# DevilInChina/spmv

Measured on AMD Instinct MI355X. Metric: SpMV GFLOP/s (fp64 CSR, y = A x through spmv()), higher is better.
Workload: dtype f64

## Files before the change

include/spmv_hip.h:

```cpp
#include "spmv_Defines.h"
#if defined(__cplusplus)
extern "C" {
#endif
#ifndef SPMV_HIP_EXT_H
#define SPMV_HIP_EXT_H

enum {
    SPMV_HIP_OK = 0,
    SPMV_HIP_E_NODEVICE = 1,
    SPMV_HIP_E_ALLOC = 2,
    SPMV_HIP_E_ARG = 3,
    SPMV_HIP_E_RUNTIME = 4,
    SPMV_HIP_E_NOSTATE = 5,
    SPMV_HIP_E_RANGE = 6
};
int spmv_hip_last_error(void);
const char *spmv_hip_last_error_string(void);
void spmv_hip_clear_error(void);

int spmv_hip_device_count(void);
int spmv_hip_set_stream(spmv_Handle_t handle, void *hip_stream);
int spmv_hip_set_async(spmv_Handle_t handle, int async);
int spmv_hip_synchronize(spmv_Handle_t handle);
void spmv_hip_trim_pool(void);
// ... 88 lines not shown
int spmv_hip_attention_merge(spmv_Handle_t handle, int heads, int dv,
                             const void *O1, long long ldo1, const void *L1, long long ldl1,
                             const void *O2, long long ldo2, const void *L2, long long ldl2,
                             void *O, long long ldo,
                             void *L, long long ldl);

int spmv_hip_attention_gqa_backward_lse(spmv_Handle_t handle, BASIC_INT_TYPE m, const BASIC_INT_TYPE *RowPtr, const BASIC_INT_TYPE *ColIdx,
                                        const void *Matrix_Val, int heads, int kv_heads, int k, int dv, double scale,
                                        const void *Q, long long ldq, const void *K, long long ldk, const void *V, long long ldv,
                                        const void *B, long long ldb,
                                        const void *G, long long ldg,
                                        const void *O, long long ldo,
                                        const void *L, long long ldl,
                                        void *dQ, long long lddq,
                                        void *dK, long long lddk,
                                        void *dV, long long lddv,
                                        void *dB, long long lddb);

enum { SPMV_HIP_T_HANDLE = 0, SPMV_HIP_T_F16 = 1, SPMV_HIP_T_BF16 = 2 };

int spmv_hip_attention_gqa_lse_16(spmv_Handle_t handle, BASIC_INT_TYPE m, const BASIC_INT_TYPE *RowPtr, const BASIC_INT_TYPE *ColIdx,
                                  const void *Matrix_Val, int heads, int kv_heads, int k, int dv, double scale,
                                  int io_type,
                                  const void *Q, long long ldq, const void *K, long long ldk, const void *V, long long ldv,
                                  const void *B, long long ldb,
                                  void *O, long long ldo, int o_type,
                                  void *L, long long ldl);

int spmv_hip_attention_gqa_backward_16(spmv_Handle_t handle, BASIC_INT_TYPE m, const BASIC_INT_TYPE *RowPtr, const BASIC_INT_TYPE *ColIdx,
                                       const void *Matrix_Val, int heads, int kv_heads, int k, int dv, double scale,
                                       int io_type,
                                       const void *Q, long long ldq, const void *K, long long ldk, const void *V, long long ldv,
                                       const void *B, long long ldb,
                                       const void *G, long long ldg,
                                       const void *O, long long ldo,
                                       const void *L, long long ldl,
                                       int dq_type, void *dQ, long long lddq,
                                       int dkv_type, void *dK, long long lddk,
                                       void *dV, long long lddv,
                                       void *dB, long long lddb);

int spmv_hip_set_option(const char *key, long value);
long spmv_hip_get_option(const char *key);
int spmv_hip_set_thread_option(const char *key, long value);
void spmv_hip_clear_thread_options(void);
long spmv_hip_get_handle_option(spmv_Handle_t handle, const char *key);

typedef struct spmv_hip_info {
    int device;
    int schedule;
    int lanes_per_row;
    int sell_c, sell_sigma;
    int tile_nnz;
    int m, n;
    long long nnz;
    long long stored_nnz;
    int max_row_len, min_row_len, empty_rows;
    double mean_row_len;
    long long device_bytes;
    long long alg_bytes;
    double inspect_ms;
    const char *schedule_name;
    const char *kernel_name;
    int tuned_choice;
    float tune_ms[3];
    int x_groups;
    int x_groups_staged;
    int cache_blocked;
    long long stream_bytes;
    long long x_bytes;
    float route_ms[2];
    float split_ms[2];
    long long far_nnz;
    long long run_nnz;
    long long byte_nnz;
    long long tmpl_nnz;
    int blk_waves;
    char launch_kernels[160];
    int reproducible;
    int x_span_max;
    int lds_bytes;
    long long packed_nnz;
    float pack_ms[2];
} spmv_hip_info;
int spmv_hip_get_info(spmv_Handle_t handle, spmv_hip_info *out);
int spmv_hip_get_transpose_info(spmv_Handle_t handle, spmv_hip_info *out);

int spmv_hip_multi_gpus(spmv_Handle_t handle);
int spmv_hip_multi_uses_rccl(spmv_Handle_t handle);
int spmv_hip_multi_slices(spmv_Handle_t handle, int gpu, void **x_slice, long long *x_first, long long *x_count,
                          void **y_block, long long *y_first, long long *y_count, int *device);
int spmv_hip_multi_step(spmv_Handle_t handle);
int spmv_hip_multi_step_async(spmv_Handle_t handle);
int spmv_hip_multi_synchronize(spmv_Handle_t handle);
void spmv_hip_create_handle_from_blocks(spmv_Handle_t *Handle, int blocks, const BASIC_INT_TYPE *rows, BASIC_INT_TYPE n,
                                        BASIC_INT_TYPE *const *RowPtr, BASIC_INT_TYPE *const *ColIdx, void *const *Matrix_Val,
                                        SPMV_METHODS Function, BASIC_SIZE_TYPE size);

enum { SPMV_HIP_CG_CONVERGED = 0, SPMV_HIP_CG_MAX_ITERATIONS = 1, SPMV_HIP_CG_BREAKDOWN = 2, SPMV_HIP_CG_NONFINITE = 3 };
typedef struct spmv_hip_cg_options {
    double rtol, atol;
    int max_iterations;
    int check_every;
    int use_x0;
    const void *Dinv;
    double *history;
} spmv_hip_cg_options;
typedef struct spmv_hip_cg_result {
    int status;
    int iterations;
    double rr, bb;
} spmv_hip_cg_result;
int spmv_hip_cg(spmv_Handle_t handle, BASIC_INT_TYPE m, const BASIC_INT_TYPE *RowPtr, const BASIC_INT_TYPE *ColIdx,
                const void *Matrix_Val, const void *B, void *X,
                const spmv_hip_cg_options *opt, spmv_hip_cg_result *res);

int spmv_hip_bicgstab(spmv_Handle_t handle, BASIC_INT_TYPE m, const BASIC_INT_TYPE *RowPtr, const BASIC_INT_TYPE *ColIdx,
                      const void *Matrix_Val, const void *B, void *X,
                      const spmv_hip_cg_options *opt, spmv_hip_cg_result *res);

#define SPMV_HIP_CG_COLUMNS_MAX 16
int spmv_hip_cg_columns(spmv_Handle_t handle, BASIC_INT_TYPE m, const BASIC_INT_TYPE *RowPtr, const BASIC_INT_TYPE *ColIdx,
                        const void *Matrix_Val, int k, const void *B, long long ldb, void *X, long long ldx,
                        const spmv_hip_cg_options *opt, spmv_hip_cg_result *res );

#define SPMV_HIP_GMRES_RESTART_MAX 32
int spmv_hip_gmres(spmv_Handle_t handle, BASIC_INT_TYPE m, const BASIC_INT_TYPE *RowPtr, const BASIC_INT_TYPE *ColIdx,
                   const void *Matrix_Val, const void *B, void *X, int restart,
                   const spmv_hip_cg_options *opt, spmv_hip_cg_result *res);

#endif

#if defined(__cplusplus)
}
#endif
```

spmv_amd/api.py:

```python
from __future__ import annotations

import ctypes as C
import enum
import math
import os

import numpy as np

_PKG = os.path.dirname(os.path.abspath(__file__))
LIB_PATH = os.path.join(_PKG, "lib", "libspmv_hip.so")


class VECTORIZED_WAY(enum.IntEnum):
    VECTOR_NONE = 0
    VECTOR_AVX2 = 1
    VECTOR_AVX512 = 2
    VECTOR_HIP = 3
    VECTOR_TOTAL_SIZE = 4


class SPMV_METHODS(enum.IntEnum):
    Method_Serial = 0
    Method_Parallel = 1
    Method_Balanced = 2
    Method_Balanced2 = 3
    Method_Balanced_Yid = 4
    Method_SellCSigma = 5
    Method_CSR5SPMV = 6
    Method_Total_Size = 7
    Method_Numa = 8


_I = C.POINTER(C.c_int)
_V = C.c_void_p


class spmv_Handle(C.Structure):
    _fields_ = [("spmvMethod", C.c_int), ("data_size", C.c_ulong), ("nthreads", C.c_ulong),
                ("vectorizedWay", C.c_int), ("Level_3_opt_used", C.c_int), ("RowPtr", _I),
                ("ColIdx", _I), ("index", _I), ("Matrix_Val", _V), ("Y_temp", _V),
                ("extraHandle", _V)]


spmv_Handle_t = C.POINTER(spmv_Handle)


class spmv_hip_info(C.Structure):
    _fields_ = [("device", C.c_int), ("schedule", C.c_int), ("lanes_per_row", C.c_int),
                ("sell_c", C.c_int), ("sell_sigma", C.c_int), ("tile_nnz", C.c_int),
                ("m", C.c_int), ("n", C.c_int), ("nnz", C.c_longlong), ("stored_nnz", C.c_longlong),
                ("max_row_len", C.c_int), ("min_row_len", C.c_int), ("empty_rows", C.c_int),
                ("mean_row_len", C.c_double), ("device_bytes", C.c_longlong),
                ("alg_bytes", C.c_longlong), ("inspect_ms", C.c_double),
                ("schedule_name", C.c_char_p), ("kernel_name", C.c_char_p),
                ("tuned_choice", C.c_int), ("tune_ms", C.c_float * 3),
                ("x_groups", C.c_int), ("x_groups_staged", C.c_int), ("cache_blocked", C.c_int),
                ("stream_bytes", C.c_longlong), ("x_bytes", C.c_longlong), ("route_ms", C.c_float * 2), ("split_ms", C.c_float * 2), ("far_nnz", C.c_longlong), ("run_nnz", C.c_longlong), ("byte_nnz", C.c_longlong), ("tmpl_nnz", C.c_longlong),
                ("blk_waves", C.c_int), ("launch_kernels", C.c_char * 160), ("reproducible", C.c_int),
                ("x_span_max", C.c_int), ("lds_bytes", C.c_int),
                ("packed_nnz", C.c_longlong), ("pack_ms", C.c_float * 2)]


class spmv_hip_cg_options(C.Structure):
    _fields_ = [("rtol", C.c_double), ("atol", C.c_double), ("max_iterations", C.c_int), ("check_every", C.c_int), ("use_x0", C.c_int),
                ("Dinv", C.c_void_p), ("history", C.POINTER(C.c_double))]


class spmv_hip_cg_result(C.Structure):
    _fields_ = [("status", C.c_int), ("iterations", C.c_int), ("rr", C.c_double), ("bb", C.c_double)]


CG_STATUS = ("converged", "max_iterations", "breakdown", "nonfinite")

_GQA = "heads kv_heads k dv scale"
_ATTENTION = {stem: tuple((sizes + " " + operands).split()) for stem, sizes, operands in (
    ("attention", "k dv scale", "Q K V O"),
    ("attention_heads", "heads k dv scale", "Q K V O"),
    ("attention_backward", "k dv scale", "Q K V G dQ dK dV"),
    ("attention_heads_backward", "heads k dv scale", "Q K V G dQ dK dV"),
    ("attention_bias", "heads k dv scale", "Q K V B O"),
    ("attention_bias_backward", "heads k dv scale", "Q K V B G dQ dK dV dB"),
    ("attention_gqa", _GQA, "Q K V B O"),
    ("attention_gqa_backward", _GQA, "Q K V B G dQ dK dV dB"),
    ("attention_gqa_lse", _GQA, "Q K V B O L"),
    ("attention_gqa_lse_16", _GQA + " io_type", "Q K V B O o_type L"),
    ("attention_gqa_backward_lse", _GQA, "Q K V B G O L dQ dK dV dB"),
    ("attention_gqa_backward_16", _GQA + " io_type", "Q K V B G O L dq_type dQ dkv_type dK dV dB"),
)}
_CSR = [spmv_Handle_t, C.c_int, _V, _V, _V]
_TIMED = [spmv_Handle_t]
_TAIL = [C.c_int, C.c_int, C.POINTER(C.c_float)]


def _attention_prototypes():
    out = {}
    for stem, row in _ATTENTION.items():
        args = []
        for name in row:
            args += [C.c_double] if name == "scale" else [C.c_int] if name.islower() else [_V, C.c_longlong]
        out[f"spmv_hip_{stem}"] = (C.c_int, _CSR + args)
        out[f"spmv_hip_time_{stem}_launches"] = (C.c_double, _TIMED + args + _TAIL)
    return out


FUNCTIONS = {
    "spmv_create_handle_all_in_one": (None, [C.POINTER(spmv_Handle_t), C.c_int, C.c_int, _V, _V, _V,
                                             C.c_ulong, C.c_int, C.c_ulong, C.c_int, C.c_char_p]),
    "spmv": (None, [spmv_Handle_t, C.c_int, _V, _V, _V, _V, _V]),
    "spmv_destory_handle": (None, [spmv_Handle_t]),
    "spmv_clear_handle": (None, [spmv_Handle_t]),
    "spmv_hip_last_error": (C.c_int, []),
    "spmv_hip_last_error_string": (C.c_char_p, []),
    "spmv_hip_clear_error": (None, []),
    "spmv_hip_device_count": (C.c_int, []),
    "spmv_hip_trim_pool": (None, []),
    "spmv_hip_set_stream": (C.c_int, [spmv_Handle_t, _V]),
    "spmv_hip_set_async": (C.c_int, [spmv_Handle_t, C.c_int]),
    "spmv_hip_synchronize": (C.c_int, [spmv_Handle_t]),
    "spmv_hip_set_option": (C.c_int, [C.c_char_p, C.c_long]),
    "spmv_hip_get_option": (C.c_long, [C.c_char_p]),
    "spmv_hip_set_thread_option": (C.c_int, [C.c_char_p, C.c_long]),
    "spmv_hip_clear_thread_options": (None, []),
    "spmv_hip_get_handle_option": (C.c_long, [spmv_Handle_t, C.c_char_p]),
    "spmv_hip_update_values": (C.c_int, [spmv_Handle_t, _V]),
    "spmv_hip_multi_gpus": (C.c_int, [spmv_Handle_t]),
    "spmv_hip_multi_uses_rccl": (C.c_int, [spmv_Handle_t]),
    "spmv_hip_multi_slices": (C.c_int, [spmv_Handle_t, C.c_int, C.POINTER(_V), C.POINTER(C.c_longlong), C.POINTER(C.c_longlong),
                                        C.POINTER(_V), C.POINTER(C.c_longlong), C.POINTER(C.c_longlong), _I]),
    "spmv_hip_multi_step": (C.c_int, [spmv_Handle_t]),
    "spmv_hip_multi_step_async": (C.c_int, [spmv_Handle_t]),
    "spmv_hip_multi_synchronize": (C.c_int, [spmv_Handle_t]),
    "spmv_hip_create_handle_from_blocks": (None, [C.POINTER(spmv_Handle_t), C.c_int, _I, C.c_int, C.POINTER(_V), C.POINTER(_V), C.POINTER(_V),
                                                  C.c_int, C.c_ulong]),
    "spmv_hip_get_info": (C.c_int, [spmv_Handle_t, C.POINTER(spmv_hip_info)]),
    "spmv_hip_time_launches": (C.c_double, [spmv_Handle_t, _V, _V, C.c_int, C.c_int, C.POINTER(C.c_float)]),
    "spmv_hip_spmm": (C.c_int, [spmv_Handle_t, C.c_int, _V, _V, _V, C.c_int, _V, C.c_longlong, _V, C.c_longlong]),
    "spmv_hip_time_spmm_launches": (C.c_double, [spmv_Handle_t, C.c_int, _V, C.c_longlong, _V, C.c_longlong, C.c_int, C.c_int,
                                                 C.POINTER(C.c_float)]),
    "spmv_hip_spmv_transpose": (C.c_int, [spmv_Handle_t, C.c_int, _V, _V, _V, _V, _V]),
    "spmv_hip_prepare_transpose": (C.c_int, [spmv_Handle_t]),
    "spmv_hip_get_transpose_info": (C.c_int, [spmv_Handle_t, C.POINTER(spmv_hip_info)]),
    "spmv_hip_time_transpose_launches": (C.c_double, [spmv_Handle_t, _V, _V, C.c_int, C.c_int, C.POINTER(C.c_float)]),
    "spmv_hip_transpose_map": (C.c_int, [spmv_Handle_t, _I, _I]),
# ... 95 lines not shown


def _ptr(a):
    if a is None:
        return None
    if isinstance(a, int):
        return a
    if isinstance(a, np.ndarray):
        if not a.flags["C_CONTIGUOUS"]:
            raise ValueError("array must be contiguous")
        return a.ctypes.data
    if hasattr(a, "data_ptr"):
        if not a.is_contiguous():
            raise ValueError("tensor must be contiguous")
        return a.data_ptr()
    raise TypeError(type(a))


def _itemsize(a):
    return a.dtype.itemsize if isinstance(a, np.ndarray) else a.element_size()


def spmv_create_handle_all_in_one(m, n, RowPtr, ColIdx, Matrix_Val, nthreads, Function, size,
                                  vectorizedWay=VECTORIZED_WAY.VECTOR_HIP, MtxToken=None, check=True):
    lib = load()
    lib.spmv_hip_clear_error()
    h = spmv_Handle_t()
    tok = MtxToken.encode() if isinstance(MtxToken, str) else MtxToken
    lib.spmv_create_handle_all_in_one(C.byref(h), int(m), int(n), _ptr(RowPtr), _ptr(ColIdx), _ptr(Matrix_Val),
                                      int(nthreads), int(Function), int(size), int(vectorizedWay), tok)
    if check:
        _raise_if_error("spmv_create_handle_all_in_one")
    return h


def spmv(handle, m, RowPtr, ColIdx, Matrix_Val, Vector_Val_X, Vector_Val_Y, check=True):
    lib = load()
    lib.spmv(handle, int(m), _ptr(RowPtr), _ptr(ColIdx), _ptr(Matrix_Val), _ptr(Vector_Val_X), _ptr(Vector_Val_Y))
    if check:
        _raise_if_error("spmv")


def spmv_destory_handle(handle):
    load().spmv_destory_handle(handle)


def spmv_clear_handle(handle):
    load().spmv_clear_handle(handle)


def set_option(key, value):
    if load().spmv_hip_set_option(key.encode(), int(value)) != 0:
        load().spmv_hip_clear_error()
        raise ValueError(f"bad option {key}={value}")


def get_option(key):
    return load().spmv_hip_get_option(key.encode())


def set_thread_option(key, value):
    if load().spmv_hip_set_thread_option(key.encode(), int(value)) != 0:
        load().spmv_hip_clear_error()
        raise ValueError(f"bad option {key}={value}")


def clear_thread_options():
    load().spmv_hip_clear_thread_options()


def update_values(handle, Matrix_Val):
    _checked(load().spmv_hip_update_values(handle, _ptr(Matrix_Val)), "spmv_hip_update_values")


def _info_dict(info):
    out = {k: getattr(info, k) for k, _ in spmv_hip_info._fields_}
    out["schedule_name"] = (out["schedule_name"] or b"").decode()
    out["kernel_name"] = (out["kernel_name"] or b"").decode()
    out["launch_kernels"] = [k for k in (out["launch_kernels"] or b"").decode().split("+") if k]
    out["tune_ms"] = [float(v) for v in out["tune_ms"]]
    out["route_ms"] = [float(v) for v in out["route_ms"]]
    out["split_ms"] = [float(v) for v in out["split_ms"]]
    out["pack_ms"] = [float(v) for v in out["pack_ms"]]
    return out


def get_info(handle):
    info = spmv_hip_info()
    _checked(load().spmv_hip_get_info(handle, C.byref(info)), "spmv_hip_get_info")
    return _info_dict(info)


def get_transpose_info(handle):
    info = spmv_hip_info()
    _checked(load().spmv_hip_get_transpose_info(handle, C.byref(info)), "spmv_hip_get_transpose_info")
    return _info_dict(info)


def set_stream(handle, stream_ptr, async_=True):
    lib = load()
    lib.spmv_hip_set_stream(handle, stream_ptr)
    lib.spmv_hip_set_async(handle, 1 if async_ else 0)
    _raise_if_error("spmv_hip_set_stream")


def time_launches(handle, x, y, warmup=10, iters=100):
    return _timed("spmv_hip_time_launches", (handle, _ptr(x), _ptr(y)), warmup, iters)


def _block(a, name):
    if a is None:
        return None, 0, 0, 0
    if isinstance(a, np.ndarray):
        if a.ndim == 2 and a.size == 0:
            return a.ctypes.data, a.shape[0], a.shape[1], max(a.shape[1], 1)
        if a.ndim != 2 or (a.strides[1] != a.itemsize and a.shape[1] > 1) or a.strides[0] % a.itemsize:
            raise ValueError(f"{name} must be 2-D with column stride 1")
        return a.ctypes.data, a.shape[0], a.shape[1], a.strides[0] // a.itemsize
    if hasattr(a, "data_ptr"):
        if a.dim() != 2 or (a.stride(1) != 1 and a.shape[1] > 1):
            raise ValueError(f"{name} must be 2-D with column stride 1")
        return a.data_ptr(), a.shape[0], a.shape[1], a.stride(0)
    raise TypeError(type(a))


def _blocks(A, a_name, B, b_name):
    pa, _, k, lda = _block(A, a_name)
    pb, _, kb, ldb = _block(B, b_name)
    if A is not None and B is not None and kb != k:
        raise ValueError(f"{a_name} has {k} columns, {b_name} {kb}")
    if A is None:
        k = kb
    return int(k), pa, int(max(lda, 1) if A is not None else k), pb, int(max(ldb, 1) if B is not None else k)


def spmm(handle, m, RowPtr, ColIdx, Matrix_Val, X, Y, check=True):
    k, px, ldx, py, ldy = _blocks(X, "X", Y, "Y")
    return _checked(load().spmv_hip_spmm(handle, int(m), _ptr(RowPtr), _ptr(ColIdx), _ptr(Matrix_Val), k, px, ldx, py, ldy), "spmv_hip_spmm", check)


def time_spmm_launches(handle, X, Y, warmup=10, iters=100):
    px, _, k, ldx = _block(X, "X")
    py, _, _, ldy = _block(Y, "Y")
    return _timed("spmv_hip_time_spmm_launches", (handle, int(k), px, int(max(ldx, 1)), py, int(max(ldy, 1))), warmup, iters)


def spmv_transpose(handle, m, RowPtr, ColIdx, Matrix_Val, X, Y, check=True):
    return _checked(load().spmv_hip_spmv_transpose(handle, int(m), _ptr(RowPtr), _ptr(ColIdx), _ptr(Matrix_Val), _ptr(X), _ptr(Y)), "spmv_hip_spmv_transpose", check)


def prepare_transpose(handle, check=True):
    return _checked(load().spmv_hip_prepare_transpose(handle), "spmv_hip_prepare_transpose", check)


def time_transpose_launches(handle, x, y, warmup=10, iters=100):
    return _timed("spmv_hip_time_transpose_launches", (handle, _ptr(x), _ptr(y)), warmup, iters)


def transpose_map(handle, n, nnz):
    rp = np.empty(int(n) + 1, dtype=np.int32)
    perm = np.empty(max(int(nnz), 1), dtype=np.int32)
    _checked(load().spmv_hip_transpose_map(handle, rp.ctypes.data_as(_I), perm.ctypes.data_as(_I)), "spmv_hip_transpose_map")
    return rp, perm[:int(nnz)]


def spmm_transpose(handle, m, RowPtr, ColIdx, Matrix_Val, X, Y, check=True):
# ... 703 lines not shown
```

spmv_amd/csrc/kernels/csr_vector_tile.hpp:

```cpp
#pragma once
#include <climits>
#include <type_traits>
#include "common.hpp"
#include "csr_vector4.hpp"
#include "xwindows.hpp"

namespace spmv {

constexpr int kVecTileThreads = 256;
constexpr int kVecTileRows = kVecTileThreads;
constexpr int kTmplMax = 64;
constexpr int kTmplCount = 8;
constexpr int kTmplRows = 1024;
__device__ __forceinline__ void tile_rows(int b, int m, int rows_per_tile, const int *__restrict__ split, long long &r0, long long &r1)
{
    if (split) { r0 = split[b]; r1 = split[b + 1]; }
    else { r0 = (long long) b * rows_per_tile; r1 = r0 + rows_per_tile < m ? r0 + rows_per_tile : m; }
}

template <typename T, int L>
struct Lane4 {
    static constexpr int EPL = 16 / (int) sizeof(T);
    static __device__ __forceinline__ int pos(int l, int k) { return (k / EPL) * EPL * L + EPL * l + (k % EPL); }
    static __device__ __forceinline__ void load_val(const T *__restrict__ val, int base, int l, T (&v)[4])
// ... 219 lines not shown
        sum = group_sum_dpp<L>(sum);
        if (l == 0) y_lds[s * RW + sub] = sum;
        if (s + D < L) issue(s + D);
    }
    wave_lds_sync();
    const long long row = rw0 + lane;
    const int len = rp_lds[lane + 1] - rp_lds[lane];
    if (row < row_end && len <= long_thr) y[row] = y_lds[lane];
}

template <typename T, int L, int DEPTH = 4, bool PRE = true, bool PACK = false>
__global__ __launch_bounds__(kVecTileThreads) void csr_vector_tile_kernel(int m, int long_thr, const int *__restrict__ rowptr,
                                                                          const int *__restrict__ colidx,
                                                                          const unsigned short *__restrict__ col_local,
                                                                          const T *__restrict__ val,
                                                                          const TileWindows *__restrict__ wins,
                                                                          const unsigned short *__restrict__ row_slot,
                                                                          const unsigned char *__restrict__ col8,
                                                                          const unsigned short *__restrict__ tmpl, const unsigned char *__restrict__ row_tid,
                                                                          const T *__restrict__ x, T *__restrict__ y,
                                                                          const unsigned *__restrict__ pk_lo = nullptr, const unsigned char *__restrict__ pk_hi = nullptr,
                                                                          const int *__restrict__ tile_e = nullptr)
{
    extern __shared__ __attribute__((aligned(16))) unsigned char vec_x_lds[];
    __shared__ unsigned short tm_lds[kTmplCount * kTmplMax];
    T *xs = reinterpret_cast<T *>(vec_x_lds);
    __shared__ int rp_lds[kVecTileThreads / kWave][kWave + 2];
    __shared__ unsigned rs_lds[kVecTileThreads / kWave][kWave];
    __shared__ T y_lds[kVecTileThreads / kWave][kWave];
    const int lane = threadIdx.x & (kWave - 1), wave = threadIdx.x / kWave;
    const long long rw0 = (long long) blockIdx.x * kVecTileRows + wave * kWave;
    long long r = rw0 + lane, re = rw0 + kWave;
    if (r > m) r = m;
    if (re > m) re = m;
    const int rp = rowptr[r];
    const int rpe = rowptr[re];
    const TileWindows &tw = wins[blockIdx.x];
    const bool staged = tw.nwin > 0, runs = tw.runs == 1, bytes = tw.runs == 2, templ = tw.runs == 3;
    int c0[4] = {0, 0, 0, 0};
    T v0[4] = {T(0), T(0), T(0), T(0)};
    PackArgs pk;
    PackRaw r0;
    bool packed = false;
    if constexpr (PACK) {
        pk.lo = pk_lo; pk.hi = pk_hi; pk.e = tile_e[blockIdx.x];
        packed = pk.e != kPackNone;
    }
    if (PRE) {
        const int sub = lane / L, l = lane % L;
        const int q0 = __shfl(rp, sub, kWave);
        const int a = q0 & ~3;
        if (runs | templ) {}
        else if (bytes) Lane4<T, L>::load_col8(col8, a, l, c0);
        else if (staged) Lane4<T, L>::load_col16(col_local, a, l, c0);
        else Lane4<T, L>::load_col32(colidx, a, l, c0);
        if (PACK && packed) r0.load(pk, a, l);
        else Lane4<T, L>::load_val(val, a, l, v0);
    }
    rp_lds[wave][lane] = rp;
    if (lane == 0) rp_lds[wave][kWave] = rpe;
    if (runs | bytes) rs_lds[wave][lane] = row_slot[r];
    if (templ) {
        rs_lds[wave][lane] = (unsigned) row_slot[r] | ((unsigned) row_tid[r] * kTmplMax << 16);
        for (int i = threadIdx.x; i < kTmplCount * kTmplMax; i += kVecTileThreads) tm_lds[i] = tmpl[(size_t) blockIdx.x * (kTmplCount * kTmplMax) + i];
    }
    stage_windows<kVecTileThreads, T>(tw, x, xs);
    if (threadIdx.x == 0) xs[tw.total] = T(0);
    __syncthreads();
    if (rw0 >= m) return;
    const unsigned zoff = (unsigned) tw.total * (unsigned) sizeof(T);
#define SPMV_TILE_WAVE(MODE, ...)                                                                                                                                   \
    do {                                                                                                                                                            \
        if (PACK && packed) csr_vector_tile_wave<T, L, MODE, DEPTH, PRE, 0, PACK>((long long) m, long_thr, rw0, lane, rp_lds[wave], rs_lds[wave], y_lds[wave], colidx, col_local, val, x, xs, zoff, y, c0, v0, __VA_ARGS__, pk, r0); \
        else csr_vector_tile_wave<T, L, MODE, DEPTH, PRE>((long long) m, long_thr, rw0, lane, rp_lds[wave], rs_lds[wave], y_lds[wave], colidx, col_local, val, x, xs, zoff, y, c0, v0, __VA_ARGS__); \
    } while (0)
    if (runs) SPMV_TILE_WAVE(2, col8, nullptr);
    else if (bytes) SPMV_TILE_WAVE(3, col8, nullptr);
    else if (templ) SPMV_TILE_WAVE(4, col8, tm_lds);
    else if (staged) SPMV_TILE_WAVE(1, col8, nullptr);
    else SPMV_TILE_WAVE(0, col8, nullptr);
#undef SPMV_TILE_WAVE
}

template <typename T, int L, int DEPTH = 4, bool WIDE = false>
__global__ __launch_bounds__(kVecTileThreads) void csr_vector_rows_kernel(int long_thr, const int *__restrict__ split,
                                                                          int rows_per_block, int m,
                                                                          const int *__restrict__ rowptr,
                                                                          const int *__restrict__ colidx,
                                                                          const unsigned short *__restrict__ col_local,
                                                                          const T *__restrict__ val,
                                                                          const TileWindows *__restrict__ wins,
                                                                          const unsigned short *__restrict__ row_slot,
                                                                          const unsigned char *__restrict__ col8,
                                                                          const unsigned short *__restrict__ tmpl, const unsigned char *__restrict__ row_tid,
                                                                          const T *__restrict__ x, T *__restrict__ y)
{
    __shared__ unsigned short tm_lds[kTmplCount * kTmplMax];
    constexpr int SHIFT = WIDE ? (sizeof(T) == 8 ? 3 : 2) : 0;
    extern __shared__ __attribute__((aligned(16))) unsigned char vec_x_lds[];
    T *xs = reinterpret_cast<T *>(vec_x_lds);
    __shared__ int rp_lds[kVecTileThreads / kWave][kWave + 2];
    __shared__ unsigned rs_lds[kVecTileThreads / kWave][kWave];
    __shared__ T y_lds[kVecTileThreads / kWave][kWave];
    const int lane = threadIdx.x & (kWave - 1), wave = threadIdx.x / kWave;
    long long r_begin, r_end;
    tile_rows(blockIdx.x, m, rows_per_block, split, r_begin, r_end);
    const TileWindows &tw = wins[blockIdx.x];
    const bool staged = tw.nwin > 0, runs = tw.runs == 1, bytes = tw.runs == 2, templ = tw.runs == 3;
    if (templ) for (int i = threadIdx.x; i < kTmplCount * kTmplMax; i += kVecTileThreads) tm_lds[i] = tmpl[(size_t) blockIdx.x * (kTmplCount * kTmplMax) + i];
    stage_windows<kVecTileThreads, T>(tw, x, xs);
    if (threadIdx.x == 0) xs[tw.total] = T(0);
    __syncthreads();
    const unsigned zoff = WIDE ? (unsigned) tw.total : (unsigned) tw.total * (unsigned) sizeof(T);
    const int c0[4] = {0, 0, 0, 0};
    const T v0[4] = {T(0), T(0), T(0), T(0)};
    for (long long rw0 = r_begin + (long long) wave * kWave; rw0 < r_end; rw0 += kVecTileRows) {
        long long r = rw0 + lane, re = rw0 + kWave;
        if (r > r_end) r = r_end;
        if (re > r_end) re = r_end;
        rp_lds[wave][lane] = rowptr[r];
        if (lane == 0) rp_lds[wave][kWave] = rowptr[re];
        if (runs | bytes) rs_lds[wave][lane] = row_slot[r];
        if (templ) rs_lds[wave][lane] = (unsigned) row_slot[r] | ((unsigned) row_tid[r] * kTmplMax << 16);
        wave_lds_sync();
        if (runs) csr_vector_tile_wave<T, L, 2, DEPTH, false, SHIFT>(r_end, long_thr, rw0, lane, rp_lds[wave], rs_lds[wave], y_lds[wave], colidx, col_local, val, x, xs, zoff, y, c0, v0);
        else if (bytes) csr_vector_tile_wave<T, L, 3, DEPTH, false, SHIFT>(r_end, long_thr, rw0, lane, rp_lds[wave], rs_lds[wave], y_lds[wave], colidx, col_local, val, x, xs, zoff, y, c0, v0, col8);
        else if (templ) csr_vector_tile_wave<T, L, 4, DEPTH, false, SHIFT>(r_end, long_thr, rw0, lane, rp_lds[wave], rs_lds[wave], y_lds[wave], colidx, col_local, val, x, xs, zoff, y, c0, v0, col8, tm_lds);
        else if (staged) csr_vector_tile_wave<T, L, 1, DEPTH, false, SHIFT>(r_end, long_thr, rw0, lane, rp_lds[wave], rs_lds[wave], y_lds[wave], colidx, col_local, val, x, xs, zoff, y, c0, v0);
        else csr_vector_tile_wave<T, L, 0, DEPTH, false, SHIFT>(r_end, long_thr, rw0, lane, rp_lds[wave], rs_lds[wave], y_lds[wave], colidx, col_local, val, x, xs, zoff, y, c0, v0);
        wave_lds_sync();
    }
}

enum { kVecPipeKernel, kVecTileKernel, kVecRowsKernel };
struct VecArgs {
    int kernel = kVecPipeKernel;
    int lanes = 64, depth = 4;
    bool pre = true, wide = false;
    int m = 0, long_thr = INT_MAX, tiles = 0, maxspan = 0, rows = 256;
    const int *rowptr = nullptr, *colidx = nullptr, *split = nullptr;
    const void *val = nullptr;
    const unsigned short *col = nullptr, *rowslot = nullptr, *tmpl = nullptr;
    const unsigned char *col8 = nullptr, *rowtid = nullptr;
    const TileWindows *wins = nullptr;
    const unsigned *pk_lo = nullptr;
    const unsigned char *pk_hi = nullptr;
    const int *pk_e = nullptr;
    int device = 0;
    hipStream_t stream = nullptr;
};
hipError_t vector_launch(const VecArgs &a, const double *x, double *y);
hipError_t vector_launch(const VecArgs &a, const float *x, float *y);
hipError_t vector_launch_packed(const VecArgs &a, const double *x, double *y);
hipError_t rows_launch(const VecArgs &a, const double *x, double *y);
hipError_t rows_launch(const VecArgs &a, const float *x, float *y);

}
```

spmv_amd/csrc/kernels/xwindows_inspect.hpp:

```cpp
#pragma once
#include "csr_vector_tile.hpp"

namespace spmv {

static __global__ __launch_bounds__(kBlock) void csr_tile_windows_kernel(int m, int n, int rows_per_tile, int long_thr, int max_cols, int slot_bytes,
                                                                  const int *__restrict__ split,
                                                                  const int *__restrict__ rowptr,
                                                                  const int *__restrict__ colidx,
                                                                  TileWindows *__restrict__ wins,
                                                                  unsigned short *__restrict__ col_local,
                                                                  unsigned short *__restrict__ row_slot ,
                                                                  unsigned char *__restrict__ col8 ,
                                                                  unsigned short *__restrict__ tmpl ,
                                                                  unsigned char *__restrict__ row_tid ,
                                                                  int *__restrict__ staged )
{
    long long r0, r1;
    tile_rows(blockIdx.x, m, rows_per_tile, split, r0, r1);
    const int sub = threadIdx.x / 16, l = threadIdx.x % 16;
    auto loop = [&](auto body) {
        for (long long r = r0 + sub; r < r1; r += kBlock / 16) {
            const int p0 = rowptr[r], p1 = rowptr[r + 1];
            if (p1 - p0 > long_thr) continue;
            for (int p = p0 + l; p < p1; p += 16) body(colidx[p], (long long) p);
// ... 106 lines not shown
            int mn = INT_MAX, mx = 0;
            for (int p = p0 + l; p < p1; p += 16) { const int sl = col_local[p]; mn = sl < mn ? sl : mn; mx = sl > mx ? sl : mx; }
#pragma unroll
            for (int o = 8; o > 0; o >>= 1) { mn = min(mn, __shfl_xor(mn, o, 16)); mx = max(mx, __shfl_xor(mx, o, 16)); }
            okb &= mx - mn <= 255 * slot_bytes;
            if (l == 0) nb += p1 - p0;
        }
        okb = __syncthreads_and(okb);
        if (!okb) return;
        for (long long r = r0 + sub; r < r1; r += kBlock / 16) {
            const int p0 = rowptr[r], p1 = rowptr[r + 1];
            int mn = INT_MAX;
            const bool on = p1 - p0 <= long_thr && p1 > p0;
            if (on) for (int p = p0 + l; p < p1; p += 16) { const int sl = col_local[p]; mn = sl < mn ? sl : mn; }
#pragma unroll
            for (int o = 8; o > 0; o >>= 1) mn = min(mn, __shfl_xor(mn, o, 16));
            if (on) for (int p = p0 + l; p < p1; p += 16) col8[p] = (unsigned char) ((col_local[p] - mn) / slot_bytes);
            if (l == 0) row_slot[r] = (unsigned short) (on ? mn : 0);
        }
#pragma unroll
        for (int o = kWave / 2; o > 0; o >>= 1) nb += __shfl_xor(nb, o, kWave);
        if ((threadIdx.x & (kWave - 1)) == 0 && nb) atomicAdd(staged + 6, nb);
        if (threadIdx.x == 0) {
            wins[blockIdx.x].runs = 2;
            atomicAdd(staged + 5, 1);
            atomicAdd(staged + 7, (int) (r1 - r0));
        }
        return;
    }
    for (long long r = r0 + sub * 16 + l; r < r1; r += kBlock) {
        const int p0 = rowptr[r], p1 = rowptr[r + 1];
        int slot = 0;
        if (p1 > p0 && p1 - p0 <= long_thr) {
            const int c0 = colidx[p0];
            int w = 0;
            for (int k = 1; k < nwin; ++k) w = c0 >= tw.start[k] ? k : w;
            slot = (tw.base[w] + (c0 - tw.start[w])) * slot_bytes;
        }
        row_slot[r] = (unsigned short) slot;
    }
#pragma unroll
    for (int o = kWave / 2; o > 0; o >>= 1) entries += __shfl_xor(entries, o, kWave);
    if ((threadIdx.x & (kWave - 1)) == 0 && entries) atomicAdd(staged + 3, entries);
    if (threadIdx.x == 0) {
        wins[blockIdx.x].runs = 1;
        atomicAdd(staged + 2, 1);
        atomicAdd(staged + 4, (int) (r1 - r0));
    }
}

static __global__ __launch_bounds__(kBlock) void range_windows_kernel(long long total, long long group_len,
                                                               const long long *__restrict__ bounds, int bstride, int scale,
                                                               long long nbounds ,
                                                               int n, int max_cols, int *__restrict__ cols,
                                                               unsigned short *__restrict__ cols16, int pack16,
                                                               TileWindows *__restrict__ wins, int *__restrict__ staged, int rewrite)
{
    long long b, e;
    if (bounds) {
        long long i0 = (long long) blockIdx.x * bstride, i1 = i0 + bstride;
        if (i0 > nbounds) i0 = nbounds;
        if (i1 > nbounds) i1 = nbounds;
        b = bounds[i0] * scale;
        e = bounds[i1] * scale;
    }
    else { b = (long long) blockIdx.x * group_len; e = b + group_len; }
    if (e > total) e = total;
    auto loop = [&](auto body) {
        for (long long i = b + threadIdx.x; i < e; i += kBlock) body(cols[i], i);
    };
    auto store = [&](long long pos, int slot, int tile_total) {
        if (!cols16) { if (slot >= 0) cols[pos] = slot; return; }
        long long q = pos;
        if (pack16) {
            const long long tn = (long long) kWave * pack16, t = pos / tn;
            const int o = (int) (pos - t * tn), i = o / kWave, lane = o % kWave;
            q = t * tn + (i / 4) * (4 * kWave) + lane * 4 + (i % 4);
        }
        cols16[q] = (unsigned short) (slot >= 0 ? slot : tile_total);
    };
    build_windows(n, max_cols, loop, store, wins[blockIdx.x], staged, rewrite != 0);
}

static __global__ __launch_bounds__(kBlock) void wins_total_kernel(int count, const TileWindows *__restrict__ wins, unsigned long long *__restrict__ sum,
                                                            unsigned long long *__restrict__ staged_tiles)
{
    unsigned long long t = 0, c = 0;
    for (long long i = (long long) blockIdx.x * kBlock + threadIdx.x; i < count; i += (long long) gridDim.x * kBlock)
        if (wins[i].nwin > 0) { t += (unsigned long long) wins[i].total; c += 1; }
#pragma unroll
    for (int o = kWave / 2; o > 0; o >>= 1) { t += __shfl_xor(t, o, kWave); c += __shfl_xor(c, o, kWave); }
    if ((threadIdx.x & (kWave - 1)) == 0 && c) { atomicAdd(sum, t); atomicAdd(staged_tiles, c); }
}

}
```

spmv_amd/csrc/shim/inspect.hpp:

```cpp
#pragma once

static int build_range_windows(spmv_dev *d, int groups, long long total, long long group_len, const long long *bounds, int bstride,
                               int scale, int max_cols, int *cols, TileWindows *wins, int *staged_out, int *maxtotal_out,
                               unsigned short *cols16 = nullptr, int pack16 = 0, long long nbounds = 0)
{
    int *cnt = nullptr;
    int host2[2] = {0, 0};
    *staged_out = *maxtotal_out = 0;
    if (groups <= 0) return SPMV_HIP_OK;
    HIP_TRY(pool_malloc((void **) &cnt, 2 * sizeof(int)));
    hipError_t e = hipMemsetAsync(cnt, 0, 2 * sizeof(int), d->stream);
    range_windows_kernel<<<groups, kBlock, 0, d->stream>>>(total, group_len, bounds, bstride, scale, nbounds, d->n, max_cols, cols, cols16, pack16, wins, cnt, 0);
    if (e == hipSuccess) e = hipGetLastError();
    if (e == hipSuccess) e = hipMemcpyAsync(host2, cnt, sizeof host2, hipMemcpyDeviceToHost, d->stream);
    if (e == hipSuccess) e = hipStreamSynchronize(d->stream);
    if (e == hipSuccess && host2[0] * 2 >= groups) {
        range_windows_kernel<<<groups, kBlock, 0, d->stream>>>(total, group_len, bounds, bstride, scale, nbounds, d->n, max_cols, cols, cols16, pack16, wins, cnt, 1);
        e = hipGetLastError();
        if (e == hipSuccess) e = hipStreamSynchronize(d->stream);
        *staged_out = host2[0];
        *maxtotal_out = host2[1];
    }
    (void) pool_free(cnt);
    if (e != hipSuccess) return fail(SPMV_HIP_E_RUNTIME, "x-window inspector: %s", hipGetErrorString(e));
    return SPMV_HIP_OK;
}

constexpr size_t kVecXTileBytes = 48 * 1024;
template <typename T> static int build_long_rows(spmv_dev *d, int thr);
template <typename T>
static int build_csr5(spmv_dev *d, Csr5Plan &P, int m, long long nnz, const int *rowptr, const int *colidx, const T *val, int empty_rows,
                      double mean_row_len, const int *out_rows, bool natural = false, int sigma_override = 0);
template <typename T> static int autotune_vector(spmv_dev *d);
template <typename T> static int autotune_rows(spmv_dev *d);
static int build_packed_values(spmv_dev *d);
template <typename T> static int autotune_blocked(spmv_dev *d);
template <typename T> static double time_schedule(spmv_dev *d, int iters);
template <typename T> static int split_make(spmv_dev *d, spmv_dev **near_out, spmv_dev **far_out, bool values_only);
template <typename T> static int build_tile_windows(spmv_dev *d, int tiles, const int *split, int rows_per_tile = kVecTileRows, bool wide = false);
static int wins_sum(spmv_dev *d, const TileWindows *wins, int count, long long *elems, long long *tiles);
constexpr size_t kVecWideXTileBytes = 96 * 1024;

static int build_rowblock(spmv_dev *d)
{
    d->rb_stride = d->plan.rowblock_nnz;
    d->nblocks = (int) ((d->nnz + d->rb_stride - 1) / d->rb_stride);
    if (d->nblocks < 1) d->nblocks = 1;
    ALLOC_TRY(d, &d->rb_split, sizeof(int) * ((size_t) d->nblocks + 1), true);
    rowblock_split_kernel<<<grid_for((long long) d->nblocks + 1, kBlock, INT_MAX), kBlock, 0, d->stream>>>(
        d->m, (int) d->nnz, d->nblocks, d->rb_stride, d->rowptr, d->rb_split);
    HIP_TRY(hipGetLastError());
    HIP_TRY(hipStreamSynchronize(d->stream));
    return SPMV_HIP_OK;
}

template <typename T>
static int build_rowblock_tiles(spmv_dev *d)
{
    const int L = d->plan.lanes_per_row;
    int rc = build_long_rows<T>(d, L * 64 > 256 ? L * 64 : 256);
    if (rc) return rc;
    rc = build_tile_windows<T>(d, d->nblocks, d->rb_split);
    if (rc) return rc;
    if (d->vt_staged * 2 < d->vt_tiles && !d->plan.forced) {
        rc = build_tile_windows<T>(d, d->nblocks, d->rb_split, kVecTileRows, true);
        if (rc) return rc;
        if (d->vt_staged * 2 < d->vt_tiles) rc = build_tile_windows<T>(d, d->nblocks, d->rb_split);
    }
    return rc;
}

template <typename T>
static int build_tile_windows(spmv_dev *d, int tiles, const int *split, int rows_per_tile, bool wide)
{
    int *cnt = nullptr;
    int host2[11] = {0, 0, 0, 0, 0, 0, 0, 0, 0, 0, 0};
    d->vt_tiles = tiles;
    ALLOC_TRY(d, &cnt, sizeof host2, true);
    static_assert(kVecXTileBytes <= 65536, "LDS byte offsets must fit 16 bits");
    static_assert(kVecWideXTileBytes / sizeof(float) <= 65536, "LDS slot indices must fit 16 bits");
    if (!d->vt_col) {
        ALLOC_TRY(d, &d->vt_col, sizeof(unsigned short) * ((size_t) d->nnz + kStreamPad), true);
        HIP_TRY(hipMemsetAsync(d->vt_col, 0, sizeof(unsigned short) * ((size_t) d->nnz + kStreamPad), d->stream));
    }
    if (!d->vt_rowslot && d->plan.run_tiles) {
        ALLOC_TRY(d, &d->vt_rowslot, sizeof(unsigned short) * ((size_t) d->m + kStreamPad), true);
        HIP_TRY(hipMemsetAsync(d->vt_rowslot, 0, sizeof(unsigned short) * ((size_t) d->m + kStreamPad), d->stream));
    }
    if (!d->vt_col8 && d->vt_rowslot && !getenv("SPMV_HIP_NO_BYTE_TILES")) {
        ALLOC_TRY(d, &d->vt_col8, (size_t) d->nnz + kStreamPad, true);
        HIP_TRY(hipMemsetAsync(d->vt_col8, 0, (size_t) d->nnz + kStreamPad, d->stream));
    }
    if (d->vt_tmpl) { sched_free(d, d->vt_tmpl); d->vt_tmpl = nullptr; }
    if (d->vt_rowslot && !getenv("SPMV_HIP_NO_TEMPLATE_TILES")) {
        ALLOC_TRY(d, &d->vt_tmpl, sizeof(unsigned short) * kTmplCount * kTmplMax * (size_t) tiles, true);
        if (!d->vt_rowtid) {
            ALLOC_TRY(d, &d->vt_rowtid, (size_t) d->m + kStreamPad, true);
            HIP_TRY(hipMemsetAsync(d->vt_rowtid, 0, (size_t) d->m + kStreamPad, d->stream));
        }
    }
    if (d->vt_wins) sched_free(d, d->vt_wins);
    ALLOC_TRY(d, &d->vt_wins, sizeof(TileWindows) * (size_t) tiles, true);
    HIP_TRY(hipMemsetAsync(cnt, 0, sizeof host2, d->stream));
    csr_tile_windows_kernel<<<tiles, kBlock, 0, d->stream>>>(d->m, d->n, rows_per_tile, d->long_thr,
                                                             (int) ((wide ? kVecWideXTileBytes : kVecXTileBytes) / sizeof(T)) - 1, wide ? 1 : (int) sizeof(T),
                                                             split, d->rowptr, d->colidx,
                                                             d->vt_wins, d->vt_col, d->vt_rowslot, d->vt_col8, d->vt_tmpl, d->vt_rowtid, cnt);
    HIP_TRY(hipGetLastError());
    HIP_TRY(hipMemcpyAsync(host2, cnt, sizeof host2, hipMemcpyDeviceToHost, d->stream));
    HIP_TRY(hipStreamSynchronize(d->stream));
    d->vt_staged = host2[0];
    d->vt_maxspan = host2[1];
    d->vt_run_tiles = host2[2];
    d->vt_run_nnz = host2[3];
    d->vt_run_rows = host2[4];
    d->vt_byte_tiles = host2[5];
    d->vt_byte_nnz = host2[6];
    d->vt_byte_rows = host2[7];
    d->vt_tmpl_tiles = host2[8];
    d->vt_tmpl_nnz = host2[9];
    d->vt_tmpl_rows = host2[10];
    if (d->vt_tmpl && d->vt_tmpl_tiles == 0) { sched_free(d, d->vt_tmpl); d->vt_tmpl = nullptr; sched_free(d, d->vt_rowtid); d->vt_rowtid = nullptr; }
    if (d->vt_col8 && d->vt_byte_tiles == 0) { sched_free(d, d->vt_col8); d->vt_col8 = nullptr; }
    d->vt_wide = wide;
    d->vt_rows = rows_per_tile;
    return SPMV_HIP_OK;
}

constexpr size_t kSellXTileBytes = 96 * 1024;

template <typename T>
static int build_long_rows(spmv_dev *d, int thr)
{
    d->long_thr = thr;
    d->nlong = 0;
    d->c5_long = Csr5Plan();
    if (d->stats.max_row_len <= thr) return SPMV_HIP_OK;
    const int nb = (int) (((long long) d->m + kScanTile - 1) / kScanTile);
    int *flags = nullptr, *sums = nullptr, *total = nullptr, *scratch = nullptr;
    ALLOC_TRY(d, &sums, sizeof(int) * (size_t) nb, true);
    ALLOC_TRY(d, &total, sizeof(int), true);
    HIP_TRY(pool_malloc((void **) &flags, sizeof(int) * (size_t) d->m));
    long_rows_flag_kernel<<<grid_for(d->m, kBlock, d->cus * 8), kBlock, 0, d->stream>>>(d->m, thr, d->rowptr, flags);
    scan_block_sums_kernel<<<nb, kBlock, 0, d->stream>>>(d->m, flags, sums);
    scan_sums_inplace_kernel<<<1, kBlock, 0, d->stream>>>(nb, sums, total);
    if (hipMemcpyAsync(&d->nlong, total, sizeof(int), hipMemcpyDeviceToHost, d->stream) != hipSuccess || hipStreamSynchronize(d->stream) != hipSuccess) {
        (void) pool_free(flags);
        d->nlong = 0;
        return fail(SPMV_HIP_E_RUNTIME, "long-row scan failed");
    }
    if (d->nlong == 0) { (void) pool_free(flags); return SPMV_HIP_OK; }
    int rc = dev_alloc(d, (void **) &d->long_rows, sizeof(int) * (size_t) d->nlong, true);
    if (!rc) rc = dev_alloc(d, (void **) &scratch, sizeof(int) * (size_t) d->nlong, true);
    if (rc) { (void) pool_free(flags); d->nlong = 0; return rc; }
    csr5_compact_kernel<<<nb, kBlock, 0, d->stream>>>(d->m, flags, sums, d->rowptr, scratch, d->long_rows);
    hipError_t e = hipStreamSynchronize(d->stream);
    (void) pool_free(flags);
    if (e != hipSuccess) { d->nlong = 0; return fail(SPMV_HIP_E_RUNTIME, "long-row compaction: %s", hipGetErrorString(e)); }
    ALLOC_TRY(d, &d->lr_seg_start, sizeof(long long) * ((size_t) d->nlong + 1), true);

    {
        long long sub_nnz = 0;
        long_rows_len_kernel<<<grid_for(d->nlong, kBlock, INT_MAX), kBlock, 0, d->stream>>>(d->nlong, d->long_rows, d->rowptr, scratch);
        scan_i32_to_i64_kernel<<<1, kBlock, 0, d->stream>>>(d->nlong, scratch, d->lr_seg_start);
        HIP_TRY(hipGetLastError());
        HIP_TRY(hipMemcpyAsync(&sub_nnz, d->lr_seg_start + d->nlong, sizeof(long long), hipMemcpyDeviceToHost, d->stream));
        HIP_TRY(hipStreamSynchronize(d->stream));
        d->lsub_nnz = sub_nnz;
        ALLOC_TRY(d, &d->lsub_rowptr, sizeof(int) * ((size_t) d->nlong + 1), true);
        ALLOC_TRY(d, &d->lsub_colidx, sizeof(int) * (size_t) sub_nnz, true);
        ALLOC_TRY(d, &d->lsub_val, sizeof(T) * (size_t) sub_nnz, true);
        narrow_i64_kernel<<<grid_for((long long) d->nlong + 1, kBlock, INT_MAX), kBlock, 0, d->stream>>>(d->nlong + 1, d->lr_seg_start, d->lsub_rowptr);
        long_rows_gather_kernel<T><<<d->nlong, kBlock, 0, d->stream>>>(d->long_rows, d->rowptr, d->colidx, (const T *) d->val, d->lsub_rowptr,
                                                                      d->lsub_colidx, (T *) d->lsub_val);
        HIP_TRY(hipGetLastError());
        return build_csr5<T>(d, d->c5_long, d->nlong, sub_nnz, d->lsub_rowptr, d->lsub_colidx, (const T *) d->lsub_val, 0,
                             (double) sub_nnz / (double) d->nlong, d->long_rows);
    }
}


template <typename T>
static int build_vector_tiles(spmv_dev *d)
{
    d->vt_staged = d->vt_maxspan = 0;
    const int rows = kVecTileRows;
    d->vt_tiles = (int) (((long long) d->m + rows - 1) / rows);
    if (d->vt_tiles == 0 || d->nnz == 0) return SPMV_HIP_OK;
    int rc = build_tile_windows<T>(d, d->vt_tiles, nullptr, rows);
    if (rc || d->plan.forced) return rc;
    if (d->vt_staged * 2 >= d->vt_tiles) {
        long long welems = 0, wtiles = 0;
        const long long stream = (d->nnz - d->lsub_nnz) * ((long long) sizeof(T) + 2);
        if (getenv("SPMV_HIP_NO_WIDE_BY_COST") || wins_sum(d, d->vt_wins, d->vt_tiles, &welems, &wtiles) != SPMV_HIP_OK || stream <= 0 ||
            (double) welems * sizeof(T) <= 0.5 * (double) stream)
            return SPMV_HIP_OK;
        const int narrow_tiles = d->vt_tiles, w_rows = 4 * kVecTileRows;
        const int w_tiles = (int) (((long long) d->m + w_rows - 1) / w_rows);
        rc = build_tile_windows<T>(d, w_tiles, nullptr, w_rows, true);
        if (rc) return rc;
        long long welems_w = 0;
        if (d->vt_staged == d->vt_tiles && wins_sum(d, d->vt_wins, d->vt_tiles, &welems_w, &wtiles) == SPMV_HIP_OK && welems_w * 2 <= welems) return SPMV_HIP_OK;
        return build_tile_windows<T>(d, narrow_tiles, nullptr, rows);
    }
    const int wide_rows = 4 * kVecTileRows;
    const int wide_tiles = (int) (((long long) d->m + wide_rows - 1) / wide_rows);
    rc = build_tile_windows<T>(d, wide_tiles, nullptr, wide_rows, true);
    if (rc) return rc;
    if (d->vt_staged * 2 >= d->vt_tiles) return SPMV_HIP_OK;
    return build_tile_windows<T>(d, (int) (((long long) d->m + rows - 1) / rows), nullptr, rows);
}

static __global__ __launch_bounds__(kVecTileThreads) void pack_tiles_kernel(int m, int L, int long_thr, const int *__restrict__ rowptr, const double *__restrict__ val,
                                                                            unsigned *__restrict__ lo, unsigned char *__restrict__ hi, int *__restrict__ tile_e,
                                                                            unsigned long long *__restrict__ cnt)
{
    __shared__ int s_bad, s_top, s_low;
    const int C = 4 * L;
    const long long r0 = (long long) blockIdx.x * kVecTileRows, r1 = r0 + kVecTileRows < m ? r0 + kVecTileRows : m;
    if (threadIdx.x == 0) { s_bad = 0; s_top = INT_MIN; s_low = INT_MAX; }
    __syncthreads();
    const int p_begin = rowptr[r0], p_end = rowptr[r1];
    int bad = 0, top = INT_MIN, low = INT_MAX;
    if (r0 + threadIdx.x < r1) {
        const int a = rowptr[r0 + threadIdx.x], len = rowptr[r0 + threadIdx.x + 1] - a;
        bad = (a & (C - 1)) != 0 || (len & (C - 1)) != 0 || len > long_thr;
    }
    for (int p = p_begin + (int) threadIdx.x; p < p_end; p += kVecTileThreads) {
        const unsigned long long b = (unsigned long long) __double_as_longlong(val[p]);
        const int E = (int) ((b >> 52) & 0x7ff);
        const unsigned long long frac = b & 0xfffffffffffffull;
        if (E == 0x7ff || b == 0x8000000000000000ull) bad = 1;
        else if (E | (frac != 0)) {
            const unsigned long long mant = E ? frac | (1ull << 52) : frac;
            const int base = (E ? E : 1) - 1075;
            top = max(top, base + 63 - __clzll((long long) mant));
            low = min(low, base + __ffsll((long long) mant) - 1);
        }
    }
#pragma unroll
    for (int o = kWave / 2; o > 0; o >>= 1) {
        bad |= __shfl_xor(bad, o, kWave);
        top = max(top, __shfl_xor(top, o, kWave));
        low = min(low, __shfl_xor(low, o, kWave));
    }
    if ((threadIdx.x & (kWave - 1)) == 0) {
        if (bad) atomicOr(&s_bad, 1);
        atomicMax(&s_top, top);
        atomicMin(&s_low, low);
    }
    __syncthreads();
    const bool zero = s_top == INT_MIN;
    const bool ok = !s_bad && (zero || s_top - s_low <= 54);
    const int e = zero ? 0 : s_low;
    if (threadIdx.x == 0) {
        tile_e[blockIdx.x] = ok ? e : kPackNone;
        if (ok) { atomicAdd(cnt, 1ull); atomicAdd(cnt + 1, (unsigned long long) (p_end - p_begin)); }
    }
    if (!ok || !lo) return;
    for (int s = p_begin + 4 * (int) threadIdx.x; s < p_end; s += 4 * kVecTileThreads) {
        const int q = s & (C - 1), blk = s - q, l = q >> 2;
        unsigned w[4], h[4];
#pragma unroll
        for (int k = 0; k < 4; ++k) {
            const unsigned long long b = (unsigned long long) __double_as_longlong(val[blk + (k >> 1) * 2 * L + 2 * l + (k & 1)]);
            const int E = (int) ((b >> 52) & 0x7ff);
            const unsigned long long frac = b & 0xfffffffffffffull;
            const unsigned long long mant = E ? frac | (1ull << 52) : frac;
            const int sh = (E ? E : 1) - 1075 - e;
            long long kk = sh >= 0 ? (long long) (mant << sh) : (long long) (mant >> -sh);
            if (b >> 63) kk = -kk;
            w[k] = (unsigned) kk;
            h[k] = (unsigned) (kk >> 32) & 0xffffffu;
// ... 529 lines not shown
    if (threadIdx.x == 0 && distinct > seg_limit && distinct * 3 > wlen) atomicAdd(hopeless, 1);
}

static bool sample_says_no_locality(spmv_dev *d)
{
    constexpr int kWindows = 64, kLen = 4096;
    if (d->nnz < (long long) kWindows * kLen * 4) return false;
    int *cnt = nullptr, h = 0;
    if (pool_malloc((void **) &cnt, sizeof(int)) != hipSuccess) { (void) hipGetLastError(); return false; }
    hipError_t e = hipMemsetAsync(cnt, 0, sizeof(int), d->stream);
    const int seg_limit = (int) (kCsr5XTileBytes / d->vsize / 64);
    locality_sample_kernel<<<kWindows, kBlock, 0, d->stream>>>(d->nnz, kWindows, kLen, d->colidx, seg_limit, cnt);
    if (e == hipSuccess) e = hipGetLastError();
    if (e == hipSuccess) e = hipMemcpyAsync(&h, cnt, sizeof(int), hipMemcpyDeviceToHost, d->stream);
    if (e == hipSuccess) e = hipStreamSynchronize(d->stream);
    (void) pool_free(cnt);
    if (e != hipSuccess) { (void) hipGetLastError(); return false; }
    return h * 16 >= kWindows * 15;
}

struct Traffic {
    long long bytes = 0, x_elems = 0;
    bool gathers_global = false;
};

static int wins_sum(spmv_dev *d, const TileWindows *wins, int count, long long *elems, long long *tiles)
{
    *elems = *tiles = 0;
    if (!wins || count <= 0) return SPMV_HIP_OK;
    unsigned long long *dv = nullptr, hv[2] = {0, 0};
    HIP_TRY(pool_malloc((void **) &dv, sizeof hv));
    hipError_t e = hipMemsetAsync(dv, 0, sizeof hv, d->stream);
    wins_total_kernel<<<grid_for(count, kBlock, d->cus * 4), kBlock, 0, d->stream>>>(count, wins, dv, dv + 1);
    if (e == hipSuccess) e = hipGetLastError();
    if (e == hipSuccess) e = hipMemcpyAsync(hv, dv, sizeof hv, hipMemcpyDeviceToHost, d->stream);
    if (e == hipSuccess) e = hipStreamSynchronize(d->stream);
    (void) pool_free(dv);
    if (e != hipSuccess) return fail(SPMV_HIP_E_RUNTIME, "window totals: %s", hipGetErrorString(e));
    *elems = (long long) hv[0];
    *tiles = (long long) hv[1];
    return SPMV_HIP_OK;
}

static long long stream_part(long long stored, long long s, double fs)
{
    return stored * s + (long long) ((double) stored * (2.0 * fs + 4.0 * (1.0 - fs)));
}

static int csr5_traffic(spmv_dev *d, const Csr5Plan &P, Traffic &t)
{
    if (P.nnz == 0) return SPMV_HIP_OK;
    const long long s = (long long) d->vsize, TN = (long long) kWave * P.sigma, p = P.tiles;
    long long welems = 0, wtiles = 0;
    if (P.staged > 0) { const int rc = wins_sum(d, P.wins, P.groups, &welems, &wtiles); if (rc) return rc; }
    const double fs = P.groups > 0 ? (double) wtiles / (double) P.groups : 0.0;
    t.bytes += stream_part(P.natural ? P.nnz : p * TN, s, fs);
    t.bytes += 4 * (p + 1) + 4 * kWave * p + s * p;
    if (P.forward) t.bytes += 4ll * p;
    else if (P.fixup && p > 1) t.bytes += (s + 8) * p;
    if (P.staged > 0) t.bytes += (long long) sizeof(TileWindows) * P.groups;
    t.bytes += P.run_tiles * (4ll * kWave - 2ll * TN);
    if (P.row_map) t.bytes += 4ll * P.m2;
    t.bytes += s * P.m2 + (s + 4) * (long long) P.n_empty;
    t.x_elems += welems;
    if (wtiles < P.groups) t.gathers_global = true;
    return SPMV_HIP_OK;
}

static int account_stream_bytes(spmv_dev *d)
{
    const long long s = (long long) d->vsize, m = d->m, n = d->n;
    Traffic t;
    int rc = SPMV_HIP_OK;
    if (d->blk_on) {
        t.bytes = (d->blk.groups << d->blk.ge) * (s + 4) + 4ll * d->blk.groups + (long long) (sizeof(BlkDir) + 8) * d->blk.B + s * m;
        t.gathers_global = true;
    } else {
        switch (d->plan.sched) {
        case SPMV_SCHED_CSR_VECTOR:
        case SPMV_SCHED_ROWBLOCK: {
            long long welems = 0, wtiles = 0;
            rc = wins_sum(d, d->vt_wins, d->vt_tiles, &welems, &wtiles);
            if (rc) return rc;
            const bool tile_form = d->vt_tiles > 0 && (d->plan.sched == SPMV_SCHED_ROWBLOCK || d->vt_wide || d->vt_staged * 2 >= d->vt_tiles);
            const double fs = tile_form && d->vt_tiles > 0 ? (double) wtiles / (double) d->vt_tiles : 0.0;
            t.bytes = 4 * (m + 1) + stream_part(d->nnz - d->lsub_nnz, s, fs) + s * (m - d->nlong);
            if (tile_form) { t.bytes += (long long) sizeof(TileWindows) * d->vt_tiles; t.x_elems = welems; }
            if (tile_form) t.bytes += 2ll * d->vt_run_rows - 2ll * d->vt_run_nnz;
            if (tile_form) t.bytes += 3ll * d->vt_tmpl_rows + 2ll * kTmplCount * kTmplMax * d->vt_tmpl_tiles - 2ll * d->vt_tmpl_nnz;
            if (tile_form) t.bytes += 2ll * d->vt_byte_rows - 1ll * d->vt_byte_nnz;
            t.bytes += packed_stream_bytes(d);
            if (d->plan.sched == SPMV_SCHED_ROWBLOCK) t.bytes += 4ll * (d->nblocks + 1);
            if (!tile_form || wtiles < d->vt_tiles) t.gathers_global = true;
            rc = csr5_traffic(d, d->c5_long, t);
            break;
        }
        case SPMV_SCHED_NNZ_SPLIT: rc = csr5_traffic(d, d->ns, t); break;
        case SPMV_SCHED_CSR5: rc = csr5_traffic(d, d->c5, t); break;
        case SPMV_SCHED_SELL: {
            long long welems = 0, wtiles = 0;
            if (d->sell_staged > 0) { rc = wins_sum(d, d->sell_wins, d->sell_nwin, &welems, &wtiles); if (rc) return rc; }
            const double fs = d->sell_nwin > 0 ? (double) wtiles / (double) d->sell_nwin : 0.0;
            t.bytes = stream_part(d->sell_cols * kSellC, s, fs) + 8ll * (d->nchunks + 1) + 4ll * d->nchunks * kSellC + s * (m - d->nlong);
            t.bytes += 4ll * d->sell_run_slots - 2ll * d->sell_run_stored;
            t.bytes += 4ll * d->sell_byte_slots - d->sell_byte_stored;
            if (d->sell_staged > 0) t.bytes += (long long) sizeof(TileWindows) * d->sell_nwin;
            t.x_elems = welems;
            if (wtiles < d->sell_nwin) t.gathers_global = true;
            rc = csr5_traffic(d, d->c5_long, t);
            break;
        }
        default:
            t.bytes = 4 * (m + 1) + d->nnz * (4 + s) + s * m;
            t.gathers_global = d->nnz > 0;
            break;
        }
    }
    if (rc) return rc;
    const long long x_cap = 8ll * n;
    d->x_bytes = s * ((t.x_elems < x_cap ? t.x_elems : x_cap) + (t.gathers_global ? n : 0));
    d->stream_bytes = t.bytes + d->x_bytes;
    return SPMV_HIP_OK;
}
```

spmv_amd/csrc/shim/launch.hpp:

```cpp
#pragma once

enum { VEC_AUTO = 0, VEC_PIPE = 4, VEC_TILE_D2 = 5, VEC_TILE_D8 = 6, VEC_TILE_D4 = 10, VEC_TILE_D4_NOPRE = 11, VEC_TILE_D2_NOPRE = 12 };

static VecArgs vector_args(const spmv_dev *d)
{
    VecArgs a;
    const bool f64 = d->vsize == sizeof(double);
    if (d->plan.sched == SPMV_SCHED_ROWBLOCK || d->vt_wide) {
        const int v = d->plan.vector_form;
        a.kernel = kVecRowsKernel;
        a.depth = d->rows_depth ? d->rows_depth : (f64 ? 4 : 2);
        if (v == VEC_TILE_D2 || v == VEC_TILE_D2_NOPRE) a.depth = 2;
        if (v == VEC_TILE_D4 || v == VEC_TILE_D4_NOPRE) a.depth = 4;
        a.wide = d->vt_wide;
        a.split = d->plan.sched == SPMV_SCHED_ROWBLOCK ? d->rb_split : nullptr;
    } else {
        const int v = d->plan.vector_form ? d->plan.vector_form : d->vec_choice;
        const bool tile_default = d->vt_staged * 2 >= d->vt_tiles;
        const bool tile_forced = v == VEC_TILE_D2 || v == VEC_TILE_D4 || v == VEC_TILE_D8 || v == VEC_TILE_D4_NOPRE || v == VEC_TILE_D2_NOPRE;
        if (d->vt_tiles > 0 && v != VEC_PIPE && (tile_default || tile_forced)) {
            a.kernel = kVecTileKernel;
            a.depth = v == VEC_TILE_D2 || v == VEC_TILE_D2_NOPRE ? 2 : v == VEC_TILE_D8 ? 8 : v == VEC_TILE_D4 || v == VEC_TILE_D4_NOPRE ? 4 : (f64 ? 4 : 2);
            a.pre = v != VEC_TILE_D4_NOPRE && v != VEC_TILE_D2_NOPRE;
        }
    }
    a.lanes = d->plan.lanes_per_row; a.m = d->m; a.long_thr = d->long_thr; a.tiles = d->vt_tiles; a.maxspan = d->vt_maxspan; a.rows = d->vt_rows;
    a.rowptr = d->rowptr; a.colidx = d->colidx; a.val = d->val; a.wins = d->vt_wins;
    a.col = d->vt_col; a.rowslot = d->vt_rowslot; a.tmpl = d->vt_tmpl; a.col8 = d->vt_col8; a.rowtid = d->vt_rowtid;
    a.device = d->device; a.stream = d->stream;
    if (d->pk_use && a.kernel == kVecTileKernel && a.depth != 8) {
        a.pk_lo = d->pk_lo; a.pk_hi = d->pk_hi; a.pk_e = d->pk_e;
        if (d->pk_depth) a.depth = d->pk_depth;
    }
    return a;
}

template <typename T>
static hipError_t launch_vector(const spmv_dev *d, const T *x, T *y)
{
    const VecArgs a = vector_args(d);
    return a.kernel == kVecRowsKernel ? rows_launch(a, x, y) : vector_launch(a, x, y);
}

template <typename T>
static int autotune_vector(spmv_dev *d)
{
    d->vec_choice = VEC_AUTO;
    if (d->nnz < (1ll << 24) || d->plan.forced || d->vt_tiles <= 0) return SPMV_HIP_OK;
    if (d->vt_wide || d->vt_staged * 2 < d->vt_tiles) return SPMV_HIP_OK;
    T *x = nullptr, *y = nullptr;
    if (pool_malloc((void **) &x, sizeof(T) * (size_t) d->n) != hipSuccess || pool_malloc((void **) &y, sizeof(T) * (size_t) d->m) != hipSuccess) {
        (void) hipGetLastError();
        if (x) (void) pool_free(x);
        return SPMV_HIP_OK;
    }
    fill_value_kernel<T><<<grid_for(d->n, kBlock, d->cus * 8), kBlock, 0, d->stream>>>(d->n, x, T(1));
    hipEvent_t e0, e1;
    (void) hipEventCreate(&e0);
    (void) hipEventCreate(&e1);
    constexpr int kCand = 5;
    const int cand[kCand] = {VEC_TILE_D4, VEC_TILE_D4_NOPRE, VEC_TILE_D2, VEC_TILE_D2_NOPRE, VEC_PIPE};
    const int ncand = (long long) d->vt_staged * 100 >= (long long) d->vt_tiles * 99 ? kCand - 1 : kCand;
    float tmin[kCand];
    for (int k = 0; k < kCand; ++k) tmin[k] = 1e30f;
    for (int k = 0; k < ncand; ++k) { d->vec_choice = cand[k]; (void) launch_vector<T>(d, x, y); }
    for (int round = 0; round < 3; ++round)
        for (int k = 0; k < ncand; ++k) {
            d->vec_choice = cand[k];
            (void) hipEventRecord(e0, d->stream);
            (void) launch_vector<T>(d, x, y);
            (void) hipEventRecord(e1, d->stream);
            (void) hipEventSynchronize(e1);
            float ms = 0;
            (void) hipEventElapsedTime(&ms, e0, e1);
            if (ms < tmin[k]) tmin[k] = ms;
        }
    float best = 1e30f;
    int best_c = VEC_AUTO;
    for (int k = 0; k < kCand - 1; ++k) {
        if (tmin[k] < best) { best = tmin[k]; best_c = cand[k]; }
    }
    if (ncand == kCand && tmin[kCand - 1] < 0.95f * best) { best = tmin[kCand - 1]; best_c = VEC_PIPE; }
    d->tune_ms[0] = tmin[0] < tmin[1] ? tmin[0] : tmin[1];
    d->tune_ms[1] = tmin[2] < tmin[3] ? tmin[2] : tmin[3];
    d->tune_ms[2] = ncand == kCand ? tmin[4] : 0.f;
    d->vec_choice = best_c;
    (void) hipEventDestroy(e0);
    (void) hipEventDestroy(e1);
    (void) pool_free(x);
    (void) pool_free(y);
    if (hipGetLastError() != hipSuccess) d->vec_choice = VEC_AUTO;
    return SPMV_HIP_OK;
}

static void free_packed_values(spmv_dev *d)
{
    quiesce(d);
    for (void *p : {(void *) d->pk_lo, (void *) d->pk_hi, (void *) d->pk_e, (void *) d->pk_cnt}) if (p) sched_free(d, p);
    d->pk_lo = nullptr; d->pk_hi = nullptr; d->pk_e = nullptr; d->pk_cnt = nullptr;
    d->pk_tiles = d->pk_nnz = 0; d->pk_use = false; d->pk_depth = 0;
}

static int build_packed_values(spmv_dev *d)
{
    const int mode = d->plan.pack_values;
    d->pack_ms[0] = d->pack_ms[1] = 0;
    if (mode == 0 || d->vsize != sizeof(double) || d->plan.sched != SPMV_SCHED_CSR_VECTOR || d->vt_wide || d->vt_tiles <= 0 || d->nnz == 0) return SPMV_HIP_OK;
    const VecArgs plain = vector_args(d);
    if (plain.kernel != kVecTileKernel || plain.depth == 8) return SPMV_HIP_OK;
    const bool timed = d->vec_choice != VEC_AUTO;
    if (mode == 2 && !timed) return SPMV_HIP_OK;
    int rc = SPMV_HIP_OK;
    ALLOC_TRY(d, &d->pk_e, sizeof(int) * (size_t) d->vt_tiles, true);
    ALLOC_TRY(d, &d->pk_cnt, 2 * sizeof(unsigned long long), true);
    if (mode == 2) {
        rc = pack_tiles_run(d, false);
        if (rc || d->pk_tiles * 2 < d->vt_tiles) { free_packed_values(d); return rc; }
    }
    if ((rc = dev_alloc(d, (void **) &d->pk_lo, sizeof(unsigned) * ((size_t) d->nnz + kStreamPad), true)) ||
        (rc = dev_alloc(d, (void **) &d->pk_hi, 3 * ((size_t) d->nnz + kStreamPad) + 4, true))) {
        (void) hipGetLastError();
        free_packed_values(d);
        return mode == 2 ? SPMV_HIP_OK : rc;
    }
    HIP_TRY(hipMemsetAsync(d->pk_lo + d->nnz, 0, sizeof(unsigned) * kStreamPad, d->stream));
    HIP_TRY(hipMemsetAsync(d->pk_hi + 3 * (size_t) d->nnz, 0, 3 * (size_t) kStreamPad + 4, d->stream));
    rc = pack_tiles_run(d, true);
    if (rc || d->pk_tiles == 0) { free_packed_values(d); return rc; }
    if (mode == 1) { d->pk_use = true; return SPMV_HIP_OK; }
    double *x = nullptr, *y = nullptr;
    if (pool_malloc((void **) &x, sizeof(double) * (size_t) d->n) != hipSuccess || pool_malloc((void **) &y, sizeof(double) * (size_t) d->m) != hipSuccess) {
        (void) hipGetLastError();
        if (x) (void) pool_free(x);
        free_packed_values(d);
        return SPMV_HIP_OK;
    }
    fill_value_kernel<double><<<grid_for(d->n, kBlock, d->cus * 8), kBlock, 0, d->stream>>>(d->n, x, 1.0);
    hipEvent_t e0, e1;
    (void) hipEventCreate(&e0);
    (void) hipEventCreate(&e1);
    constexpr int kCand = 3;
    const int depth[kCand] = {0, 4, 2};
    float tmin[kCand] = {1e30f, 1e30f, 1e30f};
    auto set = [&](int k) { d->pk_use = k > 0; d->pk_depth = depth[k]; };
    for (int k = 0; k < kCand; ++k) { set(k); (void) launch_vector<double>(d, x, y); }
    for (int round = 0; round < 3; ++round)
        for (int k = 0; k < kCand; ++k) {
            set(k);
            (void) hipEventRecord(e0, d->stream);
            (void) launch_vector<double>(d, x, y);
            (void) hipEventRecord(e1, d->stream);
            (void) hipEventSynchronize(e1);
            float ms = 0;
            (void) hipEventElapsedTime(&ms, e0, e1);
            if (ms < tmin[k]) tmin[k] = ms;
        }
    (void) hipEventDestroy(e0);
    (void) hipEventDestroy(e1);
    (void) pool_free(x);
    (void) pool_free(y);
    float plain_best = tmin[0];
    for (int k = 0; k < 2; ++k) if (d->tune_ms[k] > 0 && d->tune_ms[k] < plain_best) plain_best = d->tune_ms[k];
    const int best = tmin[2] < tmin[1] ? 2 : 1;
    d->pack_ms[0] = plain_best;
    d->pack_ms[1] = tmin[best];
    if (hipGetLastError() != hipSuccess || !(tmin[best] < 0.95f * plain_best)) { free_packed_values(d); return SPMV_HIP_OK; }
    d->pk_use = true;
    d->pk_depth = depth[best];
    return SPMV_HIP_OK;
}

static void blocked_forms(const BlkSet &S, int un[2])
{
    un[0] = S.waves == 8 ? 6 : 8;
    un[1] = S.waves == 8 ? 8 : 12;
}

template <typename T>
static void launch_blocked(spmv_dev *d, const T *x, T *y)
{
    const BlkSet &S = d->blk;
    const size_t lds = blocked_lds_bytes(S);
#define SPMV_BLK_LAUNCH(UN, DBG)                                                                                                  \
    do {                                                                                                                          \
        ensure_lds<blk_kernel<T, UN, DBG>>(d->device, lds);                                                                       \
        blk_kernel<T, UN, DBG><<<S.B, kWave, lds, d->stream>>>(S.row0, S.R, S.dir, (const T *) S.val, S.meta, S.hdr, S.order, x, y, d->accumulate ? 1 : 0); \
    } while (0)
#define SPMV_BLK_WLAUNCH(UN, W, ORD)                                                                                              \
    do {                                                                                                                          \
        ensure_lds<blk_wide_kernel<T, UN, W, ORD>>(d->device, lds);                                                               \
// ... 26 lines not shown
}

template <typename T>
static int autotune_blocked(spmv_dev *d)
{
    d->blk.form = 0;
    d->blk.tune_ms[0] = d->blk.tune_ms[1] = d->blk.tune_ms[2] = 0;
    if (!d->blk_on || !d->plan.autotune || d->plan.blk_groups != 0) return SPMV_HIP_OK;
    T *x = nullptr, *y = nullptr;
    if (pool_malloc((void **) &x, sizeof(T) * (size_t) d->n) != hipSuccess || pool_malloc((void **) &y, sizeof(T) * (size_t) d->m) != hipSuccess) {
        (void) hipGetLastError();
        if (x) (void) pool_free(x);
        return SPMV_HIP_OK;
    }
    fill_value_kernel<T><<<grid_for(d->n, kBlock, d->cus * 8), kBlock, 0, d->stream>>>(d->n, x, T(1));
    hipEvent_t e0, e1;
    (void) hipEventCreate(&e0);
    (void) hipEventCreate(&e1);
    constexpr int kForms = 2;
    float tmin[kForms] = {1e30f, 1e30f};
    for (int f = 0; f < kForms; ++f) { d->blk.form = f; launch_blocked<T>(d, x, y); }
    for (int round = 0; round < 4; ++round)
        for (int f = 0; f < kForms; ++f) {
            d->blk.form = f;
            (void) hipEventRecord(e0, d->stream);
            launch_blocked<T>(d, x, y);
            (void) hipEventRecord(e1, d->stream);
            (void) hipEventSynchronize(e1);
            float ms = 0;
            (void) hipEventElapsedTime(&ms, e0, e1);
            if (ms < tmin[f]) tmin[f] = ms;
        }
    int best = 0;
    for (int f = 0; f < kForms; ++f) { d->blk.tune_ms[f] = tmin[f]; if (tmin[f] < tmin[best]) best = f; }
    d->blk.form = best;
    (void) hipEventDestroy(e0);
    (void) hipEventDestroy(e1);
    (void) pool_free(x);
    (void) pool_free(y);
    if (hipGetLastError() != hipSuccess) d->blk.form = 0;
    return SPMV_HIP_OK;
}

template <typename T>
static int autotune_rows(spmv_dev *d)
{
    d->rows_depth = 0;
    if (d->nnz < (1ll << 24) || d->plan.forced || d->vt_tiles <= 0 || d->vt_staged * 2 < d->vt_tiles) return SPMV_HIP_OK;
    T *x = nullptr, *y = nullptr;
    if (pool_malloc((void **) &x, sizeof(T) * (size_t) d->n) != hipSuccess || pool_malloc((void **) &y, sizeof(T) * (size_t) d->m) != hipSuccess) {
        (void) hipGetLastError();
        if (x) (void) pool_free(x);
        return SPMV_HIP_OK;
    }
    fill_value_kernel<T><<<grid_for(d->n, kBlock, d->cus * 8), kBlock, 0, d->stream>>>(d->n, x, T(1));
    hipEvent_t e0, e1;
    (void) hipEventCreate(&e0);
    (void) hipEventCreate(&e1);
    const int depth[2] = {4, 2};
    float tmin[2] = {1e30f, 1e30f};
    for (int k = 0; k < 2; ++k) { d->rows_depth = depth[k]; (void) launch_vector<T>(d, x, y); }
    for (int round = 0; round < 2; ++round)
        for (int k = 0; k < 2; ++k) {
            d->rows_depth = depth[k];
            (void) hipEventRecord(e0, d->stream);
            (void) launch_vector<T>(d, x, y);
            (void) hipEventRecord(e1, d->stream);
            (void) hipEventSynchronize(e1);
            float ms = 0;
            (void) hipEventElapsedTime(&ms, e0, e1);
            if (ms < tmin[k]) tmin[k] = ms;
        }
    d->tune_ms[0] = tmin[0];
    d->tune_ms[1] = tmin[1];
    d->rows_depth = tmin[1] < tmin[0] ? 2 : 4;
    (void) hipEventDestroy(e0);
    (void) hipEventDestroy(e1);
    (void) pool_free(x);
    (void) pool_free(y);
    if (hipGetLastError() != hipSuccess) d->rows_depth = 0;
    return SPMV_HIP_OK;
}

static bool csr5_two_deep(const spmv_dev *d, const Csr5Plan &P)
{
    if (P.natural || P.staged <= 0 || P.staged != P.groups || P.group_tiles > kCsr5PipeMaxGroupTiles || d->plan.csr5_two_deep == 1) return false;
    return d->vsize == sizeof(float) || d->plan.csr5_two_deep == 2;
}

struct Csr5Lds {
    int rm_stride = 0;
    size_t x = 0, rm = 0;
};
static Csr5Lds csr5_lds(const Csr5Plan &P, size_t elem)
{
    Csr5Lds L;
    const int sigma = P.sigma == 4 || P.sigma == 8 ? P.sigma : 16;
    L.rm_stride = P.row_map ? (P.max_tile_rows < kWave ? kWave : (sigma + 1) * kWave) : 0;
    L.rm = (size_t) (kBlock / kWave) * L.rm_stride * sizeof(int);
    L.x = P.staged > 0 ? xwin_lds_bytes(P.maxspan, elem) : 0;
    return L;
}

static size_t sell_lds_bytes(const spmv_dev *d, size_t *xbytes_out)
{
    const int cpw = d->sell_group * (d->plan.sell_sigma / kSellC);
    const size_t xbytes = xwin_lds_bytes(d->sell_maxspan, d->vsize);
    if (xbytes_out) *xbytes_out = xbytes;
    return xbytes + d->vsize * (size_t) cpw * kSellC;
}

template <typename T, int SIGMA, bool MAPPED>
static void launch_csr5_form(spmv_dev *d, const Csr5Plan &P, const T *x, T *y)
{
    const Csr5Lds L = csr5_lds(P, sizeof(T));
    const int rm_stride = L.rm_stride;
    const size_t rmb = L.rm;
    if (P.staged > 0) {
        const size_t lds = L.x;
        if (P.natural) {
            constexpr size_t full = (size_t) (kBlock / kWave) * NatLds<T, SIGMA, false>::kBytes;
            const bool half = lds + rmb + full > 76 * 1024;
            if (half) {
                ensure_lds<nat_group_kernel<T, SIGMA, MAPPED, true>>(d->device, lds + rmb, (size_t) (kBlock / kWave) * NatLds<T, SIGMA, true>::kBytes);
                nat_group_kernel<T, SIGMA, MAPPED, true><<<P.groups, kBlock, lds + rmb, d->stream>>>(P.group_tiles, P.tiles, (int) P.nnz, P.tile_ptr, P.desc, P.col, P.col16,
                                                                                                    (const T *) P.val, P.row_map, P.wins, x, y, (T *) P.carry, P.n_empty, P.empty_list,
                                                                                                    (int) lds, rm_stride);
            } else {
                ensure_lds<nat_group_kernel<T, SIGMA, MAPPED, false>>(d->device, lds + rmb, full);
                nat_group_kernel<T, SIGMA, MAPPED, false><<<P.groups, kBlock, lds + rmb, d->stream>>>(P.group_tiles, P.tiles, (int) P.nnz, P.tile_ptr, P.desc, P.col, P.col16,
                                                                                                     (const T *) P.val, P.row_map, P.wins, x, y, (T *) P.carry, P.n_empty, P.empty_list,
                                                                                                     (int) lds, rm_stride);
            }
            return;
        }
        if (csr5_two_deep(d, P)) {
            ensure_lds<csr5_group_pipe_kernel<T, SIGMA, MAPPED>>(d->device, lds + rmb);
            csr5_group_pipe_kernel<T, SIGMA, MAPPED><<<P.groups, kBlock, lds + rmb, d->stream>>>(P.group_tiles, P.tiles, P.tile_ptr, P.desc, P.col16, (const T *) P.val, P.row_map, P.wins, P.lane_run,
                                                                                                x, y, (T *) P.carry, P.n_empty, P.empty_list, (int) lds, rm_stride);
            return;
        }
        ensure_lds<csr5_group_kernel<T, SIGMA, MAPPED>>(d->device, lds + rmb);
        csr5_group_kernel<T, SIGMA, MAPPED><<<P.groups, kBlock, lds + rmb, d->stream>>>(P.group_tiles, P.tiles, P.tile_ptr, P.desc, P.col, P.col16, (const T *) P.val, P.row_map, P.wins, P.lane_run,
                                                                                       x, y, (T *) P.carry, P.n_empty, P.empty_list, (int) lds, rm_stride);
        return;
    }
    const int grid = grid_for(P.tiles, kBlock / kWave, INT_MAX);
    const int xcd = d->plan.xcd_order ? 1 : 0;
    if (P.natural && P.forward) {
        const int long_blocks = (P.n_long + 7) & ~7;
        nat_kernel<T, SIGMA, MAPPED, true><<<grid + long_blocks, kBlock, rmb, d->stream>>>(P.tiles, (int) P.nnz, P.tile_ptr, P.desc, P.col, (const T *) P.val, P.row_map, x, y, (T *) P.carry,
                                                                                          P.n_empty, P.empty_list, rm_stride, xcd, P.fwd, P.long_list, P.n_long, long_blocks);
    } else if (P.natural)
        nat_kernel<T, SIGMA, MAPPED><<<grid, kBlock, rmb, d->stream>>>(P.tiles, (int) P.nnz, P.tile_ptr, P.desc, P.col, (const T *) P.val, P.row_map, x, y, (T *) P.carry, P.n_empty,
                                                                      P.empty_list, rm_stride, xcd);
    else
        csr5_kernel<T, SIGMA, MAPPED><<<grid, kBlock, rmb, d->stream>>>(P.tiles, P.tile_ptr, P.desc, P.col, (const T *) P.val, P.row_map, x, y, (T *) P.carry, P.n_empty, P.empty_list,
                                                                       rm_stride, xcd);
}

template <typename T, int SIGMA>
static void launch_csr5_sigma(spmv_dev *d, const Csr5Plan &P, const T *x, T *y)
{
    if (P.row_map) launch_csr5_form<T, SIGMA, true>(d, P, x, y);
    else launch_csr5_form<T, SIGMA, false>(d, P, x, y);
}
// ... 114 lines not shown
```

spmv_amd/csrc/shim/state.hpp:

```cpp
#pragma once

static thread_local char t_err[400] = "";

static int fail(int code, const char *fmt, ...)
{
    va_list ap;
    va_start(ap, fmt);
    vsnprintf(t_err, sizeof t_err, fmt, ap);
    va_end(ap);
    return code;
}

extern "C" const char *spmv_shim_error_text(void) { return t_err; }

#define HIP_TRY(expr)                                                                              \
    do {                                                                                           \
        hipError_t e__ = (expr);                                                                   \
        if (e__ != hipSuccess) {                                                                   \
            (void) hipGetLastError();                                                              \
            return fail(e__ == hipErrorOutOfMemory ? SPMV_HIP_E_ALLOC : SPMV_HIP_E_RUNTIME,        \
                        "%s -> %s", #expr, hipGetErrorString(e__));                                \
        }                                                                                          \
    } while (0)

// ... 92 lines not shown
        if (prev != device && hipSetDevice(device) != hipSuccess) { (void) hipGetLastError(); ok = false; }
        if (prev == device) prev = -1;
    }
    ~DeviceGuard() { if (prev >= 0) (void) hipSetDevice(prev); }
};

struct DevStats {
    int max_len, min_len, empty, bad, first, last;
    unsigned long long hist_rows[SPMV_LEN_BUCKETS], hist_nnz[SPMV_LEN_BUCKETS];
};

struct Csr5Plan {
    int sigma = 0, tiles = 0, m2 = 0, fixup = 0, groups = 0, staged = 0, maxspan = 0, group_tiles = kCsr5GroupTiles;
    long long nnz = 0;
    int max_tile_rows = 0;
    int n_empty = 0;
    const int *empty_list = nullptr;
    bool natural = false;
    TileWindows *wins = nullptr;
    int *tile_ptr = nullptr, *run_len = nullptr, *col = nullptr;
    unsigned short *col16 = nullptr;
    unsigned *lane_run = nullptr;
    int run_groups = 0;
    long long run_tiles = 0;
    const int *row_map = nullptr;
    unsigned *desc = nullptr;
    void *val = nullptr, *carry = nullptr;
    int forward = 0, n_long = 0;
    int *fwd = nullptr;
    int4 *long_list = nullptr;
};

struct BlkSet {
    int R = 0, K = 0, B = 0, wshift = kBlkSlabShift;
    int ge = 7;
    int form = 0;
    int waves = 1;
    bool ordered = true;
    bool subsort = true;
    float tune_ms[3] = {0, 0, 0};
    long long groups = 0;
    int *row0 = nullptr;
    long long *gstart = nullptr;
    BlkDir *dir = nullptr;
    int *order = nullptr;
    void *val = nullptr;
    unsigned *meta = nullptr;
    int *hdr = nullptr;
};

struct StageBuf { void *p = nullptr; size_t bytes = 0; };
enum { STAGE_X, STAGE_Y, STAGE_SPMM_X, STAGE_SPMM_Y, STAGE_SDDMM_U, STAGE_SDDMM_V, STAGE_SDDMM_O, STAGE_ROWRED_A, STAGE_ROWRED_G, STAGE_ROWRED_O,
       STAGE_ATT_Q, STAGE_ATT_K, STAGE_ATT_V, STAGE_ATT_O,
       STAGE_ATTB_Q, STAGE_ATTB_K, STAGE_ATTB_V, STAGE_ATTB_G, STAGE_ATTB_DQ, STAGE_ATTB_DK, STAGE_ATTB_DV,
       STAGE_ATT_B, STAGE_ATT_DB,
       STAGE_ATT_L,
       STAGE_ATTB_O, STAGE_ATTB_L,
       STAGE_MRG_O1, STAGE_MRG_L1, STAGE_MRG_O2, STAGE_MRG_L2, STAGE_MRG_O, STAGE_MRG_L,
       STAGE_CG_B, STAGE_CG_X, STAGE_CG_DINV,
       STAGE_CGC_B, STAGE_CGC_X,
       STAGE_COUNT };

struct spmv_dev {
    int device = 0;
    int cus = 256;
    hipStream_t stream = nullptr;
    int async = 0;
    int m = 0, n = 0;
    long long nnz = 0;
    size_t vsize = 8;
    int col_min = 0, col_max = -1;
    int *rowptr = nullptr, *colidx = nullptr;
    void *val = nullptr;
    spmv_stats stats{};
    spmv_plan plan{};
    bool built = false;
    int nblocks = 0, rb_stride = 0;
    int *rb_split = nullptr;
    int vt_tiles = 0, vt_staged = 0, vt_maxspan = 0, vec_choice = 0;
    int rows_depth = 0;
    bool vt_wide = false;
    int vt_rows = 256;
    float tune_ms[3] = {0, 0, 0};
    unsigned short *vt_col = nullptr;
    unsigned short *vt_rowslot = nullptr;
    int vt_run_tiles = 0, vt_run_nnz = 0, vt_run_rows = 0;
    unsigned char *vt_col8 = nullptr;
    int vt_byte_tiles = 0, vt_byte_nnz = 0, vt_byte_rows = 0;
    unsigned short *vt_tmpl = nullptr;
    unsigned char *vt_rowtid = nullptr;
    int vt_tmpl_tiles = 0, vt_tmpl_nnz = 0, vt_tmpl_rows = 0;
    TileWindows *vt_wins = nullptr;
    unsigned *pk_lo = nullptr;
    unsigned char *pk_hi = nullptr;
    int *pk_e = nullptr;
    unsigned long long *pk_cnt = nullptr;
    long long pk_tiles = 0, pk_nnz = 0;
    bool pk_use = false;
    int pk_depth = 0;
    float pack_ms[2] = {0, 0};
    int nlong = 0, long_thr = INT_MAX;
    int *long_rows = nullptr;
    long long *lr_seg_start = nullptr;
    int nchunks = 0;
    long long sell_cols = 0;
    int *perm = nullptr, *scol = nullptr;
    TileWindows *sell_wins = nullptr;
    unsigned *sell_run = nullptr;
    unsigned short *sell_tmpl = nullptr;
    long long sell_tmpl_nnz = 0;
    unsigned char *scol8 = nullptr;
    long long sell_byte_nnz = 0, sell_byte_stored = 0, sell_byte_slots = 0;
    int sell_run_groups = 0;
    long long sell_run_nnz = 0, sell_run_stored = 0, sell_run_slots = 0;
    unsigned short *scol16 = nullptr;
    int sell_nwin = 0, sell_staged = 0, sell_xcap = 0, sell_maxspan = 0, sell_group = 1;
    long long *chunk_ptr = nullptr;
    void *sval = nullptr;
    Csr5Plan c5, c5_long, ns;
    bool blk_on = false;
    BlkSet blk;
    int *lsub_rowptr = nullptr, *lsub_colidx = nullptr;
    void *lsub_val = nullptr;
    long long lsub_nnz = 0;
    StageBuf stage[STAGE_COUNT];
    void *scratch8 = nullptr;
    long long stream_bytes = 0, x_bytes = 0;
    int x_groups_seen = 0;
    float route_ms[2] = {0, 0};
    spmv_dev *sp_near = nullptr, *sp_far = nullptr;
    int *sp_centre = nullptr;
    int sp_half = 0;
    float near_share = -1.f;
    float split_ms[2] = {0, 0};
    bool accumulate = false;
    bool spmm_planned = false;
    int spmm_nb = 0, spmm_nlong = 0;
    int *spmm_split = nullptr, *spmm_longs = nullptr;
    bool att_planned = false;
    int *att_off = nullptr;
    void *att_park = nullptr;
    void *attb_p = nullptr, *attb_ds = nullptr;
    int attb_planes = 0;
    size_t attb_bytes = 0;
    StageBuf attb_nk, attb_nv;
    void *cg_ws = nullptr;
    StageBuf cg_hist;
    void *bicg_ws = nullptr;
    StageBuf bicg_hist;
    void *cgc_ws = nullptr;
    int cgc_k = 0;
    StageBuf cgc_hist;
    void *gmres_ws = nullptr;
    int gmres_restart = 0;
    StageBuf gmres_hist;
    spmv_dev *tr = nullptr;
    int *tr_perm = nullptr;
    size_t tr_perm_bytes = 0;
    unsigned long long val_gen = 0, tr_gen = 0;
    long long device_bytes = 0;
    double inspect_ms = 0;
    std::vector<std::pair<void *, size_t>> sched_allocs;
};

static int dev_alloc(spmv_dev *d, void **p, size_t bytes, bool sched)
{
    *p = nullptr;
    if (bytes == 0) bytes = 16;
    HIP_TRY(pool_malloc(p, bytes));
    d->device_bytes += (long long) bytes;
    if (sched) d->sched_allocs.push_back({*p, bytes});
    return SPMV_HIP_OK;
}
#define ALLOC_TRY(d, p, bytes, sched)                                        \
    do {                                                                     \
        int rc__ = dev_alloc((d), (void **) (p), (bytes), (sched));          \
        if (rc__) return rc__;                                               \
    } while (0)

static void sched_free(spmv_dev *d, void *p)
{
    for (size_t i = 0; i < d->sched_allocs.size(); ++i)
        if (d->sched_allocs[i].first == p) {
            d->device_bytes -= (long long) d->sched_allocs[i].second;
            d->sched_allocs.erase(d->sched_allocs.begin() + (long) i);
            (void) pool_free(p);
            return;
        }
}

static void reset_tile_fields(spmv_dev *d)
{
    d->rb_split = nullptr;
    d->perm = d->scol = d->long_rows = nullptr; d->sell_wins = nullptr; d->scol16 = nullptr; d->sell_run = nullptr; d->sell_tmpl = nullptr; d->sell_tmpl_nnz = 0; d->scol8 = nullptr; d->sell_byte_nnz = d->sell_byte_stored = d->sell_byte_slots = 0; d->sell_run_groups = 0; d->sell_run_nnz = d->sell_run_stored = d->sell_run_slots = 0; d->sell_staged = d->sell_nwin = 0; d->chunk_ptr = d->lr_seg_start = nullptr;
    d->sval = nullptr;
    d->nblocks = d->nchunks = d->nlong = 0;
    d->long_thr = INT_MAX;
    d->vt_col = nullptr; d->vt_wins = nullptr; d->vt_tiles = d->vt_staged = d->vt_maxspan = 0; d->vt_wide = false; d->vt_rows = 256;
    d->vt_rowslot = nullptr; d->vt_run_tiles = d->vt_run_nnz = d->vt_run_rows = 0; d->rows_depth = 0;
    d->vt_col8 = nullptr; d->vt_byte_tiles = d->vt_byte_nnz = d->vt_byte_rows = 0;
    d->vt_tmpl = nullptr; d->vt_rowtid = nullptr; d->vt_tmpl_tiles = d->vt_tmpl_nnz = d->vt_tmpl_rows = 0;
    d->pk_lo = nullptr; d->pk_hi = nullptr; d->pk_e = nullptr; d->pk_cnt = nullptr; d->pk_tiles = d->pk_nnz = 0; d->pk_use = false; d->pk_depth = 0; d->pack_ms[0] = d->pack_ms[1] = 0;
    d->c5 = Csr5Plan();
    d->c5_long = Csr5Plan();
    d->ns = Csr5Plan();
    d->lsub_rowptr = d->lsub_colidx = nullptr; d->lsub_val = nullptr; d->lsub_nnz = 0;
}

static void quiesce(spmv_dev *d)
{
    DeviceGuard guard(d->device);
    if (hipStreamSynchronize(d->stream) != hipSuccess) (void) hipGetLastError();
}

static void free_schedule(spmv_dev *d)
{
    if (!d->sched_allocs.empty()) quiesce(d);
    for (auto &a : d->sched_allocs) { (void) pool_free(a.first); d->device_bytes -= (long long) a.second; }
    d->sched_allocs.clear();
    reset_tile_fields(d);
    d->blk_on = false;
    d->blk = BlkSet();
    d->built = false;
}

static void drop_tile_schedule(spmv_dev *d, size_t count)
{
    quiesce(d);
    for (size_t i = 0; i < count && i < d->sched_allocs.size(); ++i) { (void) pool_free(d->sched_allocs[i].first); d->device_bytes -= (long long) d->sched_allocs[i].second; }
    d->sched_allocs.erase(d->sched_allocs.begin(), d->sched_allocs.begin() + (long) (count < d->sched_allocs.size() ? count : d->sched_allocs.size()));
    reset_tile_fields(d);
}

static bool is_device_ptr(const void *p)
{
    if (!p) return false;
    hipPointerAttribute_t a;
    memset(&a, 0, sizeof a);
    if (hipPointerGetAttributes(&a, p) != hipSuccess) {
        (void) hipGetLastError();
        return false;
    }
    return a.type == hipMemoryTypeDevice || a.type == hipMemoryTypeManaged;
}

struct Stager {
    static constexpr int kMaxRes = 4;
    struct Res { const StageBuf *buf; void *host; size_t ld, rows, k, es; };
    spmv_dev *d;
    bool all_dev = true;
    Res res[kMaxRes] = {};
    int nres = 0;

    int reserve(StageBuf &b, size_t bytes)
    {
        if (b.p && b.bytes >= bytes) return SPMV_HIP_OK;
        if (b.p) {
            quiesce(d);
            (void) pool_free(b.p);
            d->device_bytes -= (long long) b.bytes;
            b = StageBuf();
        }
        ALLOC_TRY(d, &b.p, bytes, false);
        b.bytes = bytes ? bytes : 16;
        return SPMV_HIP_OK;
    }
    hipError_t copy(void *dst, size_t dst_ld, const void *src, size_t src_ld, size_t rows, size_t k, hipMemcpyKind kind, size_t s)
    {
        if (dst_ld == k && src_ld == k) return hipMemcpyAsync(dst, src, s * k * rows, kind, d->stream);
        return hipMemcpy2DAsync(dst, s * dst_ld, src, s * src_ld, s * k, rows, kind, d->stream);
    }
    template <class P> int in(StageBuf &b, P &p, long long &ld, size_t rows, int k, size_t es = 0)
    {
        const bool dev = is_device_ptr(p);
        all_dev = all_dev && dev;
        if (dev || !p || rows == 0) return SPMV_HIP_OK;
        if (es == 0) es = d->vsize;
        const int rc = reserve(b, es * (size_t) k * rows);
        if (rc) return rc;
        HIP_TRY(copy(b.p, (size_t) k, p, (size_t) ld, rows, (size_t) k, hipMemcpyHostToDevice, es));
        p = (P) b.p;
// ... 155 lines not shown
```

spmv_amd/csrc/spmv_internal.h:

```cpp
#ifndef SPMV_INTERNAL_H
#define SPMV_INTERNAL_H
#include <stddef.h>
#include "spmv_Defines.h"
#include "spmv_shim.h"

enum {
    SPMV_OPT_LANES_PER_ROW, SPMV_OPT_SELL_C, SPMV_OPT_SELL_SIGMA, SPMV_OPT_SELL_LDS_X, SPMV_OPT_SELL_LONG_THR,
    SPMV_OPT_CSR5_SIGMA, SPMV_OPT_ROWBLOCK_NNZ, SPMV_OPT_CACHE_BLOCK, SPMV_OPT_SLAB_KIB, SPMV_OPT_BLOCK_ROWS,
    SPMV_OPT_VECTOR_FORM, SPMV_OPT_X_WINDOWS, SPMV_OPT_XCD_ORDER, SPMV_OPT_CSR5_TWO_DEEP, SPMV_OPT_RUN_TILES, SPMV_OPT_ROW_FORWARD, SPMV_OPT_AUTO_METHOD, SPMV_OPT_AUTOTUNE, SPMV_OPT_REORDER, SPMV_OPT_HOST_ROWS,
    SPMV_OPT_CHECK_VALUES, SPMV_OPT_GPUS, SPMV_OPT_X_EXCHANGE, SPMV_OPT_SPLIT,
    SPMV_OPT_KEEP_COLUMNS, SPMV_OPT_BLK_WAVES, SPMV_OPT_BLK_GROUPS, SPMV_OPT_BLK_SUBSORT, SPMV_OPT_DETERMINISTIC,
    SPMV_OPT_ATTENTION_BACKWARD_HEADS, SPMV_OPT_PACK_VALUES,
    SPMV_N_OPTS
};
typedef struct spmv_options { long v[SPMV_N_OPTS]; } spmv_options;
void spmv_options_snapshot(spmv_options *out);
long spmv_options_get(const spmv_options *o, const char *key);

typedef struct spmv_hip_state {
    spmv_dev *dev;
    struct spmv_multi *multi;
    int host_rows;
    SPMV_METHODS requested;
    spmv_plan plan;
    spmv_plan tplan;
    SPMV_METHODS tmethod;
    spmv_options opts;
    int m, n;
    void *stream;
    int stream_set, async, warned_rebuild;
    unsigned long long val_sum;
    int val_sum_valid;
    long long val_words;
    int from_blocks;
} spmv_hip_state;

void spmv_set_error(int code, const char *where, const char *what);

void spmv_plan_choose(SPMV_METHODS requested, const spmv_stats *st, size_t value_size, const spmv_options *opt,
                      spmv_plan *plan, SPMV_METHODS *actual, int allow_auto);

double spmv_host_dot_d(BASIC_INT_TYPE len, const BASIC_INT_TYPE *indx, const double *val, const double *x);
float spmv_host_dot_s(BASIC_INT_TYPE len, const BASIC_INT_TYPE *indx, const float *val, const float *x);
void spmv_host_rows(BASIC_INT_TYPE m, const BASIC_INT_TYPE *rowptr, const BASIC_INT_TYPE *colidx, const void *val,
                    size_t value_size, const void *x, void *y, int threads);

#endif
```

spmv_amd/csrc/spmv_plan.c:

```c
#include <ctype.h>
#include <pthread.h>
#include <stdio.h>
#include <stdlib.h>
#include <string.h>

#include "spmv_hip.h"
#include "spmv_internal.h"

typedef struct { const char *key; long value; long lo, hi; int pow2; int env_read; } opt_t;
static opt_t g_opts[SPMV_N_OPTS] = {
    [SPMV_OPT_LANES_PER_ROW] = {"lanes_per_row", 0, 0, 64, 1, 0},
    [SPMV_OPT_SELL_C] = {"sell_c", 64, 64, 64, 1, 0},
    [SPMV_OPT_SELL_SIGMA] = {"sell_sigma", 1024, 64, 1 << 20, 1, 0},
    [SPMV_OPT_SELL_LDS_X] = {"sell_lds_x", 1, 0, 1, 0, 0},
    [SPMV_OPT_SELL_LONG_THR] = {"sell_long_thr", 0, 0, 1 << 20, 0, 0},
    [SPMV_OPT_CSR5_SIGMA] = {"csr5_sigma", 0, 0, 16, 0, 0},
    [SPMV_OPT_ROWBLOCK_NNZ] = {"rowblock_nnz", 0, 0, 1 << 20, 0, 0},
    [SPMV_OPT_CACHE_BLOCK] = {"cache_block", 1, 0, 2, 0, 0},
    [SPMV_OPT_SLAB_KIB] = {"slab_kib", 0, 0, 1 << 16, 1, 0},
    [SPMV_OPT_BLOCK_ROWS] = {"block_rows", 0, 0, 16384, 1, 0},
    [SPMV_OPT_SPLIT] = {"split", 1, 0, 1, 0, 0},
    [SPMV_OPT_VECTOR_FORM] = {"vector_form", 0, 0, 12, 0, 0},
    [SPMV_OPT_X_WINDOWS] = {"x_windows", 1, 0, 1, 0, 0},
    [SPMV_OPT_XCD_ORDER] = {"xcd_order", 1, 0, 1, 0, 0},
    [SPMV_OPT_CSR5_TWO_DEEP] = {"csr5_two_deep", 0, 0, 2, 0, 0},
    [SPMV_OPT_RUN_TILES] = {"run_tiles", 1, 0, 1, 0, 0},
    [SPMV_OPT_ROW_FORWARD] = {"row_forward", 1, 0, 1, 0, 0},
    [SPMV_OPT_AUTO_METHOD] = {"auto_method", 0, 0, 2, 0, 0},
    [SPMV_OPT_AUTOTUNE] = {"autotune", 1, 0, 1, 0, 0},
    [SPMV_OPT_REORDER] = {"reorder", 0, 0, 2, 0, 0},
    [SPMV_OPT_HOST_ROWS] = {"host_rows", 0, 0, 1, 0, 0},
    [SPMV_OPT_CHECK_VALUES] = {"check_values", 2, 0, 2, 0, 0},
    [SPMV_OPT_GPUS] = {"gpus", 0, 0, 64, 0, 0},
    [SPMV_OPT_KEEP_COLUMNS] = {"keep_columns", 0, 0, 1, 0, 0},
    [SPMV_OPT_BLK_WAVES] = {"blk_waves", 0, 0, 8, 1, 0},
    [SPMV_OPT_BLK_GROUPS] = {"blk_groups", 0, 0, 12, 0, 0},
    [SPMV_OPT_BLK_SUBSORT] = {"blk_subsort", 1, 0, 1, 0, 0},
    [SPMV_OPT_DETERMINISTIC] = {"deterministic", 1, 0, 1, 0, 0},
    [SPMV_OPT_ATTENTION_BACKWARD_HEADS] = {"attention_backward_heads", 0, 0, 1024, 0, 0},
    [SPMV_OPT_PACK_VALUES] = {"pack_values", 2, 0, 2, 0, 0},
    [SPMV_OPT_X_EXCHANGE] = {"x_exchange", 0, 0, 2, 0, 0},
};

static pthread_mutex_t g_opt_lock = PTHREAD_MUTEX_INITIALIZER;
static _Thread_local long t_over[SPMV_N_OPTS];
static _Thread_local unsigned char t_over_set[SPMV_N_OPTS];

static int is_pow2_or_zero(long v) { return v == 0 || (v & (v - 1)) == 0; }
static int opt_legal(const opt_t *o, long v) { return v >= o->lo && v <= o->hi && (!o->pow2 || is_pow2_or_zero(v)); }

static int opt_find(const char *key)
{
    int i;
    if (!key) return -1;
    for (i = 0; i < SPMV_N_OPTS; ++i) {
        opt_t *o = &g_opts[i];
        if (strcmp(o->key, key) != 0) continue;
        if (!o->env_read) {
            char name[64] = "SPMV_HIP_";
            size_t k, off = strlen(name);
            const char *e;
            for (k = 0; key[k] && off + k + 1 < sizeof name; ++k) name[off + k] = (char) toupper((unsigned char) key[k]);
            name[off + k] = 0;
            e = getenv(name);
            if (e && *e) {
                long v = strtol(e, NULL, 10);
                if (opt_legal(o, v)) o->value = v;
            }
            o->env_read = 1;
        }
        return i;
    }
    return -1;
}

int spmv_hip_set_option(const char *key, long value)
{
    int i, rc = SPMV_HIP_OK;
    pthread_mutex_lock(&g_opt_lock);
    i = opt_find(key);
    if (i < 0 || !opt_legal(&g_opts[i], value)) rc = SPMV_HIP_E_ARG;
    else g_opts[i].value = value;
    pthread_mutex_unlock(&g_opt_lock);
    if (rc) spmv_set_error(rc, "set_option", key ? key : "(null)");
    return rc;
}

long spmv_hip_get_option(const char *key)
{
    long v = -1;
    int i;
    pthread_mutex_lock(&g_opt_lock);
    i = opt_find(key);
    if (i >= 0) v = t_over_set[i] ? t_over[i] : g_opts[i].value;
    pthread_mutex_unlock(&g_opt_lock);
    return v;
}

int spmv_hip_set_thread_option(const char *key, long value)
{
    int i, rc = SPMV_HIP_OK;
    pthread_mutex_lock(&g_opt_lock);
    i = opt_find(key);
    if (i < 0 || !opt_legal(&g_opts[i], value)) rc = SPMV_HIP_E_ARG;
    pthread_mutex_unlock(&g_opt_lock);
    if (rc) { spmv_set_error(rc, "set_thread_option", key ? key : "(null)"); return rc; }
    t_over[i] = value;
    t_over_set[i] = 1;
    return SPMV_HIP_OK;
}

void spmv_hip_clear_thread_options(void) { memset(t_over_set, 0, sizeof t_over_set); }

void spmv_options_snapshot(spmv_options *out)
{
    int i;
    pthread_mutex_lock(&g_opt_lock);
    for (i = 0; i < SPMV_N_OPTS; ++i) {
        (void) opt_find(g_opts[i].key);
        out->v[i] = t_over_set[i] ? t_over[i] : g_opts[i].value;
    }
    pthread_mutex_unlock(&g_opt_lock);
}
// ... 24 lines not shown
    const int NB = SPMV_LEN_BUCKETS;
    double best = -1.0;
    int L, best_l = pow2_at_least(st->mean_row_len / 4.0, 1, 64), best_thr = 0;
    long long rows_all = 0;
    int b;
    for (b = 0; b < NB; ++b) rows_all += st->hist_rows[b];
    *cost_out = -1.0;
    if (rows_all <= 0) { *lanes_out = best_l; *thr_out = 0; return; }
    for (L = 1; L <= 64; L <<= 1) {
        const int R = 64 / L;
        const int def_thr = L * 64 > 256 ? L * 64 : 256;
        int cand;
        for (cand = -1; cand < NB - 1; ++cand) {
            const int thr = cand < 0 ? def_thr : (4 << cand);
            long long rows_short = 0, cum = 0;
            double nnz_long = 0.0, e_max = 0.0, f_prev = 0.0, cost;
            int last_short = -1;
            if (cand >= 0 && (thr < 64 || thr < 4 * L || thr >= def_thr)) continue;
            for (b = 0; b < NB; ++b) {
                const int upper_ok = b < NB - 1 ? (4 << b) <= thr : st->max_row_len <= thr;
                if (upper_ok) { rows_short += st->hist_rows[b]; last_short = b; }
                else nnz_long += (double) st->hist_nnz[b];
            }
            for (b = 0; b <= last_short && rows_short > 0; ++b) {
                double mean_len, it, f;
                if (st->hist_rows[b] == 0) continue;
                cum += st->hist_rows[b];
                mean_len = (double) st->hist_nnz[b] / (double) st->hist_rows[b];
                it = (double) (long long) ((mean_len + 4.0 * L - 1.0) / (4.0 * L));
                if (it < 1.0) it = 1.0;
                f = pow_int((double) cum / (double) rows_short, R);
                e_max += (1.0 + 3.0 * (it - 1.0)) * (f - f_prev);
                f_prev = f;
            }
            cost = (double) rows_short / R * e_max + nnz_long / 256.0 * 1.1;
            if (best < 0.0 || cost < best * 0.98 || (cost <= best && L > best_l)) {
                best = cost;
                best_l = L;
                best_thr = cand < 0 ? 0 : thr;
            }
        }
    }
    *lanes_out = best_l;
    *thr_out = best_thr;
    *cost_out = best;
}

static int choose_sell_long_threshold(const spmv_stats *st, int sigma)
{
    const int NB = SPMV_LEN_BUCKETS;
    double best_cost = -1.0;
    int best_thr = 0, best_cand = SPMV_LEN_BUCKETS, cand, b;
    if (st->m <= 0 || st->nnz <= 0) return 0;
    for (cand = NB; cand >= 1; --cand) {
        double cost = 0.0;
        for (b = 0; b < NB; ++b) {
            const double rows = (double) st->hist_rows[b], nnz = (double) st->hist_nnz[b];
            if (rows <= 0.0) continue;
            if (b < cand) {
                double upper = b < NB - 1 ? (double) (4 << b) : (double) st->max_row_len;
                if (upper > (double) st->max_row_len) upper = (double) st->max_row_len;
                const double lower = b == 0 ? 0.0 : (double) (4 << (b - 1));
                const double per_window = rows * (double) sigma / (double) st->m;
                double span = (upper - lower) * (per_window >= 64.0 ? 64.0 / per_window : 1.0);
                if (per_window < 64.0) span += upper - nnz / rows;
                cost += nnz + rows * span * 0.5;
            } else {
                cost += nnz * 1.05;
            }
        }
        if (best_cost < 0.0 || cost < best_cost * 0.97) {
            best_cost = cost;
            best_cand = cand;
        }
    }
    while (best_cand < NB && best_cand > 1) {
        const double per_window = (double) st->hist_rows[best_cand - 1] * (double) sigma / (double) st->m;
        if (per_window > 0.0 && per_window < 64.0) --best_cand; else break;
    }
    best_thr = best_cand >= NB ? 0 : (4 << (best_cand - 1));
    return best_thr;
}

void spmv_plan_choose(SPMV_METHODS requested, const spmv_stats *st, size_t value_size, const spmv_options *opt,
                      spmv_plan *plan, SPMV_METHODS *actual, int allow_auto)
{
    long lanes = opt->v[SPMV_OPT_LANES_PER_ROW];
    long rb = opt->v[SPMV_OPT_ROWBLOCK_NNZ];
    double vector_cost = -1.0;
    memset(plan, 0, sizeof *plan);
    plan->vector_form = (int) opt->v[SPMV_OPT_VECTOR_FORM];
    plan->x_windows = (int) opt->v[SPMV_OPT_X_WINDOWS];
    plan->xcd_order = (int) opt->v[SPMV_OPT_XCD_ORDER];
    plan->csr5_two_deep = (int) opt->v[SPMV_OPT_CSR5_TWO_DEEP];
    plan->run_tiles = (int) opt->v[SPMV_OPT_RUN_TILES];
    plan->row_forward = (int) opt->v[SPMV_OPT_ROW_FORWARD];
    plan->pack_values = (int) opt->v[SPMV_OPT_PACK_VALUES];
    plan->forced = plan->vector_form != 0 || plan->x_windows != 1 || plan->xcd_order != 1 || plan->csr5_two_deep != 0 || plan->run_tiles != 1 || plan->row_forward != 1;
    plan->autotune = (int) opt->v[SPMV_OPT_AUTOTUNE];
    plan->sell_c = (int) opt->v[SPMV_OPT_SELL_C];
    plan->sell_sigma = (int) opt->v[SPMV_OPT_SELL_SIGMA];
    plan->sell_lds_x = (int) opt->v[SPMV_OPT_SELL_LDS_X];
    plan->sell_long_thr = (int) opt->v[SPMV_OPT_SELL_LONG_THR];
    plan->cache_block = (int) opt->v[SPMV_OPT_CACHE_BLOCK];
    plan->slab_kib = (int) opt->v[SPMV_OPT_SLAB_KIB];
    plan->block_rows = (int) opt->v[SPMV_OPT_BLOCK_ROWS];
    plan->blk_waves = (int) opt->v[SPMV_OPT_BLK_WAVES];
    plan->blk_groups = (int) opt->v[SPMV_OPT_BLK_GROUPS];
    plan->blk_subsort = (int) opt->v[SPMV_OPT_BLK_SUBSORT];
    plan->deterministic = (int) opt->v[SPMV_OPT_DETERMINISTIC];
    plan->csr5_sigma = (int) opt->v[SPMV_OPT_CSR5_SIGMA];
    if (rb > 0) plan->rowblock_nnz = (int) rb;
    else {
        double share = 256.0 * st->mean_row_len;
        if (share < 2048.0) share = 2048.0;
        if (share > 65536.0) share = 65536.0;
        plan->rowblock_nnz = (int) share;
    }
    if (lanes > 0) plan->lanes_per_row = (int) lanes;
    else choose_vector_shape(st, &plan->lanes_per_row, &plan->long_thr, &vector_cost);
    (void) value_size;
    if (allow_auto && opt->v[SPMV_OPT_AUTO_METHOD] >= 1 && st->m > 0) {
        const int regular = st->mean_row_len >= 4.0 && (double) st->max_row_len <= 4.0 * st->mean_row_len &&
                            (double) st->empty_rows <= 0.01 * (double) st->m;
        double slots = 0.0;
        const double chunk = 4.0 * plan->lanes_per_row;
        int b;
        for (b = 0; b < SPMV_LEN_BUCKETS; ++b)
            if (st->hist_rows[b] > 0) {
                const double mean_len = (double) st->hist_nnz[b] / (double) st->hist_rows[b];
                double passes = (double) (long long) ((mean_len + chunk - 1.0) / chunk);
                if (passes < 1.0) passes = 1.0;
                slots += (double) st->hist_rows[b] * passes * chunk;
            }
        requested = regular && (slots <= 0.0 || (double) st->nnz >= 0.9 * slots) ? Method_Parallel : Method_CSR5SPMV;
    }
    *actual = requested;
    switch (requested) {
    case Method_Parallel:
        plan->sched = SPMV_SCHED_CSR_VECTOR;
        break;
    case Method_Balanced:
    case Method_Balanced2: {
        int worker_share = plan->lanes_per_row * 64 > 256 ? plan->lanes_per_row * 64 : 256;
        if (worker_share > plan->rowblock_nnz) worker_share = plan->rowblock_nnz;
        if (st->max_row_len > worker_share) {
            *actual = Method_Balanced2;
            plan->sched = SPMV_SCHED_NNZ_SPLIT;
        } else {
            *actual = Method_Balanced;
            plan->sched = SPMV_SCHED_ROWBLOCK;
        }
        break;
    }
    case Method_Balanced_Yid:
        plan->sched = SPMV_SCHED_NNZ_SPLIT;
        break;
    case Method_SellCSigma:
        plan->sched = SPMV_SCHED_SELL;
        if (plan->sell_long_thr == 0) {
            const int t = choose_sell_long_threshold(st, plan->sell_sigma);
            double cap = 8.0 * st->mean_row_len;
            if (cap < 64.0) cap = 64.0;
            if (t > 0 && (double) t < cap) plan->sell_long_thr = t;
        }
        break;
    case Method_CSR5SPMV:
        plan->sched = SPMV_SCHED_CSR5;
        break;
    case Method_Serial:
    default:
        *actual = Method_Serial;
        plan->sched = SPMV_SCHED_CSR_SCALAR;
        break;
    }
    if ((plan->sched == SPMV_SCHED_CSR_VECTOR || plan->sched == SPMV_SCHED_SELL) && lanes == 0 && !plan->forced && vector_cost > 0.0 &&
        !(plan->sched == SPMV_SCHED_SELL && (opt->v[SPMV_OPT_SELL_SIGMA] != 1024 || opt->v[SPMV_OPT_SELL_LONG_THR] != 0 || opt->v[SPMV_OPT_SELL_LDS_X] != 1)) &&
        st->mean_row_len < 8.0 && (double) st->nnz / 256.0 * 1.1 < 0.5 * vector_cost)
        plan->sched = SPMV_SCHED_NNZ_SPLIT;
}
// ... 1 lines not shown
```

spmv_amd/csrc/spmv_shim.h:

```cpp
#ifndef SPMV_SHIM_H
#define SPMV_SHIM_H
#include <stddef.h>
#include "spmv_hip.h"

#if defined(__cplusplus)
extern "C" {
#endif

typedef struct spmv_dev spmv_dev;

enum spmv_sched {
    SPMV_SCHED_CSR_SCALAR = 0,
    SPMV_SCHED_CSR_VECTOR = 1,
    SPMV_SCHED_ROWBLOCK = 2,
    SPMV_SCHED_NNZ_SPLIT = 3,
    SPMV_SCHED_SELL = 4,
    SPMV_SCHED_CSR5 = 5,
    SPMV_SCHED_COUNT,
    SPMV_SCHED_HOST_ROWS = 100
};

#define SPMV_LEN_BUCKETS 11

typedef struct spmv_stats {
    int m, n;
    long long nnz;
    int max_row_len, min_row_len, empty_rows;
    double mean_row_len;
    long long hist_rows[SPMV_LEN_BUCKETS], hist_nnz[SPMV_LEN_BUCKETS];
} spmv_stats;

typedef struct spmv_plan {
    int sched;
    int lanes_per_row;
    int long_thr;
    int sell_c, sell_sigma, sell_lds_x, sell_long_thr;
    int csr5_sigma;
    int slab_kib, block_rows;
    int blk_waves, blk_groups, blk_subsort;
    int deterministic;
    int cache_block;
    int rowblock_nnz;
    int vector_form, x_windows, xcd_order, csr5_two_deep, run_tiles, row_forward;
    int pack_values;
    int forced;
    int autotune;
} spmv_plan;

int spmv_shim_device_count(void);
const char *spmv_shim_error_text(void);

int spmv_shim_matrix_create(spmv_dev **out, int m, int n, const int *rowptr, const int *colidx,
                            const void *val, size_t value_size);
int spmv_shim_matrix_stats(const spmv_dev *d, spmv_stats *out);
int spmv_shim_build(spmv_dev *d, const spmv_plan *plan);
int spmv_shim_run(spmv_dev *d, const void *x, void *y);
int spmv_shim_set_stream(spmv_dev *d, void *stream);
int spmv_shim_set_async(spmv_dev *d, int async);
int spmv_shim_sync(spmv_dev *d);
int spmv_shim_info(const spmv_dev *d, spmv_hip_info *out);
double spmv_shim_time(spmv_dev *d, const void *x, void *y, int warmup, int iters, float *ms_out);
double spmv_shim_time_self(spmv_dev *d, int iters);
void spmv_shim_matrix_destroy(spmv_dev *d);
int spmv_shim_copy_to_host(void *dst, const void *src, size_t bytes);
void spmv_shim_trim_pool(void);
int spmv_shim_is_device_ptr(const void *p);
int spmv_shim_release_columns(spmv_dev *d);
int spmv_shim_update_values(spmv_dev *d, const void *val);
int spmv_shim_checksum(spmv_dev *d, const void *val, unsigned long long *out);
int spmv_shim_checksum_words(const void *val, long long words, unsigned long long *out);

int spmv_shim_reorder_rcm(spmv_dev *d, int *perm_host);

int spmv_shim_spmm(spmv_dev *d, int k, const void *x, long long ldx, void *y, long long ldy);
double spmv_shim_time_spmm(spmv_dev *d, int k, const void *x, long long ldx, void *y, long long ldy, int warmup, int iters, float *ms_out);
int spmv_shim_restore_columns(spmv_dev *d, const int *rowptr, const int *colidx, const int *perm_host);

int spmv_shim_transpose(spmv_dev *d, spmv_dev **out, int **perm_out);
int spmv_shim_attach_transpose(spmv_dev *d, spmv_dev *child, int *perm);
spmv_dev *spmv_shim_transpose_of(const spmv_dev *d);
int spmv_shim_transpose_refresh(spmv_dev *d);
int spmv_shim_transpose_map(spmv_dev *d, int *rowptr_t, int *perm);
int spmv_shim_transpose_restore_columns(spmv_dev *d);

int spmv_shim_sddmm(spmv_dev *d, int k, const void *u, long long ldu, const void *v, long long ldv, void *out);
double spmv_shim_time_sddmm(spmv_dev *d, int k, const void *u, long long ldu, const void *v, long long ldv, void *out, int warmup, int iters, float *ms_out);

int spmv_shim_row_softmax(spmv_dev *d, const void *s, void *out);
int spmv_shim_row_softmax_backward(spmv_dev *d, const void *p, const void *g, void *out);
double spmv_shim_time_row_softmax(spmv_dev *d, const void *s, void *out, int warmup, int iters, float *ms_out);

typedef struct spmv_attention_call {
    int heads, kv_heads, k, dv;
    double scale;
    int io_type, o_type;
    const void *q;    long long ldq;
    const void *kk;   long long ldk;
    const void *v;    long long ldv;
    const void *bias; long long ldb;
    void *o;          long long ldo;
    void *lse;        long long ldl;
} spmv_attention_call;

typedef struct spmv_attention_backward_call {
    int heads, kv_heads, k, dv;
    int max_heads;
    double scale;
    int io_type, dq_type, dkv_type;
    const void *q;    long long ldq;
    const void *kk;   long long ldk;
    const void *v;    long long ldv;
    const void *bias; long long ldb;
    const void *g;    long long ldg;
    int stats;
    const void *o;    long long ldo;
    const void *lse;  long long ldl;
    void *dq;         long long lddq;
    void *dk;         long long lddk;
    void *dvo;        long long lddv;
    void *db;         long long lddb;
} spmv_attention_backward_call;

int spmv_shim_attention(spmv_dev *d, const spmv_attention_call *c);
double spmv_shim_time_attention(spmv_dev *d, const spmv_attention_call *c, int warmup, int iters, float *ms_out);
int spmv_shim_attention_merge(spmv_dev *d, int heads, int dv, const void *o1, long long ldo1, const void *l1, long long ldl1, const void *o2, long long ldo2, const void *l2,
                              long long ldl2, void *o, long long ldo, void *l, long long ldl);
double spmv_shim_time_attention_merge(spmv_dev *d, int heads, int dv, const void *o1, long long ldo1, const void *l1, long long ldl1, const void *o2, long long ldo2,
                                      const void *l2, long long ldl2, void *o, long long ldo, void *l, long long ldl, int warmup, int iters, float *ms_out);

int spmv_shim_attention_backward(spmv_dev *d, const spmv_attention_backward_call *c);
// ... 44 lines not shown
```

spmv_amd/csrc/spmv_shim.hip:

```cpp
#include <hip/hip_runtime.h>

#include <chrono>
#include <climits>
#include <cstdarg>
#include <cstdio>
#include <cstdlib>
#include <cstring>
#include <algorithm>
#include <mutex>
#include <vector>

#include "spmv_shim.h"
#include "kernels/common.hpp"
#include "kernels/csr_rows.hpp"
#include "kernels/csr_vector4.hpp"
#include "kernels/rowblock.hpp"
#include "kernels/sell.hpp"
#include "kernels/csr5.hpp"
#include "kernels/long_rows.hpp"
#include "kernels/blocked.hpp"
#include "kernels/split.hpp"
#include "kernels/rcm.hpp"
#include "kernels/csr_vector_tile.hpp"
#include "kernels/xwindows_inspect.hpp"
// ... 71 lines not shown

    if ((rc = dev_alloc(d, (void **) &d->rowptr, sizeof(int) * ((size_t) m + 1), false))) return bail(rc);
    if (m > 0) {
        if (hipMemcpy(d->rowptr, rowptr, sizeof(int) * ((size_t) m + 1), hipMemcpyDefault) != hipSuccess)
            return bail(fail(SPMV_HIP_E_RUNTIME, "copy RowPtr to HBM: %s", hipGetErrorString(hipGetLastError())));
    } else {
        (void) hipMemset(d->rowptr, 0, sizeof(int));
    }
    if ((rc = matrix_row_stats(d))) return bail(rc);
    if (d->nnz > 0 && (!colidx || !val)) return bail(fail(SPMV_HIP_E_ARG, "ColIdx / Matrix_Val is NULL"));

    if ((rc = dev_alloc(d, (void **) &d->colidx, sizeof(int) * ((size_t) d->nnz + kStreamPad), false))) return bail(rc);
    if ((rc = dev_alloc(d, &d->val, d->vsize * ((size_t) d->nnz + kStreamPad), false))) return bail(rc);
    (void) hipMemset(d->colidx + d->nnz, 0, sizeof(int) * kStreamPad);
    (void) hipMemset((char *) d->val + d->vsize * (size_t) d->nnz, 0, d->vsize * kStreamPad);
    if (d->nnz > 0) {
        if (hipMemcpy(d->colidx, colidx, sizeof(int) * (size_t) d->nnz, hipMemcpyDefault) != hipSuccess ||
            hipMemcpy(d->val, val, d->vsize * (size_t) d->nnz, hipMemcpyDefault) != hipSuccess)
            return bail(fail(SPMV_HIP_E_RUNTIME, "copy ColIdx/Val to HBM: %s", hipGetErrorString(hipGetLastError())));
        int host2[2] = {INT_MAX, INT_MIN};
        int *mnmx = nullptr;
        if (pool_malloc((void **) &mnmx, sizeof host2) != hipSuccess) return bail(fail(SPMV_HIP_E_ALLOC, "pool_malloc(colidx range)"));
        (void) hipMemcpy(mnmx, host2, sizeof host2, hipMemcpyHostToDevice);
        colidx_range_kernel<<<grid_for(d->nnz, kBlock * 16, d->cus * 8), kBlock>>>(d->nnz, d->colidx, mnmx);
        const hipError_t e2 = hipMemcpy(host2, mnmx, sizeof host2, hipMemcpyDeviceToHost);
        (void) pool_free(mnmx);
        if (e2 != hipSuccess) return bail(fail(SPMV_HIP_E_RUNTIME, "colidx range kernel: %s", hipGetErrorString(e2)));
        if (host2[0] < 0 || host2[1] >= n)
            return bail(fail(SPMV_HIP_E_ARG, "ColIdx out of range: min %d, max %d, n = %d", host2[0], host2[1], n));
        d->col_min = host2[0];
        d->col_max = host2[1];
    }
    *out = d;
    return SPMV_HIP_OK;
}

extern "C" void spmv_shim_matrix_arrays(const spmv_dev *d, const int **rowptr, const int **colidx, const void **val)
{
    if (rowptr) *rowptr = d ? d->rowptr : nullptr;
    if (colidx) *colidx = d ? d->colidx : nullptr;
    if (val) *val = d ? d->val : nullptr;
}

extern "C" int spmv_shim_copy_to_host(void *dst, const void *src, size_t bytes)
{
    if (bytes == 0) return SPMV_HIP_OK;
    if (!dst || !src) return fail(SPMV_HIP_E_ARG, "copy_to_host: NULL");
    HIP_TRY(hipMemcpy(dst, src, bytes, hipMemcpyDefault));
    return SPMV_HIP_OK;
}

extern "C" int spmv_shim_matrix_stats(const spmv_dev *d, spmv_stats *out)
{
    if (!d || !out) return fail(SPMV_HIP_E_ARG, "stats: NULL");
    *out = d->stats;
    return SPMV_HIP_OK;
}

extern "C" void spmv_shim_matrix_destroy(spmv_dev *d)
{
    if (!d) return;
    quiesce(d);
    if (d->sp_near) { spmv_shim_matrix_destroy(d->sp_near); d->sp_near = nullptr; }
    if (d->sp_far) { spmv_shim_matrix_destroy(d->sp_far); d->sp_far = nullptr; }
    if (d->sp_centre) { (void) pool_free(d->sp_centre); d->sp_centre = nullptr; }
    if (d->tr) { spmv_shim_matrix_destroy(d->tr); d->tr = nullptr; }
    if (d->tr_perm) { (void) pool_free(d->tr_perm); d->tr_perm = nullptr; }
    free_schedule(d);
    if (d->rowptr) (void) pool_free(d->rowptr);
    if (d->colidx) (void) pool_free(d->colidx);
    if (d->val) (void) pool_free(d->val);
    for (void *p : {d->scratch8, (void *) d->spmm_split, (void *) d->spmm_longs, (void *) d->att_off, d->att_park, d->attb_p, d->attb_ds, d->attb_nk.p, d->attb_nv.p, d->cg_ws, d->cg_hist.p, d->bicg_ws, d->bicg_hist.p, d->cgc_ws, d->cgc_hist.p, d->gmres_ws, d->gmres_hist.p}) if (p) (void) pool_free(p);
    for (StageBuf &b : d->stage) if (b.p) (void) pool_free(b.p);
    delete d;
}

#include "shim/inspect.hpp"

extern "C" int spmv_shim_build(spmv_dev *d, const spmv_plan *plan)
{
    if (!d || !plan) return fail(SPMV_HIP_E_ARG, "build: NULL");
    if (!d->colidx && d->nnz > 0) return fail(SPMV_HIP_E_NOSTATE, "build: the column indices of this matrix were released after create (option keep_columns = 1 keeps them)");
    if (plan->sched < 0 || plan->sched >= SPMV_SCHED_COUNT) return fail(SPMV_HIP_E_ARG, "unknown schedule %d", plan->sched);
    if (d->sp_near || d->sp_far) {
        if (d->sp_near) spmv_shim_matrix_destroy(d->sp_near);
        if (d->sp_far) spmv_shim_matrix_destroy(d->sp_far);
        d->sp_near = d->sp_far = nullptr;
    }
    free_schedule(d);
    d->plan = *plan;
    d->route_ms[0] = d->route_ms[1] = 0;
    d->split_ms[0] = d->split_ms[1] = 0;
    const auto t0 = std::chrono::steady_clock::now();
    int rc = SPMV_HIP_OK, staged = -1;
    const bool f64 = d->vsize == sizeof(double);
    DeviceGuard guard(d->device);
    if (!guard.ok) return fail(SPMV_HIP_E_RUNTIME, "hipSetDevice(%d) failed", d->device);
    int groups = 0;
    bool tiles = true;
    if (plan->sched != SPMV_SCHED_CSR_SCALAR && d->nnz > 0 && plan->x_windows &&
        ((plan->cache_block == 2 && blocked_possible(d)) || (plan->cache_block == 1 && blocked_size_ok(d) && !(plan->sched == SPMV_SCHED_SELL && !plan->sell_lds_x) && sample_says_no_locality(d))))
        tiles = false;
    auto build_tiles = [&]() -> int {
        int rc = SPMV_HIP_OK;
        switch (plan->sched) {
        case SPMV_SCHED_CSR_SCALAR: break;
        case SPMV_SCHED_CSR_VECTOR: {
            const int L = plan->lanes_per_row;
            if (L < 1 || L > 64 || (L & (L - 1))) return fail(SPMV_HIP_E_ARG, "lanes_per_row must be a power of two in [1, 64], got %d", L);
            const int thr = plan->long_thr > 0 ? plan->long_thr : (L * 64 > 256 ? L * 64 : 256);
            rc = f64 ? build_long_rows<double>(d, thr) : build_long_rows<float>(d, thr);
            if (!rc) rc = f64 ? build_vector_tiles<double>(d) : build_vector_tiles<float>(d);
            staged = d->vt_staged;
            groups = d->vt_tiles;
            if (!rc && plan->autotune && blocked_mode(d, staged, groups) != 1) {
                if (d->vt_wide) rc = f64 ? autotune_rows<double>(d) : autotune_rows<float>(d);
                else rc = f64 ? autotune_vector<double>(d) : autotune_vector<float>(d);
            }
            if (!rc && f64 && plan->pack_values && blocked_mode(d, staged, groups) != 1) rc = build_packed_values(d);
            break;
        }
        case SPMV_SCHED_NNZ_SPLIT:
            rc = f64 ? build_csr5<double>(d, d->ns, d->m, d->nnz, d->rowptr, d->colidx, (const double *) d->val, d->stats.empty_rows, d->stats.mean_row_len, nullptr, true)
                     : build_csr5<float>(d, d->ns, d->m, d->nnz, d->rowptr, d->colidx, (const float *) d->val, d->stats.empty_rows, d->stats.mean_row_len, nullptr, true);
            staged = d->ns.staged;
            groups = d->ns.groups;
            break;
        case SPMV_SCHED_ROWBLOCK:
            if (plan->rowblock_nnz < 64) return fail(SPMV_HIP_E_ARG, "rowblock_nnz must be >= 64");
            if (d->stats.max_row_len > plan->rowblock_nnz) return fail(SPMV_HIP_E_ARG, "row-block schedule needs max_row_len <= rowblock_nnz");
            rc = build_rowblock(d);
            if (!rc) rc = f64 ? build_rowblock_tiles<double>(d) : build_rowblock_tiles<float>(d);
            staged = d->vt_staged;
            groups = d->vt_tiles;
            if (!rc && plan->autotune && blocked_mode(d, staged, groups) != 1) rc = f64 ? autotune_rows<double>(d) : autotune_rows<float>(d);
            break;
        case SPMV_SCHED_SELL:
            rc = f64 ? build_sell<double>(d) : build_sell<float>(d);
            staged = d->plan.sell_lds_x ? d->sell_staged : -1;
            groups = d->sell_nwin;
            break;
        case SPMV_SCHED_CSR5:
            rc = f64 ? build_csr5<double>(d, d->c5, d->m, d->nnz, d->rowptr, d->colidx, (const double *) d->val, d->stats.empty_rows, d->stats.mean_row_len, nullptr)
                     : build_csr5<float>(d, d->c5, d->m, d->nnz, d->rowptr, d->colidx, (const float *) d->val, d->stats.empty_rows, d->stats.mean_row_len, nullptr);
            staged = d->c5.staged;
            groups = d->c5.groups;
            break;
        }
        return rc;
    };
    if (tiles) rc = build_tiles();
    auto blk_best = [](const BlkSet &b) { return b.tune_ms[1] > 0 && b.tune_ms[1] < b.tune_ms[0] ? b.tune_ms[1] : b.tune_ms[0]; };
    auto blk_release = [&](const BlkSet &b) {
        quiesce(d);
        for (void *p : {(void *) b.row0, (void *) b.gstart, (void *) b.dir, (void *) b.order, b.val, (void *) b.meta, (void *) b.hdr}) if (p) sched_free(d, p);
    };
    auto blk_build = [&](int rule, int waves, bool ordered) { return f64 ? build_blocked<double>(d, rule, waves, ordered) : build_blocked<float>(d, rule, waves, ordered); };
    auto blk_tune = [&]() { return f64 ? autotune_blocked<double>(d) : autotune_blocked<float>(d); };
    auto blk_try = [&](int rule, int waves, bool ordered) {
        const BlkSet first = d->blk;
        const float best0 = blk_best(first);
        d->blk_on = false;
        d->blk = BlkSet();
        const int rc2 = blk_build(rule, waves, ordered);
        if (!rc2 && d->blk_on) {
            (void) blk_tune();
            const float best1 = blk_best(d->blk);
            if (best1 > 0 && best1 < 0.97f * best0) blk_release(first);
            else { blk_release(d->blk); d->blk = first; }
        } else {
            blk_release(d->blk);
            d->blk = first;
            (void) hipGetLastError();
        }
        d->blk_on = true;
    };
    const int mode = !tiles ? 1 : (!rc && staged >= 0 ? blocked_mode(d, staged, groups) : 0);
    if (!rc && mode) {
        const size_t keep_from = d->sched_allocs.size();
        d->x_groups_seen = groups;
        double tile_ms = -1.0;
        if (mode == 2) tile_ms = f64 ? time_schedule<double>(d, 5) : time_schedule<float>(d, 5);
        const bool tiles_win_anyway = mode == 2 && tile_ms > 0 && plan->cache_block == 1 && tile_ms * 1e-3 * 5.5e12 <= (double) d->nnz * ((double) d->vsize + 4.0);
        if (tiles_win_anyway) d->route_ms[0] = (float) tile_ms;
        const int forced = plan->blk_waves;
        const bool can_try = plan->autotune && !plan->forced && plan->blk_groups == 0 && plan->block_rows == 0 && forced == 0 && d->nnz >= (1ll << 22);
        const double rows_one = std::min(9982.0, std::max(1.0, (double) d->m / (2.0 * (double) d->cus)));
        const double lambda_one = rows_one * ((double) d->nnz / (double) d->m) * (128.0 / (double) d->vsize) / (double) d->n;
        const bool wide_first = can_try && plan->deterministic != 0 && (long long) d->m >= 2048ll * d->cus && lambda_one < 1.0;
        int rcb = tiles_win_anyway ? SPMV_HIP_OK : blk_build(0, forced > 0 ? forced : (wide_first ? 2 : 1), plan->deterministic != 0);
        if (rcb && wide_first) {
            blk_release(d->blk);
            d->blk = BlkSet();
            d->blk_on = false;
            (void) hipGetLastError();
            rcb = blk_build(0, 1, true);
        }
        if (!rcb && d->blk_on) rcb = blk_tune();
        if (rcb) {
            blk_release(d->blk);
            d->blk = BlkSet();
            d->blk_on = false;
// ... 264 lines not shown
        if (x) (void) pool_free(x);
        fail(SPMV_HIP_E_ALLOC, "time_self: scratch vectors");
        return -1.0;
    }
    if (d->vsize == sizeof(double)) fill_value_kernel<double><<<grid_for(d->n, kBlock, d->cus * 8), kBlock, 0, d->stream>>>(d->n, (double *) x, 1.0);
    else fill_value_kernel<float><<<grid_for(d->n, kBlock, d->cus * 8), kBlock, 0, d->stream>>>(d->n, (float *) x, 1.0f);
    float ms[64];
    const double mean = spmv_shim_time(d, x, y, 2, iters, ms);
    (void) pool_free(x);
    (void) pool_free(y);
    if (mean < 0) return -1.0;
    float best = ms[0];
    for (int i = 1; i < iters; ++i) best = ms[i] < best ? ms[i] : best;
    return (double) best;
}

static const char *kSchedNames[] = {"csr-scalar", "csr-vector", "row-block", "nnz-split", "sell-c-sigma", "csr5"};
static const char *kKernelNames[] = {"csr_scalar_kernel", "csr_vector_pipe_kernel", "csr_vector_rows_kernel",
                                     "nat_kernel", "sell_kernel", "csr5_kernel"};
static const char *kVecKernelNames[] = {"csr_vector_pipe_kernel", "csr_vector_tile_kernel", "csr_vector_rows_kernel"};

static void append_name(char *buf, size_t cap, const char *name)
{
    const size_t n = strlen(buf);
    if (n + strlen(name) + 2 >= cap) return;
    if (n) strcat(buf, "+");
    strcat(buf, name);
}

static void csr5_kernel_names(const spmv_dev *d, const Csr5Plan &P, char *buf, size_t cap)
{
    if (P.nnz == 0) return;
    if (P.staged > 0) append_name(buf, cap, P.natural ? "nat_group_kernel" : (csr5_two_deep(d, P) ? "csr5_group_pipe_kernel" : "csr5_group_kernel"));
    else append_name(buf, cap, P.natural ? "nat_kernel" : "csr5_kernel");
    if (P.fixup && P.tiles > 1 && !P.forward) append_name(buf, cap, "csr5_fixup_kernel");
}

extern "C" int spmv_shim_info(const spmv_dev *d, spmv_hip_info *o)
{
    if (!d || !o) return fail(SPMV_HIP_E_ARG, "info: NULL");
    if (d->sp_near && d->sp_far) {
        const int rc = spmv_shim_info(d->sp_near, o);
        if (rc) return rc;
        spmv_hip_info f;
        (void) spmv_shim_info(d->sp_far, &f);
        const long long s = (long long) d->vsize;
        o->nnz = d->nnz;
        o->stored_nnz += f.stored_nnz;
        o->max_row_len = d->stats.max_row_len; o->min_row_len = d->stats.min_row_len; o->empty_rows = d->stats.empty_rows; o->mean_row_len = d->stats.mean_row_len;
        o->device_bytes = d->device_bytes + d->sp_near->device_bytes + d->sp_far->device_bytes + transpose_bytes(d);
        o->alg_bytes = 4ll * ((long long) d->m + 1) + d->nnz * (4 + s) + s * d->n + s * d->m;
        o->stream_bytes += f.stream_bytes;
        o->x_bytes += f.x_bytes;
        o->inspect_ms = d->inspect_ms;
        o->route_ms[0] = d->route_ms[0]; o->route_ms[1] = d->route_ms[1];
        o->split_ms[0] = d->split_ms[0]; o->split_ms[1] = d->split_ms[1];
        o->far_nnz = d->sp_far->nnz;
        o->packed_nnz += f.packed_nnz;
        o->blk_waves = f.blk_waves;
        o->reproducible = o->reproducible && f.reproducible;
        append_name(o->launch_kernels, sizeof o->launch_kernels, f.launch_kernels);
        return SPMV_HIP_OK;
    }
    memset(o, 0, sizeof *o);
    o->device = d->device;
    o->schedule = d->plan.sched;
    o->lanes_per_row = d->plan.sched == SPMV_SCHED_CSR_VECTOR ? d->plan.lanes_per_row : 0;
    o->sell_c = d->plan.sched == SPMV_SCHED_SELL ? kSellC : 0;
    o->sell_sigma = d->plan.sched == SPMV_SCHED_SELL ? d->plan.sell_sigma : 0;
    o->tile_nnz = d->plan.sched == SPMV_SCHED_NNZ_SPLIT ? kWave * d->ns.sigma : (d->plan.sched == SPMV_SCHED_ROWBLOCK ? d->rb_stride : (d->plan.sched == SPMV_SCHED_CSR5 ? kWave * d->c5.sigma : 0));
    o->m = d->m;
    o->n = d->n;
    o->nnz = d->nnz;
    o->stored_nnz = d->plan.sched == SPMV_SCHED_SELL ? d->sell_cols * kSellC : (d->plan.sched == SPMV_SCHED_CSR5 ? (long long) d->c5.tiles * kWave * d->c5.sigma : d->nnz);
    o->max_row_len = d->stats.max_row_len;
    o->min_row_len = d->stats.min_row_len;
    o->empty_rows = d->stats.empty_rows;
    o->mean_row_len = d->stats.mean_row_len;
    o->device_bytes = d->device_bytes + transpose_bytes(d);
    const long long s = (long long) d->vsize;
    o->alg_bytes = 4ll * ((long long) d->m + 1) + d->nnz * (4 + s) + s * d->n + s * d->m;
    o->inspect_ms = d->inspect_ms;
    o->tuned_choice = d->blk_on ? 100 + d->blk.form : d->vec_choice;
    if (!d->blk_on && d->rows_depth && (d->plan.sched == SPMV_SCHED_ROWBLOCK || (d->plan.sched == SPMV_SCHED_CSR_VECTOR && d->vt_wide))) o->tuned_choice = d->rows_depth == 2 ? VEC_TILE_D2 : VEC_TILE_D4;
    for (int k = 0; k < 3; ++k) o->tune_ms[k] = d->blk_on ? d->blk.tune_ms[k] : d->tune_ms[k];
    o->schedule_name = kSchedNames[d->plan.sched];
    o->kernel_name = kKernelNames[d->plan.sched];
    const int vec_kernel = vector_args(d).kernel;
    if (d->plan.sched == SPMV_SCHED_CSR_VECTOR) o->kernel_name = kVecKernelNames[vec_kernel];
    o->cache_blocked = d->blk_on ? 1 : 0;
    o->stream_bytes = d->stream_bytes;
    o->x_bytes = d->x_bytes;
    o->route_ms[0] = d->route_ms[0];
    o->route_ms[1] = d->route_ms[1];
    o->split_ms[0] = d->split_ms[0];
    o->split_ms[1] = d->split_ms[1];
    o->far_nnz = d->sp_far ? d->sp_far->nnz : 0;
    o->pack_ms[0] = d->pack_ms[0];
    o->pack_ms[1] = d->pack_ms[1];
    {
        const bool tiles_run = !d->blk_on && (d->plan.sched == SPMV_SCHED_CSR_VECTOR || d->plan.sched == SPMV_SCHED_ROWBLOCK) && vec_kernel != kVecPipeKernel;
        o->run_nnz = tiles_run ? d->vt_run_nnz : 0;
        o->byte_nnz = tiles_run ? d->vt_byte_nnz : 0;
        o->tmpl_nnz = tiles_run ? d->vt_tmpl_nnz : 0;
        o->packed_nnz = tiles_run && d->pk_use ? d->pk_nnz : 0;
        if (!d->blk_on && d->plan.sched == SPMV_SCHED_SELL && d->sell_staged > 0) { o->run_nnz = d->sell_run_nnz - d->sell_tmpl_nnz; o->tmpl_nnz = d->sell_tmpl_nnz; o->byte_nnz = d->sell_byte_nnz; }
        if (!d->blk_on && d->plan.sched == SPMV_SCHED_CSR5) o->run_nnz = d->c5.run_tiles * kWave * d->c5.sigma;
    }
    if (d->blk_on) { o->stored_nnz = d->blk.groups << d->blk.ge; o->x_groups = d->x_groups_seen; o->x_groups_staged = 0; }
    if (!d->blk_on) switch (d->plan.sched) {
    case SPMV_SCHED_CSR_VECTOR:
    case SPMV_SCHED_ROWBLOCK: o->x_groups = d->vt_tiles; o->x_groups_staged = d->vt_staged; break;
    case SPMV_SCHED_NNZ_SPLIT: o->x_groups = d->ns.groups; o->x_groups_staged = d->ns.staged; break;
    case SPMV_SCHED_SELL: o->x_groups = d->sell_nwin; o->x_groups_staged = d->sell_staged; break;
    case SPMV_SCHED_CSR5: o->x_groups = d->c5.groups; o->x_groups_staged = d->c5.staged; break;
    default: o->x_groups = o->x_groups_staged = 0; break;
    }
    o->blk_waves = d->blk_on ? d->blk.waves : 0;
    o->reproducible = d->blk_on && d->blk.waves > 1 && !d->blk.ordered ? 0 : 1;
    if (d->blk_on) o->kernel_name = d->blk.waves > 1 ? "blk_wide_kernel" : "blk_kernel";
    else if (d->plan.sched == SPMV_SCHED_NNZ_SPLIT)
        o->kernel_name = d->ns.staged > 0 ? "nat_group_kernel" : "nat_kernel";
    if (d->plan.sched == SPMV_SCHED_CSR5 && d->c5.staged > 0) o->kernel_name = csr5_two_deep(d, d->c5) ? "csr5_group_pipe_kernel" : "csr5_group_kernel";
    if (d->plan.sched == SPMV_SCHED_SELL && d->sell_staged > 0) o->kernel_name = "sell_window_kernel";
    if (d->blk_on) o->lds_bytes = d->nnz > 0 ? (int) blocked_lds_bytes(d->blk) : 0;
    else switch (d->nnz > 0 ? d->plan.sched : -1) {
    case SPMV_SCHED_CSR_VECTOR:
    case SPMV_SCHED_ROWBLOCK:
        if (vec_kernel != kVecPipeKernel) { o->x_span_max = d->vt_maxspan; o->lds_bytes = (int) xwin_lds_bytes(d->vt_maxspan, d->vsize); }
        break;
    case SPMV_SCHED_SELL:
        if (d->sell_staged > 0) { o->x_span_max = d->sell_maxspan; o->lds_bytes = (int) sell_lds_bytes(d, nullptr); }
        break;
    case SPMV_SCHED_NNZ_SPLIT:
    case SPMV_SCHED_CSR5: {
        const Csr5Plan &P = d->plan.sched == SPMV_SCHED_CSR5 ? d->c5 : d->ns;
        const Csr5Lds L = csr5_lds(P, d->vsize);
        o->x_span_max = P.staged > 0 ? P.maxspan : 0;
        o->lds_bytes = P.nnz > 0 ? (int) (L.x + L.rm) : 0;
        break;
    }
    default: break;
    }
    {
        char *b = o->launch_kernels;
        const size_t cap = sizeof o->launch_kernels;
        b[0] = 0;
        if (d->nnz == 0) { if (!d->accumulate && d->m > 0) append_name(b, cap, "fill_zero_kernel"); }
        else if (d->blk_on) append_name(b, cap, o->kernel_name);
        else switch (d->plan.sched) {
        case SPMV_SCHED_NNZ_SPLIT: csr5_kernel_names(d, d->ns, b, cap); break;
        case SPMV_SCHED_CSR5: csr5_kernel_names(d, d->c5, b, cap); break;
        case SPMV_SCHED_CSR_SCALAR: append_name(b, cap, o->kernel_name); break;
        default:
            append_name(b, cap, o->kernel_name);
            if (d->nlong > 0) csr5_kernel_names(d, d->c5_long, b, cap);
            break;
        }
    }
    return SPMV_HIP_OK;
}

#ifdef SPMV_BLK_DEBUG_FORMS
extern "C" int spmv_shim_debug_blk_times(unsigned long long *out)
{
    return hipMemcpyFromSymbol(out, HIP_SYMBOL(blk_dbg_times), sizeof(unsigned long long) * 4 * 8192) == hipSuccess ? 0 : 1;
}
#endif

#include "shim/reorder.hpp"
#include "shim/multi.hpp"
```

spmv_amd/csrc/spmv_vector.hip:

```cpp
#include <hip/hip_runtime.h>

#include "kernels/common.hpp"
#include "kernels/csr_vector4.hpp"
#include "kernels/xwindows.hpp"
#include "kernels/csr_vector_tile.hpp"

#ifndef SPMV_VEC_PART
#error "spmv_vector.hip is compiled with -DSPMV_VEC_PART=0..4"
#endif

namespace spmv {

template <typename T> static size_t vec_lds_bytes(const VecArgs &a) { return xwin_lds_bytes(a.maxspan, sizeof(T)); }

template <typename F>
static void with_lanes(int lanes, F f)
{
    switch (lanes) {
    case 1: f(std::integral_constant<int, 1>()); break;
    case 2: f(std::integral_constant<int, 2>()); break;
    case 4: f(std::integral_constant<int, 4>()); break;
    case 8: f(std::integral_constant<int, 8>()); break;
    case 16: f(std::integral_constant<int, 16>()); break;
    case 32: f(std::integral_constant<int, 32>()); break;
    default: f(std::integral_constant<int, 64>()); break;
    }
}

#if SPMV_VEC_PART < 2 || SPMV_VEC_PART == 4
constexpr int kVecNB = 4;

#if SPMV_VEC_PART == 4
template <int L, int DEPTH, bool PRE>
static void launch_tile_packed(const VecArgs &a, const double *x, double *y)
{
    const size_t lds = vec_lds_bytes<double>(a);
    ensure_lds<csr_vector_tile_kernel<double, L, DEPTH, PRE, true>>(a.device, lds);
    csr_vector_tile_kernel<double, L, DEPTH, PRE, true><<<a.tiles, kVecTileThreads, lds, a.stream>>>(a.m, a.long_thr, a.rowptr, a.colidx, a.col, (const double *) a.val, a.wins,
                                                                                                    a.rowslot, a.col8, a.tmpl, a.rowtid, x, y, a.pk_lo, a.pk_hi, a.pk_e);
}

hipError_t vector_launch_packed(const VecArgs &a, const double *x, double *y)
{
    with_lanes(a.lanes, [&](auto L) {
        constexpr int LL = decltype(L)::value;
        if (a.depth == 4) { if (a.pre) launch_tile_packed<LL, 4, true>(a, x, y); else launch_tile_packed<LL, 4, false>(a, x, y); }
        else { if (a.pre) launch_tile_packed<LL, 2, true>(a, x, y); else launch_tile_packed<LL, 2, false>(a, x, y); }
    });
    return hipPeekAtLastError();
}
#else
template <typename T, int L, int DEPTH, bool PRE>
static void launch_tile(const VecArgs &a, const T *x, T *y)
{
    const size_t lds = vec_lds_bytes<T>(a);
    ensure_lds<csr_vector_tile_kernel<T, L, DEPTH, PRE>>(a.device, lds);
    csr_vector_tile_kernel<T, L, DEPTH, PRE><<<a.tiles, kVecTileThreads, lds, a.stream>>>(a.m, a.long_thr, a.rowptr, a.colidx, a.col, (const T *) a.val, a.wins,
                                                                                          a.rowslot, a.col8, a.tmpl, a.rowtid, x, y);
}

template <typename T, int L>
static void launch_vector(const VecArgs &a, const T *x, T *y)
{
    if (a.kernel == kVecTileKernel) {
        if (a.depth == 8) launch_tile<T, L, 8, true>(a, x, y);
        else if (a.depth == 4) { if (a.pre) launch_tile<T, L, 4, true>(a, x, y); else launch_tile<T, L, 4, false>(a, x, y); }
        else { if (a.pre) launch_tile<T, L, 2, true>(a, x, y); else launch_tile<T, L, 2, false>(a, x, y); }
        return;
    }
    constexpr int rows = kBlock / L * kVecNB;
    csr_vector_pipe_kernel<T, L, kVecNB><<<grid_for(a.m, rows, INT_MAX), kBlock, 0, a.stream>>>(a.m, a.long_thr, a.rowptr, a.colidx, (const T *) a.val, x, y);
}

using Val = std::conditional<SPMV_VEC_PART == 0, double, float>::type;
hipError_t vector_launch(const VecArgs &a, const Val *x, Val *y)
{
#if SPMV_VEC_PART == 0
    if (a.kernel == kVecTileKernel && a.pk_e && a.depth != 8) return vector_launch_packed(a, x, y);
#endif
    with_lanes(a.lanes, [&](auto L) { launch_vector<Val, decltype(L)::value>(a, x, y); });
    return hipPeekAtLastError();
}
#endif
#else
template <typename T, int L, int DEPTH, bool WIDE>
static void launch_rows(const VecArgs &a, const T *x, T *y)
{
    const size_t lds = vec_lds_bytes<T>(a);
    ensure_lds<csr_vector_rows_kernel<T, L, DEPTH, WIDE>>(a.device, lds);
    csr_vector_rows_kernel<T, L, DEPTH, WIDE><<<a.tiles, kVecTileThreads, lds, a.stream>>>(a.long_thr, a.split, a.rows, a.m, a.rowptr, a.colidx, a.col, (const T *) a.val,
                                                                                          a.wins, a.rowslot, a.col8, a.tmpl, a.rowtid, x, y);
}

template <typename T, int L>
static void launch_rows_form(const VecArgs &a, const T *x, T *y)
{
    if (a.depth == 2) { if (a.wide) launch_rows<T, L, 2, true>(a, x, y); else launch_rows<T, L, 2, false>(a, x, y); }
    else { if (a.wide) launch_rows<T, L, 4, true>(a, x, y); else launch_rows<T, L, 4, false>(a, x, y); }
}

using Val = std::conditional<SPMV_VEC_PART == 2, double, float>::type;
hipError_t rows_launch(const VecArgs &a, const Val *x, Val *y)
{
    with_lanes(a.lanes, [&](auto L) { launch_rows_form<Val, decltype(L)::value>(a, x, y); });
    return hipPeekAtLastError();
}
#endif

}
```

Baseline: 1706.

## Add taller row tiles with window prediction and prefetch rows in uniform tile kernel

Adds an option and an automatic trial that rebuilds CSR vector tiles with 512 or 1024 rows per block when predicted x-window staging savings outweigh the cost, falling back when windows are lost. Uniform-block launches now use a rows kernel variant that preloads the next slab's rowptr/rowslot and issues the first column/value loads before the current slab is processed, overlapping latency. The intent is to cut redundant x staging across adjacent tiles and hide row-pointer load latency, at the cost of extra inspection work, register pressure and more template instantiations.

```diff
diff --git a/include/spmv_hip.h b/include/spmv_hip.h
--- a/include/spmv_hip.h
+++ b/include/spmv_hip.h
@@ -194,6 +194,9 @@
     int lds_bytes;
     long long packed_nnz;
     float pack_ms[2];
+    float tall_ms[2];
+    int tile_rows;
+    int tile_rows_fallback;
 } spmv_hip_info;
 int spmv_hip_get_info(spmv_Handle_t handle, spmv_hip_info *out);
 int spmv_hip_get_transpose_info(spmv_Handle_t handle, spmv_hip_info *out);
diff --git a/spmv_amd/api.py b/spmv_amd/api.py
--- a/spmv_amd/api.py
+++ b/spmv_amd/api.py
@@ -58,7 +58,8 @@
                 ("stream_bytes", C.c_longlong), ("x_bytes", C.c_longlong), ("route_ms", C.c_float * 2), ("split_ms", C.c_float * 2), ("far_nnz", C.c_longlong), ("run_nnz", C.c_longlong), ("byte_nnz", C.c_longlong), ("tmpl_nnz", C.c_longlong),
                 ("blk_waves", C.c_int), ("launch_kernels", C.c_char * 160), ("reproducible", C.c_int),
                 ("x_span_max", C.c_int), ("lds_bytes", C.c_int),
-                ("packed_nnz", C.c_longlong), ("pack_ms", C.c_float * 2)]
+                ("packed_nnz", C.c_longlong), ("pack_ms", C.c_float * 2),
+                ("tall_ms", C.c_float * 2), ("tile_rows", C.c_int), ("tile_rows_fallback", C.c_int)]
 
 
 class spmv_hip_cg_options(C.Structure):
@@ -320,6 +321,7 @@
     out["route_ms"] = [float(v) for v in out["route_ms"]]
     out["split_ms"] = [float(v) for v in out["split_ms"]]
     out["pack_ms"] = [float(v) for v in out["pack_ms"]]
+    out["tall_ms"] = [float(v) for v in out["tall_ms"]]
     return out
 
 
diff --git a/spmv_amd/csrc/kernels/csr_vector_tile.hpp b/spmv_amd/csrc/kernels/csr_vector_tile.hpp
--- a/spmv_amd/csrc/kernels/csr_vector_tile.hpp
+++ b/spmv_amd/csrc/kernels/csr_vector_tile.hpp
@@ -325,7 +325,7 @@
 #undef SPMV_TILE_WAVE
 }
 
-template <typename T, int L, int DEPTH = 4, bool WIDE = false>
+template <typename T, int L, int DEPTH = 4, bool WIDE = false, bool UNI = false>
 __global__ __launch_bounds__(kVecTileThreads) void csr_vector_rows_kernel(int long_thr, const int *__restrict__ split,
                                                                           int rows_per_block, int m,
                                                                           const int *__restrict__ rowptr,
@@ -350,28 +350,89 @@
     tile_rows(blockIdx.x, m, rows_per_block, split, r_begin, r_end);
     const TileWindows &tw = wins[blockIdx.x];
     const bool staged = tw.nwin > 0, runs = tw.runs == 1, bytes = tw.runs == 2, templ = tw.runs == 3;
+    if constexpr (!UNI) {
+        if (templ) for (int i = threadIdx.x; i < kTmplCount * kTmplMax; i += kVecTileThreads) tm_lds[i] = tmpl[(size_t) blockIdx.x * (kTmplCount * kTmplMax) + i];
+        stage_windows<kVecTileThreads, T>(tw, x, xs);
+        if (threadIdx.x == 0) xs[tw.total] = T(0);
+        __syncthreads();
+        const unsigned zoff = WIDE ? (unsigned) tw.total : (unsigned) tw.total * (unsigned) sizeof(T);
+        const int c0[4] = {0, 0, 0, 0};
+        const T v0[4] = {T(0), T(0), T(0), T(0)};
+        for (long long rw0 = r_begin + (long long) wave * kWave; rw0 < r_end; rw0 += kVecTileRows) {
+            long long r = rw0 + lane, re = rw0 + kWave;
+            if (r > r_end) r = r_end;
+            if (re > r_end) re = r_end;
+            rp_lds[wave][lane] = rowptr[r];
+            if (lane == 0) rp_lds[wave][kWave] = rowptr[re];
+            if (runs | bytes) rs_lds[wave][lane] = row_slot[r];
+            if (templ) rs_lds[wave][lane] = (unsigned) row_slot[r] | ((unsigned) row_tid[r] * kTmplMax << 16);
+            wave_lds_sync();
+            if (runs) csr_vector_tile_wave<T, L, 2, DEPTH, false, SHIFT>(r_end, long_thr, rw0, lane, rp_lds[wave], rs_lds[wave], y_lds[wave], colidx, col_local, val, x, xs, zoff, y, c0, v0);
+            else if (bytes) csr_vector_tile_wave<T, L, 3, DEPTH, false, SHIFT>(r_end, long_thr, rw0, lane, rp_lds[wave], rs_lds[wave], y_lds[wave], colidx, col_local, val, x, xs, zoff, y, c0, v0, col8);
+            else if (templ) csr_vector_tile_wave<T, L, 4, DEPTH, false, SHIFT>(r_end, long_thr, rw0, lane, rp_lds[wave], rs_lds[wave], y_lds[wave], colidx, col_local, val, x, xs, zoff, y, c0, v0, col8, tm_lds);
+            else if (staged) csr_vector_tile_wave<T, L, 1, DEPTH, false, SHIFT>(r_end, long_thr, rw0, lane, rp_lds[wave], rs_lds[wave], y_lds[wave], colidx, col_local, val, x, xs, zoff, y, c0, v0);
+            else csr_vector_tile_wave<T, L, 0, DEPTH, false, SHIFT>(r_end, long_thr, rw0, lane, rp_lds[wave], rs_lds[wave], y_lds[wave], colidx, col_local, val, x, xs, zoff, y, c0, v0);
+            wave_lds_sync();
+        }
+    } else {
+    struct SlabRows { int rp = 0, rpe = 0; unsigned rs = 0; };
+    auto load_rows = [&](long long rw0) {
+        SlabRows s;
+        long long r = rw0 + lane, re = rw0 + kWave;
+        if (r > r_end) r = r_end;
+        if (re > r_end) re = r_end;
+        s.rp = rowptr[r];
+        s.rpe = rowptr[re];
+        if (runs | bytes) s.rs = row_slot[r];
+        if (templ) s.rs = (unsigned) row_slot[r] | ((unsigned) row_tid[r] * kTmplMax << 16);
+        return s;
+    };
+    auto issue_step0 = [&](int rp, int (&c)[4], T (&v)[4]) {
+        const int sub = lane / L, l = lane % L;
+        const int a = __shfl(rp, sub, kWave) & ~3;
+        if (runs | templ) {}
+        else if (bytes) Lane4<T, L>::load_col8(col8, a, l, c);
+        else if (staged) Lane4<T, L>::load_col16(col_local, a, l, c);
+        else Lane4<T, L>::load_col32(colidx, a, l, c);
+        Lane4<T, L>::load_val(val, a, l, v);
+    };
+    long long rw0 = r_begin + (long long) wave * kWave;
+    SlabRows cur, nxt;
+    int c0[4] = {0, 0, 0, 0};
+    T v0[4] = {T(0), T(0), T(0), T(0)};
+    if (rw0 < r_end) {
+        cur = load_rows(rw0);
+        issue_step0(cur.rp, c0, v0);
+        if (rw0 + kVecTileRows < r_end) nxt = load_rows(rw0 + kVecTileRows);
+    }
     if (templ) for (int i = threadIdx.x; i < kTmplCount * kTmplMax; i += kVecTileThreads) tm_lds[i] = tmpl[(size_t) blockIdx.x * (kTmplCount * kTmplMax) + i];
     stage_windows<kVecTileThreads, T>(tw, x, xs);
     if (threadIdx.x == 0) xs[tw.total] = T(0);
     __syncthreads();
     const unsigned zoff = WIDE ? (unsigned) tw.total : (unsigned) tw.total * (unsigned) sizeof(T);
-    const int c0[4] = {0, 0, 0, 0};
-    const T v0[4] = {T(0), T(0), T(0), T(0)};
-    for (long long rw0 = r_begin + (long long) wave * kWave; rw0 < r_end; rw0 += kVecTileRows) {
-        long long r = rw0 + lane, re = rw0 + kWave;
-        if (r > r_end) r = r_end;
-        if (re > r_end) re = r_end;
-        rp_lds[wave][lane] = rowptr[r];
-        if (lane == 0) rp_lds[wave][kWave] = rowptr[re];
-        if (runs | bytes) rs_lds[wave][lane] = row_slot[r];
-        if (templ) rs_lds[wave][lane] = (unsigned) row_slot[r] | ((unsigned) row_tid[r] * kTmplMax << 16);
+    for (; rw0 < r_end; rw0 += kVecTileRows) {
+        rp_lds[wave][lane] = cur.rp;
+        if (lane == 0) rp_lds[wave][kWave] = cur.rpe;
+        if (runs | bytes | templ) rs_lds[wave][lane] = cur.rs;
         wave_lds_sync();
-        if (runs) csr_vector_tile_wave<T, L, 2, DEPTH, false, SHIFT>(r_end, long_thr, rw0, lane, rp_lds[wave], rs_lds[wave], y_lds[wave], colidx, col_local, val, x, xs, zoff, y, c0, v0);
-        else if (bytes) csr_vector_tile_wave<T, L, 3, DEPTH, false, SHIFT>(r_end, long_thr, rw0, lane, rp_lds[wave], rs_lds[wave], y_lds[wave], colidx, col_local, val, x, xs, zoff, y, c0, v0, col8);
-        else if (templ) csr_vector_tile_wave<T, L, 4, DEPTH, false, SHIFT>(r_end, long_thr, rw0, lane, rp_lds[wave], rs_lds[wave], y_lds[wave], colidx, col_local, val, x, xs, zoff, y, c0, v0, col8, tm_lds);
-        else if (staged) csr_vector_tile_wave<T, L, 1, DEPTH, false, SHIFT>(r_end, long_thr, rw0, lane, rp_lds[wave], rs_lds[wave], y_lds[wave], colidx, col_local, val, x, xs, zoff, y, c0, v0);
-        else csr_vector_tile_wave<T, L, 0, DEPTH, false, SHIFT>(r_end, long_thr, rw0, lane, rp_lds[wave], rs_lds[wave], y_lds[wave], colidx, col_local, val, x, xs, zoff, y, c0, v0);
+        SlabRows nxt2;
+        int cn[4] = {0, 0, 0, 0};
+        T vn[4] = {T(0), T(0), T(0), T(0)};
+        if (rw0 + kVecTileRows < r_end) {
+            issue_step0(nxt.rp, cn, vn);
+            if (rw0 + 2 * kVecTileRows < r_end) nxt2 = load_rows(rw0 + 2 * kVecTileRows);
+        }
+        if (runs) csr_vector_tile_wave<T, L, 2, DEPTH, true, SHIFT>(r_end, long_thr, rw0, lane, rp_lds[wave], rs_lds[wave], y_lds[wave], colidx, col_local, val, x, xs, zoff, y, c0, v0);
+        else if (bytes) csr_vector_tile_wave<T, L, 3, DEPTH, true, SHIFT>(r_end, long_thr, rw0, lane, rp_lds[wave], rs_lds[wave], y_lds[wave], colidx, col_local, val, x, xs, zoff, y, c0, v0, col8);
+        else if (templ) csr_vector_tile_wave<T, L, 4, DEPTH, true, SHIFT>(r_end, long_thr, rw0, lane, rp_lds[wave], rs_lds[wave], y_lds[wave], colidx, col_local, val, x, xs, zoff, y, c0, v0, col8, tm_lds);
+        else if (staged) csr_vector_tile_wave<T, L, 1, DEPTH, true, SHIFT>(r_end, long_thr, rw0, lane, rp_lds[wave], rs_lds[wave], y_lds[wave], colidx, col_local, val, x, xs, zoff, y, c0, v0);
+        else csr_vector_tile_wave<T, L, 0, DEPTH, true, SHIFT>(r_end, long_thr, rw0, lane, rp_lds[wave], rs_lds[wave], y_lds[wave], colidx, col_local, val, x, xs, zoff, y, c0, v0);
         wave_lds_sync();
+        cur = nxt;
+        nxt = nxt2;
+#pragma unroll
+        for (int k = 0; k < 4; ++k) { c0[k] = cn[k]; v0[k] = vn[k]; }
+    }
     }
 }
 
diff --git a/spmv_amd/csrc/kernels/xwindows_inspect.hpp b/spmv_amd/csrc/kernels/xwindows_inspect.hpp
--- a/spmv_amd/csrc/kernels/xwindows_inspect.hpp
+++ b/spmv_amd/csrc/kernels/xwindows_inspect.hpp
@@ -212,6 +212,71 @@
     build_windows(n, max_cols, loop, store, wins[blockIdx.x], staged, rewrite != 0);
 }
 
+static __global__ __launch_bounds__(kBlock) void tall_windows_predict_kernel(int blocks, int ratio, int tiles, int n, int cap48, int cap96,
+                                                                      const TileWindows *__restrict__ wins, unsigned long long *__restrict__ out)
+{
+    constexpr int kMaxIv = 4 * kWinMax;
+    const long long b = (long long) blockIdx.x * kBlock + threadIdx.x;
+    if (b >= blocks || ratio > 4) return;
+    int st[kMaxIv], en[kMaxIv], k = 0;
+    long long narrow = 0, lo = LLONG_MAX, hi = -1;
+    for (int t = 0; t < ratio; ++t) {
+        const long long tile = b * ratio + t;
+        if (tile >= tiles) break;
+        const TileWindows &w = wins[tile];
+        if (w.nwin <= 0) return;
+        narrow += w.total;
+        for (int i = 0; i < w.nwin && k < kMaxIv; ++i) {
+            const int s = w.start[i], e = s + w.len[i];
+            lo = s < lo ? s : lo;
+            hi = e > hi ? e : hi;
+            int ea = (e + (1 << kWinSegShift) - 1) & ~((1 << kWinSegShift) - 1);
+            st[k] = s & ~((1 << kWinSegShift) - 1);
+            en[k] = ea > n ? n : ea;
+            ++k;
+        }
+    }
+    if (k == 0) return;
+    for (int i = 1; i < k; ++i) {
+        const int s = st[i], e = en[i];
+        int j = i - 1;
+        for (; j >= 0 && st[j] > s; --j) { st[j + 1] = st[j]; en[j + 1] = en[j]; }
+        st[j + 1] = s; en[j + 1] = e;
+    }
+    long long total = 0;
+    int runs = 0, cur_s = st[0], cur_e = en[0];
+    for (int i = 1; i < k; ++i) {
+        if (st[i] <= cur_e) { cur_e = en[i] > cur_e ? en[i] : cur_e; continue; }
+        total += cur_e - cur_s; ++runs;
+        cur_s = st[i]; cur_e = en[i];
+    }
+    total += cur_e - cur_s; ++runs;
+    const bool analysed = hi - lo <= (long long) kWinBitmapWords * 32 << kWinSegShift;
+    auto fits = [&](int cap, long long &elems) {
+        if (hi - lo <= cap) { elems = hi - lo; return true; }
+        elems = total;
+        return analysed && runs <= kWinMax && total <= cap;
+    };
+    long long e48 = 0, e96 = 0;
+    const bool f48 = fits(cap48, e48), f96 = f48 || fits(cap96, e96);
+    atomicAdd(out + 0, 1ull);
+    atomicAdd(out + 3, (unsigned long long) narrow);
+    if (f48) atomicAdd(out + 1, 1ull);
+    if (f96) { atomicAdd(out + 2, 1ull); atomicAdd(out + 4, (unsigned long long) (f48 ? e48 : e96)); }
+}
+
+static __global__ __launch_bounds__(kBlock) void tall_windows_lost_kernel(int blocks, int ratio, int tiles, const TileWindows *__restrict__ narrow,
+                                                                   const TileWindows *__restrict__ tall, int *__restrict__ lost)
+{
+    const long long b = (long long) blockIdx.x * kBlock + threadIdx.x;
+    if (b >= blocks || tall[b].nwin > 0) return;
+    for (int t = 0; t < ratio; ++t) {
+        const long long tile = b * ratio + t;
+        if (tile < tiles && narrow[tile].nwin <= 0) return;
+    }
+    atomicAdd(lost, 1);
+}
+
 static __global__ __launch_bounds__(kBlock) void wins_total_kernel(int count, const TileWindows *__restrict__ wins, unsigned long long *__restrict__ sum,
                                                             unsigned long long *__restrict__ staged_tiles)
 {
diff --git a/spmv_amd/csrc/shim/inspect.hpp b/spmv_amd/csrc/shim/inspect.hpp
--- a/spmv_amd/csrc/shim/inspect.hpp
+++ b/spmv_amd/csrc/shim/inspect.hpp
@@ -40,6 +40,8 @@
 template <typename T> static int build_tile_windows(spmv_dev *d, int tiles, const int *split, int rows_per_tile = kVecTileRows, bool wide = false);
 static int wins_sum(spmv_dev *d, const TileWindows *wins, int count, long long *elems, long long *tiles);
 constexpr size_t kVecWideXTileBytes = 96 * 1024;
+template <typename T> static int try_tall_blocks(spmv_dev *d);
+static bool vt_uniform_blocks(const spmv_dev *d) { return d->vt_wide || d->vt_rows > kVecTileRows; }
 
 static int build_rowblock(spmv_dev *d)
 {
@@ -188,7 +190,7 @@
     d->vt_tiles = (int) (((long long) d->m + rows - 1) / rows);
     if (d->vt_tiles == 0 || d->nnz == 0) return SPMV_HIP_OK;
     int rc = build_tile_windows<T>(d, d->vt_tiles, nullptr, rows);
-    if (rc || d->plan.forced) return rc;
+    if (rc || d->plan.forced || d->plan.tile_rows == kVecTileRows) return rc;
     if (d->vt_staged * 2 >= d->vt_tiles) {
         long long welems = 0, wtiles = 0;
         const long long stream = (d->nnz - d->lsub_nnz) * ((long long) sizeof(T) + 2);
@@ -884,7 +886,7 @@
             long long welems = 0, wtiles = 0;
             rc = wins_sum(d, d->vt_wins, d->vt_tiles, &welems, &wtiles);
             if (rc) return rc;
-            const bool tile_form = d->vt_tiles > 0 && (d->plan.sched == SPMV_SCHED_ROWBLOCK || d->vt_wide || d->vt_staged * 2 >= d->vt_tiles);
+            const bool tile_form = d->vt_tiles > 0 && (d->plan.sched == SPMV_SCHED_ROWBLOCK || vt_uniform_blocks(d) || d->vt_staged * 2 >= d->vt_tiles);
             const double fs = tile_form && d->vt_tiles > 0 ? (double) wtiles / (double) d->vt_tiles : 0.0;
             t.bytes = 4 * (m + 1) + stream_part(d->nnz - d->lsub_nnz, s, fs) + s * (m - d->nlong);
             if (tile_form) { t.bytes += (long long) sizeof(TileWindows) * d->vt_tiles; t.x_elems = welems; }
diff --git a/spmv_amd/csrc/shim/launch.hpp b/spmv_amd/csrc/shim/launch.hpp
--- a/spmv_amd/csrc/shim/launch.hpp
+++ b/spmv_amd/csrc/shim/launch.hpp
@@ -6,7 +6,7 @@
 {
     VecArgs a;
     const bool f64 = d->vsize == sizeof(double);
-    if (d->plan.sched == SPMV_SCHED_ROWBLOCK || d->vt_wide) {
+    if (d->plan.sched == SPMV_SCHED_ROWBLOCK || vt_uniform_blocks(d)) {
         const int v = d->plan.vector_form;
         a.kernel = kVecRowsKernel;
         a.depth = d->rows_depth ? d->rows_depth : (f64 ? 4 : 2);
@@ -47,7 +47,7 @@
 {
     d->vec_choice = VEC_AUTO;
     if (d->nnz < (1ll << 24) || d->plan.forced || d->vt_tiles <= 0) return SPMV_HIP_OK;
-    if (d->vt_wide || d->vt_staged * 2 < d->vt_tiles) return SPMV_HIP_OK;
+    if (vt_uniform_blocks(d) || d->vt_staged * 2 < d->vt_tiles) return SPMV_HIP_OK;
     T *x = nullptr, *y = nullptr;
     if (pool_malloc((void **) &x, sizeof(T) * (size_t) d->n) != hipSuccess || pool_malloc((void **) &y, sizeof(T) * (size_t) d->m) != hipSuccess) {
         (void) hipGetLastError();
@@ -105,7 +105,7 @@
 {
     const int mode = d->plan.pack_values;
     d->pack_ms[0] = d->pack_ms[1] = 0;
-    if (mode == 0 || d->vsize != sizeof(double) || d->plan.sched != SPMV_SCHED_CSR_VECTOR || d->vt_wide || d->vt_tiles <= 0 || d->nnz == 0) return SPMV_HIP_OK;
+    if (mode == 0 || d->vsize != sizeof(double) || d->plan.sched != SPMV_SCHED_CSR_VECTOR || vt_uniform_blocks(d) || d->vt_tiles <= 0 || d->nnz == 0) return SPMV_HIP_OK;
     const VecArgs plain = vector_args(d);
     if (plain.kernel != kVecTileKernel || plain.depth == 8) return SPMV_HIP_OK;
     const bool timed = d->vec_choice != VEC_AUTO;
@@ -298,6 +298,174 @@
     return SPMV_HIP_OK;
 }
 
+struct VtSet {
+    TileWindows *wins = nullptr;
+    unsigned short *col = nullptr, *rowslot = nullptr, *tmpl = nullptr;
+    unsigned char *col8 = nullptr, *rowtid = nullptr;
+    int tiles = 0, staged = 0, maxspan = 0, rows = kVecTileRows;
+    bool wide = false;
+    int run[3] = {0, 0, 0}, byte[3] = {0, 0, 0}, tm[3] = {0, 0, 0};
+};
+static VtSet vt_take(spmv_dev *d)
+{
+    VtSet s;
+    s.wins = d->vt_wins; s.col = d->vt_col; s.rowslot = d->vt_rowslot; s.tmpl = d->vt_tmpl; s.col8 = d->vt_col8; s.rowtid = d->vt_rowtid;
+    s.tiles = d->vt_tiles; s.staged = d->vt_staged; s.maxspan = d->vt_maxspan; s.rows = d->vt_rows; s.wide = d->vt_wide;
+    s.run[0] = d->vt_run_tiles; s.run[1] = d->vt_run_nnz; s.run[2] = d->vt_run_rows;
+    s.byte[0] = d->vt_byte_tiles; s.byte[1] = d->vt_byte_nnz; s.byte[2] = d->vt_byte_rows;
+    s.tm[0] = d->vt_tmpl_tiles; s.tm[1] = d->vt_tmpl_nnz; s.tm[2] = d->vt_tmpl_rows;
+    d->vt_wins = nullptr; d->vt_col = nullptr; d->vt_rowslot = nullptr; d->vt_tmpl = nullptr; d->vt_col8 = nullptr; d->vt_rowtid = nullptr;
+    return s;
+}
+static void vt_put(spmv_dev *d, const VtSet &s)
+{
+    d->vt_wins = s.wins; d->vt_col = s.col; d->vt_rowslot = s.rowslot; d->vt_tmpl = s.tmpl; d->vt_col8 = s.col8; d->vt_rowtid = s.rowtid;
+    d->vt_tiles = s.tiles; d->vt_staged = s.staged; d->vt_maxspan = s.maxspan; d->vt_rows = s.rows; d->vt_wide = s.wide;
+    d->vt_run_tiles = s.run[0]; d->vt_run_nnz = s.run[1]; d->vt_run_rows = s.run[2];
+    d->vt_byte_tiles = s.byte[0]; d->vt_byte_nnz = s.byte[1]; d->vt_byte_rows = s.byte[2];
+    d->vt_tmpl_tiles = s.tm[0]; d->vt_tmpl_nnz = s.tm[1]; d->vt_tmpl_rows = s.tm[2];
+}
+static void vt_free(spmv_dev *d, const VtSet &s)
+{
+    quiesce(d);
+    for (void *p : {(void *) s.wins, (void *) s.col, (void *) s.rowslot, (void *) s.tmpl, (void *) s.col8, (void *) s.rowtid}) if (p) sched_free(d, p);
+}
+
+template <typename T>
+static int tall_candidates(spmv_dev *d, int (&height)[2], bool (&wide)[2])
+{
+    long long welems = 0, wtiles = 0;
+    if (wins_sum(d, d->vt_wins, d->vt_tiles, &welems, &wtiles) != SPMV_HIP_OK || account_stream_bytes(d) != SPMV_HIP_OK) return 0;
+    unsigned long long *dv = nullptr, hv[5];
+    if (pool_malloc((void **) &dv, sizeof hv) != hipSuccess) { (void) hipGetLastError(); return 0; }
+    int found = 0;
+    for (int H = 4 * kVecTileRows; H > kVecTileRows; H /= 2) {
+        const int ratio = H / kVecTileRows, blocks = (d->vt_tiles + ratio - 1) / ratio;
+        hipError_t e = hipMemsetAsync(dv, 0, sizeof hv, d->stream);
+        tall_windows_predict_kernel<<<grid_for(blocks, kBlock, INT_MAX), kBlock, 0, d->stream>>>(blocks, ratio, d->vt_tiles, d->n, (int) (kVecXTileBytes / sizeof(T)) - 1,
+                                                                                               (int) (kVecWideXTileBytes / sizeof(T)) - 1, d->vt_wins, dv);
+        if (e == hipSuccess) e = hipGetLastError();
+        if (e == hipSuccess) e = hipMemcpyAsync(hv, dv, sizeof hv, hipMemcpyDeviceToHost, d->stream);
+        if (e == hipSuccess) e = hipStreamSynchronize(d->stream);
+        if (e != hipSuccess) { (void) hipGetLastError(); break; }
+        if (hv[0] == 0 || hv[2] != hv[0]) continue;
+        const long long tall_elems = welems - (long long) hv[3] + (long long) hv[4];
+        if (!spmv_plan_tall_blocks_pay(welems, tall_elems, d->n, (long long) sizeof(T), d->stream_bytes)) continue;
+        height[found] = H;
+        wide[found++] = hv[1] != hv[0];
+    }
+    (void) pool_free(dv);
+    return found;
+}
+
+template <typename T>
+static int try_tall_blocks(spmv_dev *d)
+{
+    d->tall_ms[0] = d->tall_ms[1] = 0;
+    d->tall_fallback = false;
+    const int want = d->plan.tile_rows;
+    if (want == kVecTileRows || d->plan.sched != SPMV_SCHED_CSR_VECTOR || d->vt_tiles <= 0 || d->nnz == 0) return SPMV_HIP_OK;
+    if (vt_uniform_blocks(d)) return SPMV_HIP_OK;
+    if (d->vt_staged * 2 < d->vt_tiles || vector_args(d).kernel != kVecTileKernel) { d->tall_fallback = want != 0; return SPMV_HIP_OK; }
+    const bool timed = want == 0;
+    if (timed && (d->nnz < (1ll << 24) || !d->plan.autotune || d->plan.forced || d->vec_choice == VEC_AUTO)) return SPMV_HIP_OK;
+    int height[2] = {want, 0};
+    bool wide[2] = {false, false};
+    const int ncand = timed ? tall_candidates<T>(d, height, wide) : 1;
+    if (ncand == 0) return SPMV_HIP_OK;
+    const VtSet narrow = vt_take(d);
+    auto build = [&](int H, bool wide_only) {
+        const int ratio = H / kVecTileRows, blocks = (int) (((long long) d->m + H - 1) / H);
+        for (int attempt = wide_only ? 1 : 0; attempt < 2; ++attempt) {
+            int lost = -1, *dl = nullptr;
+            const int rc = build_tile_windows<T>(d, blocks, nullptr, H, attempt == 1);
+            if (!rc && pool_malloc((void **) &dl, sizeof(int)) == hipSuccess) {
+                hipError_t e = hipMemsetAsync(dl, 0, sizeof(int), d->stream);
+                tall_windows_lost_kernel<<<grid_for(blocks, kBlock, INT_MAX), kBlock, 0, d->stream>>>(blocks, ratio, narrow.tiles, narrow.wins, d->vt_wins, dl);
+                if (e == hipSuccess) e = hipGetLastError();
+                if (e == hipSuccess) e = hipMemcpyAsync(&lost, dl, sizeof(int), hipMemcpyDeviceToHost, d->stream);
+                if (e == hipSuccess) e = hipStreamSynchronize(d->stream);
+                if (e != hipSuccess) lost = -1;
+                (void) pool_free(dl);
+            }
+            if (!rc && lost == 0) return true;
+            const VtSet t = vt_take(d);
+            vt_free(d, t);
+            (void) hipGetLastError();
+        }
+        return false;
+    };
+    if (!timed) {
+        if (!build(want, false)) { vt_put(d, narrow); d->tall_fallback = true; return SPMV_HIP_OK; }
+        vt_free(d, narrow);
+        free_packed_values(d);
+        return d->plan.autotune ? autotune_rows<T>(d) : SPMV_HIP_OK;
+    }
+    T *x = nullptr, *y = nullptr;
+    if (pool_malloc((void **) &x, sizeof(T) * (size_t) d->n) != hipSuccess || pool_malloc((void **) &y, sizeof(T) * (size_t) d->m) != hipSuccess) {
+        (void) hipGetLastError();
+        if (x) (void) pool_free(x);
+        vt_put(d, narrow);
+        return SPMV_HIP_OK;
+    }
+    fill_value_kernel<T><<<grid_for(d->n, kBlock, d->cus * 8), kBlock, 0, d->stream>>>(d->n, x, T(1));
+    hipEvent_t e0, e1;
+    (void) hipEventCreate(&e0);
+    (void) hipEventCreate(&e1);
+    constexpr int kForm = 3;
+    const int depth[kForm] = {0, 4, 2};
+    VtSet best;
+    float best_ms = 1e30f, best_d4 = 0, best_d2 = 0, narrow_ms = 1e30f;
+    int best_depth = 0;
+    for (int c = 0; c < ncand; ++c) {
+        if (!build(height[c], wide[c])) continue;
+        const VtSet tall = vt_take(d);
+        float tmin[kForm] = {1e30f, 1e30f, 1e30f};
+        auto set = [&](int k) { vt_put(d, k ? tall : narrow); d->rows_depth = depth[k]; };
+        for (int k = 0; k < kForm; ++k) { set(k); (void) launch_vector<T>(d, x, y); }
+        for (int round = 0; round < 3; ++round)
+            for (int k = 0; k < kForm; ++k) {
+                set(k);
+                (void) hipEventRecord(e0, d->stream);
+                (void) launch_vector<T>(d, x, y);
+                (void) hipEventRecord(e1, d->stream);
+                (void) hipEventSynchronize(e1);
+                float ms = 0;
+                (void) hipEventElapsedTime(&ms, e0, e1);
+                if (ms < tmin[k]) tmin[k] = ms;
+            }
+        (void) vt_take(d);
+        if (tmin[0] < narrow_ms) narrow_ms = tmin[0];
+        const int k = tmin[2] < tmin[1] ? 2 : 1;
+        if (tmin[k] < best_ms) {
+            if (best.wins) vt_free(d, best);
+            best = tall; best_ms = tmin[k]; best_depth = depth[k]; best_d4 = tmin[1]; best_d2 = tmin[2];
+        } else vt_free(d, tall);
+    }
+    (void) hipEventDestroy(e0);
+    (void) hipEventDestroy(e1);
+    (void) pool_free(x);
+    (void) pool_free(y);
+    d->rows_depth = 0;
+    if (!best.wins) { vt_put(d, narrow); (void) hipGetLastError(); return SPMV_HIP_OK; }
+    float bar = narrow_ms;
+    if (d->pk_use) { if (d->pack_ms[1] > 0 && d->pack_ms[1] < bar) bar = d->pack_ms[1]; }
+    else for (int k = 0; k < 2; ++k) if (d->tune_ms[k] > 0 && d->tune_ms[k] < bar) bar = d->tune_ms[k];
+    d->tall_ms[0] = bar;
+    d->tall_ms[1] = best_ms;
+    if (hipGetLastError() != hipSuccess || !(best_ms < 0.95f * bar)) {
+        vt_put(d, narrow);
+        vt_free(d, best);
+        return SPMV_HIP_OK;
+    }
+    vt_put(d, best);
+    d->rows_depth = best_depth;
+    d->tune_ms[0] = best_d4; d->tune_ms[1] = best_d2; d->tune_ms[2] = 0;
+    vt_free(d, narrow);
+    free_packed_values(d);
+    return SPMV_HIP_OK;
+}
+
 static bool csr5_two_deep(const spmv_dev *d, const Csr5Plan &P)
 {
     if (P.natural || P.staged <= 0 || P.staged != P.groups || P.group_tiles > kCsr5PipeMaxGroupTiles || d->plan.csr5_two_deep == 1) return false;
diff --git a/spmv_amd/csrc/shim/state.hpp b/spmv_amd/csrc/shim/state.hpp
--- a/spmv_amd/csrc/shim/state.hpp
+++ b/spmv_amd/csrc/shim/state.hpp
@@ -198,6 +198,8 @@
     bool vt_wide = false;
     int vt_rows = 256;
     float tune_ms[3] = {0, 0, 0};
+    float tall_ms[2] = {0, 0};
+    bool tall_fallback = false;
     unsigned short *vt_col = nullptr;
     unsigned short *vt_rowslot = nullptr;
     int vt_run_tiles = 0, vt_run_nnz = 0, vt_run_rows = 0;
@@ -312,7 +314,7 @@
     d->sval = nullptr;
     d->nblocks = d->nchunks = d->nlong = 0;
     d->long_thr = INT_MAX;
-    d->vt_col = nullptr; d->vt_wins = nullptr; d->vt_tiles = d->vt_staged = d->vt_maxspan = 0; d->vt_wide = false; d->vt_rows = 256;
+    d->vt_col = nullptr; d->vt_wins = nullptr; d->vt_tiles = d->vt_staged = d->vt_maxspan = 0; d->vt_wide = false; d->vt_rows = 256; d->tall_ms[0] = d->tall_ms[1] = 0; d->tall_fallback = false;
     d->vt_rowslot = nullptr; d->vt_run_tiles = d->vt_run_nnz = d->vt_run_rows = 0; d->rows_depth = 0;
     d->vt_col8 = nullptr; d->vt_byte_tiles = d->vt_byte_nnz = d->vt_byte_rows = 0;
     d->vt_tmpl = nullptr; d->vt_rowtid = nullptr; d->vt_tmpl_tiles = d->vt_tmpl_nnz = d->vt_tmpl_rows = 0;
diff --git a/spmv_amd/csrc/spmv_internal.h b/spmv_amd/csrc/spmv_internal.h
--- a/spmv_amd/csrc/spmv_internal.h
+++ b/spmv_amd/csrc/spmv_internal.h
@@ -10,7 +10,7 @@
     SPMV_OPT_VECTOR_FORM, SPMV_OPT_X_WINDOWS, SPMV_OPT_XCD_ORDER, SPMV_OPT_CSR5_TWO_DEEP, SPMV_OPT_RUN_TILES, SPMV_OPT_ROW_FORWARD, SPMV_OPT_AUTO_METHOD, SPMV_OPT_AUTOTUNE, SPMV_OPT_REORDER, SPMV_OPT_HOST_ROWS,
     SPMV_OPT_CHECK_VALUES, SPMV_OPT_GPUS, SPMV_OPT_X_EXCHANGE, SPMV_OPT_SPLIT,
     SPMV_OPT_KEEP_COLUMNS, SPMV_OPT_BLK_WAVES, SPMV_OPT_BLK_GROUPS, SPMV_OPT_BLK_SUBSORT, SPMV_OPT_DETERMINISTIC,
-    SPMV_OPT_ATTENTION_BACKWARD_HEADS, SPMV_OPT_PACK_VALUES,
+    SPMV_OPT_ATTENTION_BACKWARD_HEADS, SPMV_OPT_PACK_VALUES, SPMV_OPT_TILE_ROWS,
     SPMV_N_OPTS
 };
 typedef struct spmv_options { long v[SPMV_N_OPTS]; } spmv_options;
diff --git a/spmv_amd/csrc/spmv_plan.c b/spmv_amd/csrc/spmv_plan.c
--- a/spmv_amd/csrc/spmv_plan.c
+++ b/spmv_amd/csrc/spmv_plan.c
@@ -39,6 +39,7 @@
     [SPMV_OPT_DETERMINISTIC] = {"deterministic", 1, 0, 1, 0, 0},
     [SPMV_OPT_ATTENTION_BACKWARD_HEADS] = {"attention_backward_heads", 0, 0, 1024, 0, 0},
     [SPMV_OPT_PACK_VALUES] = {"pack_values", 2, 0, 2, 0, 0},
+    [SPMV_OPT_TILE_ROWS] = {"tile_rows", 0, 0, 1024, 1, 0},
     [SPMV_OPT_X_EXCHANGE] = {"x_exchange", 0, 0, 2, 0, 0},
 };
 
@@ -229,6 +230,14 @@
     return best_thr;
 }
 
+int spmv_plan_tall_blocks_pay(long long narrow_elems, long long tall_elems, long long n, long long vsize, long long narrow_bytes)
+{
+    const long long cap = 8 * n;
+    const long long a = narrow_elems < cap ? narrow_elems : cap, b = tall_elems < cap ? tall_elems : cap;
+    if (narrow_bytes <= 0 || vsize <= 0 || b >= a) return 0;
+    return (a - b) * vsize * 20 >= narrow_bytes ? 1 : 0;
+}
+
 void spmv_plan_choose(SPMV_METHODS requested, const spmv_stats *st, size_t value_size, const spmv_options *opt,
                       spmv_plan *plan, SPMV_METHODS *actual, int allow_auto)
 {
@@ -243,6 +252,7 @@
     plan->run_tiles = (int) opt->v[SPMV_OPT_RUN_TILES];
     plan->row_forward = (int) opt->v[SPMV_OPT_ROW_FORWARD];
     plan->pack_values = (int) opt->v[SPMV_OPT_PACK_VALUES];
+    plan->tile_rows = (int) opt->v[SPMV_OPT_TILE_ROWS];
     plan->forced = plan->vector_form != 0 || plan->x_windows != 1 || plan->xcd_order != 1 || plan->csr5_two_deep != 0 || plan->run_tiles != 1 || plan->row_forward != 1;
     plan->autotune = (int) opt->v[SPMV_OPT_AUTOTUNE];
     plan->sell_c = (int) opt->v[SPMV_OPT_SELL_C];
diff --git a/spmv_amd/csrc/spmv_shim.h b/spmv_amd/csrc/spmv_shim.h
--- a/spmv_amd/csrc/spmv_shim.h
+++ b/spmv_amd/csrc/spmv_shim.h
@@ -43,9 +43,12 @@
     int rowblock_nnz;
     int vector_form, x_windows, xcd_order, csr5_two_deep, run_tiles, row_forward;
     int pack_values;
+    int tile_rows;
     int forced;
     int autotune;
 } spmv_plan;
+
+int spmv_plan_tall_blocks_pay(long long narrow_elems, long long tall_elems, long long n, long long vsize, long long narrow_bytes);
 
 int spmv_shim_device_count(void);
 const char *spmv_shim_error_text(void);
diff --git a/spmv_amd/csrc/spmv_shim.hip b/spmv_amd/csrc/spmv_shim.hip
--- a/spmv_amd/csrc/spmv_shim.hip
+++ b/spmv_amd/csrc/spmv_shim.hip
@@ -177,6 +177,7 @@
     if (!d || !plan) return fail(SPMV_HIP_E_ARG, "build: NULL");
     if (!d->colidx && d->nnz > 0) return fail(SPMV_HIP_E_NOSTATE, "build: the column indices of this matrix were released after create (option keep_columns = 1 keeps them)");
     if (plan->sched < 0 || plan->sched >= SPMV_SCHED_COUNT) return fail(SPMV_HIP_E_ARG, "unknown schedule %d", plan->sched);
+    if (plan->tile_rows != 0 && plan->tile_rows != 256 && plan->tile_rows != 512 && plan->tile_rows != 1024) return fail(SPMV_HIP_E_ARG, "tile_rows must be 0, 256, 512 or 1024, got %d", plan->tile_rows);
     if (d->sp_near || d->sp_far) {
         if (d->sp_near) spmv_shim_matrix_destroy(d->sp_near);
         if (d->sp_far) spmv_shim_matrix_destroy(d->sp_far);
@@ -213,6 +214,11 @@
                 else rc = f64 ? autotune_vector<double>(d) : autotune_vector<float>(d);
             }
             if (!rc && f64 && plan->pack_values && blocked_mode(d, staged, groups) != 1) rc = build_packed_values(d);
+            if (!rc && blocked_mode(d, staged, groups) != 1) {
+                rc = f64 ? try_tall_blocks<double>(d) : try_tall_blocks<float>(d);
+                staged = d->vt_staged;
+                groups = d->vt_tiles;
+            }
             break;
         }
         case SPMV_SCHED_NNZ_SPLIT:
@@ -643,7 +649,7 @@
     o->alg_bytes = 4ll * ((long long) d->m + 1) + d->nnz * (4 + s) + s * d->n + s * d->m;
     o->inspect_ms = d->inspect_ms;
     o->tuned_choice = d->blk_on ? 100 + d->blk.form : d->vec_choice;
-    if (!d->blk_on && d->rows_depth && (d->plan.sched == SPMV_SCHED_ROWBLOCK || (d->plan.sched == SPMV_SCHED_CSR_VECTOR && d->vt_wide))) o->tuned_choice = d->rows_depth == 2 ? VEC_TILE_D2 : VEC_TILE_D4;
+    if (!d->blk_on && d->rows_depth && (d->plan.sched == SPMV_SCHED_ROWBLOCK || (d->plan.sched == SPMV_SCHED_CSR_VECTOR && vt_uniform_blocks(d)))) o->tuned_choice = d->rows_depth == 2 ? VEC_TILE_D2 : VEC_TILE_D4;
     for (int k = 0; k < 3; ++k) o->tune_ms[k] = d->blk_on ? d->blk.tune_ms[k] : d->tune_ms[k];
     o->schedule_name = kSchedNames[d->plan.sched];
     o->kernel_name = kKernelNames[d->plan.sched];
@@ -659,6 +665,12 @@
     o->far_nnz = d->sp_far ? d->sp_far->nnz : 0;
     o->pack_ms[0] = d->pack_ms[0];
     o->pack_ms[1] = d->pack_ms[1];
+    if (!d->blk_on && d->plan.sched == SPMV_SCHED_CSR_VECTOR) {
+        o->tall_ms[0] = d->tall_ms[0];
+        o->tall_ms[1] = d->tall_ms[1];
+        o->tile_rows = d->vt_rows;
+        o->tile_rows_fallback = d->tall_fallback ? 1 : 0;
+    }
     {
         const bool tiles_run = !d->blk_on && (d->plan.sched == SPMV_SCHED_CSR_VECTOR || d->plan.sched == SPMV_SCHED_ROWBLOCK) && vec_kernel != kVecPipeKernel;
         o->run_nnz = tiles_run ? d->vt_run_nnz : 0;
diff --git a/spmv_amd/csrc/spmv_vector.hip b/spmv_amd/csrc/spmv_vector.hip
--- a/spmv_amd/csrc/spmv_vector.hip
+++ b/spmv_amd/csrc/spmv_vector.hip
@@ -83,20 +83,26 @@
 }
 #endif
 #else
-template <typename T, int L, int DEPTH, bool WIDE>
+template <typename T, int L, int DEPTH, bool WIDE, bool UNI>
 static void launch_rows(const VecArgs &a, const T *x, T *y)
 {
     const size_t lds = vec_lds_bytes<T>(a);
-    ensure_lds<csr_vector_rows_kernel<T, L, DEPTH, WIDE>>(a.device, lds);
-    csr_vector_rows_kernel<T, L, DEPTH, WIDE><<<a.tiles, kVecTileThreads, lds, a.stream>>>(a.long_thr, a.split, a.rows, a.m, a.rowptr, a.colidx, a.col, (const T *) a.val,
+    ensure_lds<csr_vector_rows_kernel<T, L, DEPTH, WIDE, UNI>>(a.device, lds);
+    csr_vector_rows_kernel<T, L, DEPTH, WIDE, UNI><<<a.tiles, kVecTileThreads, lds, a.stream>>>(a.long_thr, a.split, a.rows, a.m, a.rowptr, a.colidx, a.col, (const T *) a.val,
                                                                                           a.wins, a.rowslot, a.col8, a.tmpl, a.rowtid, x, y);
 }
 
 template <typename T, int L>
 static void launch_rows_form(const VecArgs &a, const T *x, T *y)
 {
-    if (a.depth == 2) { if (a.wide) launch_rows<T, L, 2, true>(a, x, y); else launch_rows<T, L, 2, false>(a, x, y); }
-    else { if (a.wide) launch_rows<T, L, 4, true>(a, x, y); else launch_rows<T, L, 4, false>(a, x, y); }
+    const bool uni = a.split == nullptr;
+#define SPMV_ROWS_FORM(D)                                                                     \
+    do {                                                                                      \
+        if (a.wide) { if (uni) launch_rows<T, L, D, true, true>(a, x, y); else launch_rows<T, L, D, true, false>(a, x, y); }   \
+        else { if (uni) launch_rows<T, L, D, false, true>(a, x, y); else launch_rows<T, L, D, false, false>(a, x, y); }        \
+    } while (0)
+    if (a.depth == 2) SPMV_ROWS_FORM(2); else SPMV_ROWS_FORM(4);
+#undef SPMV_ROWS_FORM
 }
 
 using Val = std::conditional<SPMV_VEC_PART == 2, double, float>::type;
```

Result: slower. 1535 (-10.0%).
